# Sirui-Xu/InterDiff

Hardware: AMD Instinct MI355X
Metric: denoising frame-steps/sec (denoising-steps/sec x B x T frames) (higher is better)
Workload: dtype f32 (every contraction of the denoiser -- feed-forward block, QKV projection, self-attention, row-block contractions and the two token GEMMs: every fp32 operand as two f16 planes, 3 f16 MFMAs per product, fp32 accumulate; SMPL and everything else fp32 MFMA / VALU)

## Files before the change

include/interdiff_hip.h:

```cpp
#ifndef INTERDIFF_HIP_H
#define INTERDIFF_HIP_H

#include <stddef.h>
#include <stdint.h>

#ifdef __cplusplus
extern "C" {
#endif

#define IDF_OK            0
#define IDF_E_INVAL      -22
#define IDF_E_NOMEM      -12
#define IDF_E_LAUNCH     -5

int         interdiff_abi_version(void);
const char *interdiff_build_info(void);

int interdiff_rotation_6d_to_matrix   (const float *d6, float *m,  int64_t n, void *stream);
int interdiff_matrix_to_rotation_6d   (const float *m,  float *d6, int64_t n, void *stream);
int interdiff_matrix_to_axis_angle    (const float *m,  float *aa, int64_t n, void *stream);
int interdiff_axis_angle_to_matrix    (const float *aa, float *m,  int64_t n, void *stream);
int interdiff_axis_angle_to_quaternion(const float *aa, float *q,  int64_t n, void *stream);
int interdiff_rotation_6d_to_axis_angle(const float *d6, float *aa, int64_t n, void *stream);

typedef struct {
    int32_t V, J, n_betas, KB, S;
    const float   *blend;
    const float   *jt;
    const float   *js;
    const int32_t *parents;
    const int32_t *skin_idx;
    const float   *skin_w;
} idf_smpl_model;

size_t interdiff_smpl_workspace_bytes(const idf_smpl_model *m, int64_t N);
int interdiff_smpl_forward(const idf_smpl_model *m, const float *pose, const float *betas,
                           const float *trans, int64_t N, float *verts, float *jtr,
                           float *v_posed, void *ws, size_t ws_bytes, void *stream);

int interdiff_vertex_normals(const float *verts, int64_t N, int32_t V, const int32_t *faces,
                             const int32_t *adj_ptr, const int32_t *adj_face,
                             const int32_t *adj_corner, float *normals, void *stream);
int interdiff_nn_argmin(const float *q, int32_t Pq, const float *r, int32_t Pr, int64_t N,
                        int32_t *idx, void *stream);
int interdiff_point2point_signed(const float *x, int32_t P1, const float *y, int32_t P2, int64_t N,
                                 const float *x_normals, const float *y_normals,
                                 float *y2x_signed, float *x2y_signed, int32_t *yidx, int32_t *xidx,
                                 float *y2x, float *x2y, void *stream);

#define IDF_MDM_LAYERS 8
#define IDF_MDM_D      256
#define IDF_MDM_FF     1024
#define IDF_MDM_HEADS  4
#define IDF_MDM_NQ     10
#define IDF_MDM_MEM    10
#define IDF_MDM_MEM_MAX 16
#define IDF_FFN_SLICES 5

typedef struct {
    int64_t is_qan;
    int64_t sa_in_w, sa_in_b, sa_out_w, sa_out_b;
    int64_t qc, wk;
    int64_t ca_q_w, ca_q_b;
    int64_t ca_kv_w, ca_kv_b;
    int64_t ca_out_w, ca_out_b;
    int64_t ff1_w, ff1_b, ff2_w, ff2_b;
    int64_t ffn_pack;
    int64_t ffn_b1p;
    int64_t sa_in_pack;
    int64_t sa_out_frag;
    int64_t ln_w[3], ln_b[3];
    int64_t ffn_pack_h2;
    int64_t sa_in_pack_h2;
    int64_t qc_h2;
    int64_t rb_h2_ok;
    int64_t sa_out_frag_h2;
    int64_t qkv_bounds_ok;
} idf_mdm_layer;

typedef struct {
    int32_t C;
    int32_t n_steps;
    const float *arena;
    int64_t in_w, in_b;
    int64_t out_w, out_b;
    int64_t temb_table;
    int64_t pe;
    int32_t max_T, has_encoder;
    idf_mdm_layer layer[IDF_MDM_LAYERS];
    idf_mdm_layer enc_layer[IDF_MDM_LAYERS];
    int32_t tune[8];
    int64_t out_w_h2, in_w_h2;
    int64_t tail_h2_ok;
    int32_t mem_len;
    int32_t rb_tokens;
} idf_mdm_weights;

int interdiff_gemm_f32(const float *A, int32_t lda, const float *W, const float *bias, const float *resid, float *C,
                       int32_t ldc, int32_t M, int32_t N, int32_t K, int32_t epi, int32_t cfg, void *stream);

int interdiff_mdm_ffn(const idf_mdm_weights *w, int32_t layer, int32_t encoder, const float *x2, int32_t M, float *parts, void *stream);
size_t interdiff_mdm_memctx_floats_for(int32_t B, int32_t mem_len);

size_t interdiff_mdm_memctx_floats(int32_t B);
size_t interdiff_mdm_workspace_bytes(int32_t B, int32_t T);
int interdiff_mdm_prepare_memory(const idf_mdm_weights *w, const float *cond, int32_t B,
                                 float *memctx, void *ws, size_t ws_bytes, void *stream);
int interdiff_mdm_forward(const idf_mdm_weights *w, const float *memctx, const float *x,
                          const int64_t *ts, int32_t B, int32_t T, float *x0,
                          void *ws, size_t ws_bytes, void *stream);

typedef struct {
    int64_t w[3], b[3];
    int32_t c[4];
} idf_pn_mlp;

typedef struct {
    const float *arena;
    idf_pn_mlp sa1[2];
    idf_pn_mlp sa2[2];
    int64_t lin_w, lin_b;
} idf_pointnet2;

int interdiff_pointnet2_encode(const idf_pointnet2 *pn, const float *obj_points, int32_t B, int32_t P, float *out,
                               void *stream);
size_t interdiff_mdm_encode_workspace_bytes(int32_t B, int32_t Tp);
int interdiff_mdm_encode(const idf_mdm_weights *w, const float *pc, const float *x_past, int32_t B, int32_t Tp,
                         float *cond, void *ws, size_t ws_bytes, void *stream);

int interdiff_inpaint(float *x0, const float *gt, const uint8_t *mask, int64_t n, void *stream);
int interdiff_posterior_step(float *x, const float *x0, const float *noise, int64_t n,
                             float c1, float c2, float sigma, uint64_t seed, uint64_t step_index,
                             void *stream);
int interdiff_randn(float *out, int64_t n, uint64_t seed, uint64_t step_index, void *stream);
int interdiff_posterior_step_at(float *x, const float *x0, const float *noise, int64_t n,
                                float c1, float c2, float sigma, uint64_t seed, uint64_t step_index,
                                uint64_t elem0, void *stream);
int interdiff_randn_at(float *out, int64_t n, uint64_t seed, uint64_t step_index, uint64_t elem0, void *stream);
int interdiff_posterior_step_dev(float *x, const float *x0, const float *gt, const uint8_t *mask, int64_t n,
                                 const float *table, int64_t *state, int64_t *ts, int32_t B, void *stream);
int interdiff_sampler_advance(int64_t *state, int64_t *ts, int32_t B, void *stream);
int interdiff_posterior_step_dev_map(float *x, const float *x0, const float *gt, const uint8_t *mask, int64_t n,
                                     const float *table, const int64_t *tmap, int64_t *state, int64_t *ts, int32_t B, void *stream);
int interdiff_sampler_advance_map(int64_t *state, int64_t *ts, const int64_t *tmap, int32_t B, void *stream);
int interdiff_mdm_forward_step(const idf_mdm_weights *w, const float *memctx, float *x, int64_t *ts, int32_t B, int32_t T,
                               const float *gt, const uint8_t *mask, const float *table, int64_t *state,
                               void *ws, size_t ws_bytes, void *stream);
#define IDF_STEP_EMBED_READY 1
#define IDF_STEP_EMBED_NEXT 2
int interdiff_mdm_forward_step_ex(const idf_mdm_weights *w, const float *memctx, float *x, int64_t *ts, int32_t B, int32_t T,
                                  const float *gt, const uint8_t *mask, const float *table, int64_t *state, void *ws,
                                  size_t ws_bytes, int32_t flags, void *stream);
int interdiff_mdm_forward_step_map(const idf_mdm_weights *w, const float *memctx, float *x, int64_t *ts, int32_t B, int32_t T,
                                   const float *gt, const uint8_t *mask, const float *table, const int64_t *tmap, int64_t *state,
                                   void *ws, size_t ws_bytes, int32_t flags, void *stream);
int interdiff_mdm_step_chaining(const idf_mdm_weights *w);
int interdiff_exclusive_cu_report(char *buf, int32_t cap);
int interdiff_debug_deny_exclusive(const char *patterns);

typedef struct {
    int32_t T, past_len, P, n_pre;
    const float *arena;
    int64_t dct_pad;
    int64_t dct;
    int64_t idct;
    int64_t hand_bonus;
    int64_t layer[12];
    int32_t cin[12], cout[12];
} idf_objproj;

int interdiff_objprojector_sample(const idf_objproj *op, const float *obj_angles,
                                  const float *obj_trans, const float *markers,
                                  const int32_t *contact, int32_t B, float *out, void *stream);
size_t interdiff_objprojector_forward_workspace_bytes(int32_t B);
int interdiff_objprojector_forward(const idf_objproj *op, const float *obj_angles, const float *obj_trans, const float *markers,
                                   const int32_t *contact, int32_t B, int32_t initialize, float *out, void *ws, size_t ws_bytes, void *stream);

typedef struct {
    const idf_smpl_model *smpl;
    const idf_objproj    *objproj;
    const int32_t *faces;
    const int32_t *adj_ptr, *adj_face, *adj_corner;
    const int32_t *markers_idx;
    int32_t n_markers, n_points, past_len;
    int32_t tune;
    const int32_t *vorder, *faces_scan, *markers_scan, *adj_pair_scan;
    const int32_t *adj_pair;
    const int32_t *vrank;
} idf_correction_ctx;

size_t interdiff_correction_workspace_bytes(const idf_correction_ctx *c, int32_t B, int32_t T);
int interdiff_correction(const idf_correction_ctx *c, float *x0, const float *gt,
                         const float *hand_pose, const float *beta, const float *obj_points,
                         int32_t B, int32_t T, float blend_t ,
                         uint8_t *condition, int32_t *contact, float *distance, float *loss,
                         void *ws, size_t ws_bytes, void *stream);
int interdiff_correction_dev(const idf_correction_ctx *c, float *x0, const float *gt, const float *hand_pose,
                             const float *beta, const float *obj_points, int32_t B, int32_t T, const float *table,
                             const int64_t *state, void *ws, size_t ws_bytes, void *stream);

#define IDF_CONTACT_STATS 12
size_t interdiff_contact_nn_workspace_bytes(const idf_correction_ctx *c, int32_t B, int32_t T);
int interdiff_contact_nn(const idf_correction_ctx *c, const float *verts, const float *obj_points, const float *objR,
                         const float *objT, int32_t B, int32_t T, float *o2h, int32_t *idx, uint64_t *stats,
                         void *ws, size_t ws_bytes, void *stream);

size_t interdiff_metrics_workspace_bytes(const idf_correction_ctx *c, int32_t B, int32_t T);
int interdiff_metrics(const idf_correction_ctx *c, const float *obj_pred, const float *jtr,
                      const float *body_trans, const float *obj_gt, const float *jtr_gt,
                      const float *body_trans_gt, const float *verts, const float *obj_points,
                      int32_t B, int32_t T, int32_t J, float *out6 ,
                      void *ws, size_t ws_bytes, void *stream);

typedef struct {
    int32_t T, past_len, J, n_pre;
    const float *arena;
    int64_t dct_pad;
    int64_t dct;
    int64_t idct;
    int64_t layer[12];
    int32_t cin[12], cout[12];
} idf_skel_objproj;

int interdiff_skeleton_objprojector_sample(const idf_skel_objproj *op, const float *obj_angles,
                                           const float *obj_trans, const float *human_points, int32_t B,
                                           float *quat_out, float *trans_out, void *stream);
int interdiff_skeleton_correction(const idf_skel_objproj *op, const float *x, const float *gt,
                                  const float *zero_pose_obj, int32_t B, int32_t T, float blend_t,
                                  float *out, void *stream);
int interdiff_skeleton_metrics(const float *body_pred, const float *body_gt, const float *obj_pred,
                               const float *obj_gt, const float *pose_pred, const float *pose_gt,
                               int32_t T, int32_t B, int32_t from_frame, float *out4, void *stream);

int interdiff_skeleton_finetune_param_table(const idf_skel_objproj *op, int32_t *table, int32_t *n_param, int32_t *n_bn);
size_t interdiff_skeleton_finetune_workspace_bytes(const idf_skel_objproj *op, int32_t B);
int interdiff_skeleton_finetune_grads(const idf_skel_objproj *op, const float *params, const float *bn, const float *obj_angles,
                                      const float *obj_trans, const float *human_points, const float *pose_gt, int32_t B, int32_t T,
                                      const float *weights8, float *out9, float *grads, void *ws, size_t ws_bytes, void *stream);
int interdiff_skeleton_finetune_step(const idf_skel_objproj *op, float *arena, float *params, const float *bn, const float *grads,
                                     float *exp_avg, float *exp_avg_sq, int32_t step, double lr, double beta1, double beta2, double eps,
                                     double weight_decay, void *stream);

typedef struct idf_skel_head {
    int32_t n_body, n_points;
    int32_t n_tiles, reserved;
    int64_t out_w, out_b;
    int64_t shape_w, shape_b;
} idf_skel_head;
int interdiff_skeleton_mdm_forward(const idf_mdm_weights *w, const idf_skel_head *head, const float *memctx, const float *x,
                                   const int64_t *ts, const float *zero_pose_obj, int32_t B, int32_t T, float *x0,
                                   void *ws, size_t ws_bytes, void *stream);
int interdiff_skeleton_mdm_forward_step(const idf_mdm_weights *w, const idf_skel_head *head, const float *memctx, float *x,
                                        int64_t *ts, const float *zero_pose_obj, int32_t B, int32_t T, const float *gt,
                                        const uint8_t *mask, const float *table, int64_t *state, void *ws, size_t ws_bytes,
                                        void *stream);
int interdiff_skeleton_mdm_forward_step_map(const idf_mdm_weights *w, const idf_skel_head *head, const float *memctx, float *x,
                                            int64_t *ts, const float *zero_pose_obj, int32_t B, int32_t T, const float *gt,
                                            const uint8_t *mask, const float *table, const int64_t *tmap, int64_t *state, void *ws,
                                            size_t ws_bytes, void *stream);
size_t interdiff_skeleton_mdm_encode_workspace_bytes(int32_t B, int32_t Tp);
int interdiff_skeleton_mdm_encode(const idf_mdm_weights *w, const idf_skel_head *head, const float *zero_pose_obj,
                                  const float *x_past, int32_t B, int32_t Tp, float *cond, void *ws, size_t ws_bytes,
                                  void *stream);

#define IDF_OPT_NP 483
#define IDF_OPT_NLOSS 6
typedef struct {
    const idf_correction_ctx *geo;
    const float   *blendT;
    const int32_t *jv_ptr;
    const int32_t *jv_vtx;
    const float   *jv_w;
    int32_t K3P, _pad;
} idf_opt_ctx;

typedef struct {
    int32_t B, T, P, max_iters;
    const float *betas;
    const float *obj_points;
    float *param, *init, *grad, *m, *v, *best;
    float *pose, *tr;
    float *verts, *vposed, *verts_gt, *gv;
    float *jtr;
    float *pts, *y2x;
    float *y2x_signed;
    int32_t *yidx;
    int32_t *near;
    float *dvposed;
    float *dA;
    float *dfeat;
    float *gtr;
    float *lossf;
    float *loss;
    float *loss_hist;
    float *best_loss;
    int32_t *flag;
    uint8_t *foot_static;
    int32_t *foot_cnt;
    int32_t *ctl;
    void *smpl_ws; size_t smpl_ws_bytes;
    int32_t *porder; float *psort, *pbox;
} idf_opt_state;

int interdiff_optimize_init(const idf_opt_ctx *c, const idf_opt_state *st, const float *pose, const float *trans,
                            const float *obj_angles, const float *obj_trans, int32_t first_iter, void *stream);
int interdiff_optimize_loss_grad(const idf_opt_ctx *c, const idf_opt_state *st, void *stream);
int interdiff_optimize_step(const idf_opt_ctx *c, const idf_opt_state *st, void *stream);
int interdiff_optimize_finish(const idf_opt_ctx *c, const idf_opt_state *st, float *pose, float *trans, float *obj_angles,
                              float *obj_trans, void *stream);
int interdiff_debug_joint_map_vjp(const float *R, const float *g_out, float *g_in, int32_t n);
int interdiff_debug_lds_sentinel(uint32_t *out, int32_t n_wg, int32_t spin, void *stream);
int interdiff_debug_f16_aggressor(const float *src, size_t n_floats, float *sink, int32_t iters, int32_t grid, int32_t with_loads, void *stream);

enum { IDF_LOSS_VAL = 0, IDF_LOSS_TEST = 1 };
int interdiff_q_sample(float *x_t, const float *x0, const float *noise, const int64_t *ts, const float *sqrt_ac, const float *sqrt_1mac,
                       int32_t n_steps, const float *gt, const uint8_t *mask, int32_t B, int64_t per_clip, uint64_t seed, uint64_t elem0,
                       void *stream);
int interdiff_denoising_losses(const float *pred, const float *target, int32_t B, int32_t T, int32_t past_len, float *out, void *stream);
size_t interdiff_sample_losses_workspace_bytes(int32_t K, int32_t B);
int interdiff_sample_losses(const float *samples, const float *gt, const float *hand_pose, int32_t K, int32_t B, int32_t T, int32_t past_len,
                            int32_t variant, float *out_terms, float *out_per_clip, void *ws, size_t ws_bytes, void *stream);

size_t interdiff_skeleton_sample_losses_workspace_bytes(int32_t K, int32_t B);
int interdiff_skeleton_sample_losses(const float *pred, const float *gt, int32_t K, int32_t B, int32_t C, int32_t T, int32_t past_len,
                                     int32_t n_body, int32_t n_points, float *out_terms, float *out_per_clip, void *ws, size_t ws_bytes,
                                     void *stream);
int interdiff_skeleton_denoising_losses(const float *pred, const float *target, int32_t B, int32_t T, int32_t past_len, int32_t n_body,
                                        int32_t n_points, float *out, void *stream);

size_t interdiff_correction_losses_workspace_bytes(int32_t T, int32_t B, int32_t V, int32_t P);
int interdiff_correction_losses(const float *obj_pred, const float *obj_gt, const float *obj_points, int32_t point_stride, const float *human_verts,
                                int32_t T, int32_t B, int32_t V, int32_t P, int32_t rot_width, int32_t past_len, float *out_terms, float *out_frames,
                                void *ws, size_t ws_bytes, void *stream);

size_t interdiff_contact_labels_workspace_bytes(int64_t N, int32_t V, int32_t F, int32_t P);
int interdiff_contact_labels(const float *verts, int64_t N, int32_t V, const int32_t *faces, int32_t F, const float *points, int32_t P,
                             int64_t point_frame_stride, const float *objR, const float *objT, float thres, uint8_t *obj_label ,
                             uint8_t *human_label , float *signed_dist , void *ws, size_t ws_bytes, void *stream);
int interdiff_debug_point_triangle(const float *tri, const float *p, float *out, int32_t n);

#define IDF_RENDER_SUBPIX 16
#define IDF_RENDER_GUARD 32768
#define IDF_RENDER_MAX_DIM 2048
#define IDF_RENDER_ZONE (1 << 28)
#define IDF_RENDER_REC_INTS 20
#define IDF_RENDER_TILE 16
#define IDF_RENDER_MAX_MESHES 8
enum { IDF_RMESH_SCENE_SPACE = 1, IDF_RMESH_VERTEX_RGB = 2 };
typedef struct {
    float off[3], cam_t[3];
    float cam_cos, cam_sin, znear, focal;
    float light[9];
    float light_gain, ambient;
    float bg[3];
    float reserved;
} idf_render_scene;
typedef struct {
    const float *verts, *normals;
    const int32_t *faces;
    const float *rgb, *R, *t;
    int32_t V, F, frames, flags;
} idf_render_mesh;
size_t interdiff_render_frames_workspace_bytes(int64_t n_images, int64_t n_triangles, int32_t H, int32_t W);
int interdiff_render_frames(const idf_render_scene *scene, const idf_render_mesh *meshes, int32_t n_meshes, int64_t N, int32_t views, int32_t H,
                            int32_t W, uint8_t *out_rgb, int32_t *out_id, int32_t *out_depth, int32_t *out_setup, int64_t *dropped, float *stage_ms,
                            void *ws, size_t ws_bytes, void *stream);
int interdiff_debug_render_setup_vertex(const idf_render_scene *scene, int32_t view, int32_t scene_space, int32_t H, int32_t W, const float *pos,
                                        const float *nrm, const float *rgb, float *out_f, int32_t *out_i, int32_t n);
int interdiff_debug_render_pixel(const int32_t *rec, const int32_t *ij, int32_t *out, int32_t n);

enum {
    IDF_K_EMBED = 0, IDF_K_GEMM_QKV, IDF_K_SELF_ATTN, IDF_K_GEMM_OUTPROJ, IDF_K_ROWBLOCK_QAN,
    IDF_K_ROWBLOCK_STD, IDF_K_FFN_FUSED, IDF_K_RESERVED7, IDF_K_GEMM_HEADS, IDF_K_MEM_PREP,
    IDF_K_INPAINT, IDF_K_POSTERIOR, IDF_K_CORR_PREPARE, IDF_K_SMPL_POSE, IDF_K_SMPL_BLEND_SKIN,
    IDF_K_CORR_CONTACT, IDF_K_CORR_REDUCE, IDF_K_OBJPROJ, IDF_K_CORR_BLEND, IDF_K_OTHER,
    IDF_K_COUNT
};
int interdiff_profile_begin(int32_t capacity);
int interdiff_profile_end(double *ms_per_kind, int64_t *count_per_kind);

enum {
    IDF_TUNE_FFN = 3, IDF_TUNE_FFN_MATH = 4, IDF_TUNE_COUNT = 8
};

#ifdef __cplusplus
}
#endif
#endif
```

interdiff_amd/_lib.py:

```python
import ctypes as C
import os
import torch

_HERE = os.path.dirname(os.path.abspath(__file__))
LIB_PATH = os.environ.get('INTERDIFF_HIP_LIB') or os.path.join(_HERE, 'csrc', 'libinterdiff_hip.so')
ABI_VERSION = 17

vp, i32, i64, f32, u64, sz = C.c_void_p, C.c_int32, C.c_int64, C.c_float, C.c_uint64, C.c_size_t

MDM_LAYERS = 8
FFN_SLICES = 5
STEP_EMBED_READY, STEP_EMBED_NEXT = 1, 2
LOSS_VAL, LOSS_TEST = 0, 1
TUNE = dict(ffn=3, ffn_math=4)


class SmplModel(C.Structure):
    _fields_ = [('V', i32), ('J', i32), ('n_betas', i32), ('KB', i32), ('S', i32),
                ('blend', vp), ('jt', vp), ('js', vp), ('parents', vp), ('skin_idx', vp), ('skin_w', vp)]


class MdmLayer(C.Structure):
    _fields_ = [('is_qan', i64),
                ('sa_in_w', i64), ('sa_in_b', i64), ('sa_out_w', i64), ('sa_out_b', i64),
                ('qc', i64), ('wk', i64),
                ('ca_q_w', i64), ('ca_q_b', i64), ('ca_kv_w', i64), ('ca_kv_b', i64),
                ('ca_out_w', i64), ('ca_out_b', i64),
                ('ff1_w', i64), ('ff1_b', i64), ('ff2_w', i64), ('ff2_b', i64), ('ffn_pack', i64), ('ffn_b1p', i64), ('sa_in_pack', i64), ('sa_out_frag', i64),
                ('ln_w', i64 * 3), ('ln_b', i64 * 3), ('ffn_pack_h2', i64), ('sa_in_pack_h2', i64), ('qc_h2', i64), ('rb_h2_ok', i64), ('sa_out_frag_h2', i64), ('qkv_bounds_ok', i64)]


class MdmWeights(C.Structure):
    _fields_ = [('C', i32), ('n_steps', i32), ('arena', vp),
                ('in_w', i64), ('in_b', i64), ('out_w', i64), ('out_b', i64),
                ('temb_table', i64), ('pe', i64), ('max_T', i32), ('has_encoder', i32),
                ('layer', MdmLayer * MDM_LAYERS), ('enc_layer', MdmLayer * MDM_LAYERS), ('tune', i32 * 8), ('out_w_h2', i64), ('in_w_h2', i64), ('tail_h2_ok', i64), ('mem_len', i32), ('rb_tokens', i32)]


class PnMlp(C.Structure):
    _fields_ = [('w', i64 * 3), ('b', i64 * 3), ('c', i32 * 4)]


class PointNet2(C.Structure):
    _fields_ = [('arena', vp), ('sa1', PnMlp * 2), ('sa2', PnMlp * 2), ('lin_w', i64), ('lin_b', i64)]


class ObjProj(C.Structure):
    _fields_ = [('T', i32), ('past_len', i32), ('P', i32), ('n_pre', i32), ('arena', vp),
                ('dct_pad', i64), ('dct', i64), ('idct', i64), ('hand_bonus', i64),
                ('layer', i64 * 12), ('cin', i32 * 12), ('cout', i32 * 12)]


class SkelObjProj(C.Structure):
    _fields_ = [('T', i32), ('past_len', i32), ('J', i32), ('n_pre', i32), ('arena', vp),
                ('dct_pad', i64), ('dct', i64), ('idct', i64),
                ('layer', i64 * 12), ('cin', i32 * 12), ('cout', i32 * 12)]


class SkelHead(C.Structure):
    _fields_ = [('n_body', i32), ('n_points', i32), ('n_tiles', i32), ('reserved', i32),
                ('out_w', i64), ('out_b', i64), ('shape_w', i64), ('shape_b', i64)]


class CorrectionCtx(C.Structure):
    _fields_ = [('smpl', C.POINTER(SmplModel)), ('objproj', C.POINTER(ObjProj)),
                ('faces', vp), ('adj_ptr', vp), ('adj_face', vp), ('adj_corner', vp), ('markers_idx', vp),
                ('n_markers', i32), ('n_points', i32), ('past_len', i32), ('tune', i32),
                ('vorder', vp), ('faces_scan', vp), ('markers_scan', vp), ('adj_pair_scan', vp), ('adj_pair', vp), ('vrank', vp)]


class OptCtx(C.Structure):
    _fields_ = [('geo', C.POINTER(CorrectionCtx)), ('blendT', vp), ('jv_ptr', vp), ('jv_vtx', vp), ('jv_w', vp), ('K3P', i32), ('_pad', i32)]


OPT_NP, OPT_NLOSS = 483, 6
_OPT_PTRS = ('betas', 'obj_points', 'param', 'init', 'grad', 'm', 'v', 'best', 'pose', 'tr', 'verts', 'vposed', 'verts_gt', 'gv',
             'jtr', 'pts', 'y2x', 'y2x_signed', 'yidx', 'near', 'dvposed', 'dA', 'dfeat', 'gtr', 'lossf', 'loss', 'loss_hist',
             'best_loss', 'flag', 'foot_static', 'foot_cnt', 'ctl', 'smpl_ws')


class OptState(C.Structure):
    _fields_ = [('B', i32), ('T', i32), ('P', i32), ('max_iters', i32)] + [(k, vp) for k in _OPT_PTRS] + [('smpl_ws_bytes', sz), ('porder', vp), ('psort', vp), ('pbox', vp)]


class RenderScene(C.Structure):
    _fields_ = [('off', f32 * 3), ('cam_t', f32 * 3), ('cam_cos', f32), ('cam_sin', f32), ('znear', f32), ('focal', f32),
                ('light', f32 * 9), ('light_gain', f32), ('ambient', f32), ('bg', f32 * 3), ('reserved', f32)]


class RenderMesh(C.Structure):
    _fields_ = [('verts', vp), ('normals', vp), ('faces', vp), ('rgb', vp), ('R', vp), ('t', vp),
                ('V', i32), ('F', i32), ('frames', i32), ('flags', i32)]


RMESH_SCENE_SPACE, RMESH_VERTEX_RGB = 1, 2
RENDER_SUBPIX, RENDER_GUARD, RENDER_MAX_DIM, RENDER_ZONE, RENDER_REC_INTS, RENDER_TILE = 16, 32768, 2048, 1 << 28, 20, 16

_SIGS = {
    'interdiff_abi_version': (C.c_int, []),
    'interdiff_build_info': (C.c_char_p, []),
    'interdiff_rotation_6d_to_matrix': (C.c_int, [vp, vp, i64, vp]),
    'interdiff_matrix_to_rotation_6d': (C.c_int, [vp, vp, i64, vp]),
    'interdiff_matrix_to_axis_angle': (C.c_int, [vp, vp, i64, vp]),
    'interdiff_axis_angle_to_matrix': (C.c_int, [vp, vp, i64, vp]),
    'interdiff_axis_angle_to_quaternion': (C.c_int, [vp, vp, i64, vp]),
    'interdiff_rotation_6d_to_axis_angle': (C.c_int, [vp, vp, i64, vp]),
    'interdiff_smpl_workspace_bytes': (sz, [C.POINTER(SmplModel), i64]),
    'interdiff_smpl_forward': (C.c_int, [C.POINTER(SmplModel), vp, vp, vp, i64, vp, vp, vp, vp, sz, vp]),
    'interdiff_vertex_normals': (C.c_int, [vp, i64, i32, vp, vp, vp, vp, vp, vp]),
    'interdiff_nn_argmin': (C.c_int, [vp, i32, vp, i32, i64, vp, vp]),
    'interdiff_point2point_signed': (C.c_int, [vp, i32, vp, i32, i64, vp, vp, vp, vp, vp, vp, vp, vp, vp]),
    'interdiff_gemm_f32': (C.c_int, [vp, i32, vp, vp, vp, vp, i32, i32, i32, i32, i32, i32, vp]),
    'interdiff_pointnet2_encode': (C.c_int, [C.POINTER(PointNet2), vp, i32, i32, vp, vp]),
    'interdiff_mdm_encode_workspace_bytes': (sz, [i32, i32]),
    'interdiff_mdm_encode': (C.c_int, [C.POINTER(MdmWeights), vp, vp, i32, i32, vp, vp, sz, vp]),
    'interdiff_mdm_ffn': (C.c_int, [C.POINTER(MdmWeights), i32, i32, vp, i32, vp, vp]),
    'interdiff_mdm_memctx_floats': (sz, [i32]),
    'interdiff_mdm_memctx_floats_for': (sz, [i32, i32]),
    'interdiff_mdm_workspace_bytes': (sz, [i32, i32]),
    'interdiff_mdm_prepare_memory': (C.c_int, [C.POINTER(MdmWeights), vp, i32, vp, vp, sz, vp]),
    'interdiff_mdm_forward': (C.c_int, [C.POINTER(MdmWeights), vp, vp, vp, i32, i32, vp, vp, sz, vp]),
    'interdiff_mdm_forward_step': (C.c_int, [C.POINTER(MdmWeights), vp, vp, vp, i32, i32, vp, vp, vp, vp, vp, sz, vp]),
    'interdiff_mdm_forward_step_ex': (C.c_int, [C.POINTER(MdmWeights), vp, vp, vp, i32, i32, vp, vp, vp, vp, vp, sz, i32, vp]),
    'interdiff_mdm_forward_step_map': (C.c_int, [C.POINTER(MdmWeights), vp, vp, vp, i32, i32, vp, vp, vp, vp, vp, vp, sz, i32, vp]),
    'interdiff_mdm_step_chaining': (C.c_int, [C.POINTER(MdmWeights)]),
    'interdiff_inpaint': (C.c_int, [vp, vp, vp, i64, vp]),
    'interdiff_posterior_step': (C.c_int, [vp, vp, vp, i64, f32, f32, f32, u64, u64, vp]),
    'interdiff_randn': (C.c_int, [vp, i64, u64, u64, vp]),
    'interdiff_posterior_step_at': (C.c_int, [vp, vp, vp, i64, f32, f32, f32, u64, u64, u64, vp]),
    'interdiff_randn_at': (C.c_int, [vp, i64, u64, u64, u64, vp]),
    'interdiff_posterior_step_dev': (C.c_int, [vp, vp, vp, vp, i64, vp, vp, vp, i32, vp]),
    'interdiff_sampler_advance': (C.c_int, [vp, vp, i32, vp]),
    'interdiff_posterior_step_dev_map': (C.c_int, [vp, vp, vp, vp, i64, vp, vp, vp, vp, i32, vp]),
    'interdiff_sampler_advance_map': (C.c_int, [vp, vp, vp, i32, vp]),
    'interdiff_objprojector_sample': (C.c_int, [C.POINTER(ObjProj), vp, vp, vp, vp, i32, vp, vp]),
    'interdiff_objprojector_forward_workspace_bytes': (sz, [i32]),
    'interdiff_objprojector_forward': (C.c_int, [C.POINTER(ObjProj), vp, vp, vp, vp, i32, i32, vp, vp, sz, vp]),
    'interdiff_correction_workspace_bytes': (sz, [C.POINTER(CorrectionCtx), i32, i32]),
    'interdiff_correction': (C.c_int, [C.POINTER(CorrectionCtx), vp, vp, vp, vp, vp, i32, i32, f32,
                                       vp, vp, vp, vp, vp, sz, vp]),
    'interdiff_correction_dev': (C.c_int, [C.POINTER(CorrectionCtx), vp, vp, vp, vp, vp, i32, i32, vp, vp, vp, sz, vp]),
    'interdiff_metrics_workspace_bytes': (sz, [C.POINTER(CorrectionCtx), i32, i32]),
    'interdiff_metrics': (C.c_int, [C.POINTER(CorrectionCtx), vp, vp, vp, vp, vp, vp, vp, vp, i32, i32, i32,
                                    vp, vp, sz, vp]),
    'interdiff_contact_nn_workspace_bytes': (sz, [C.POINTER(CorrectionCtx), i32, i32]),
    'interdiff_contact_nn': (C.c_int, [C.POINTER(CorrectionCtx), vp, vp, vp, vp, i32, i32, vp, vp, vp, vp, sz, vp]),
    'interdiff_skeleton_objprojector_sample': (C.c_int, [C.POINTER(SkelObjProj), vp, vp, vp, i32, vp, vp, vp]),
    'interdiff_skeleton_correction': (C.c_int, [C.POINTER(SkelObjProj), vp, vp, vp, i32, i32, f32, vp, vp]),
    'interdiff_skeleton_metrics': (C.c_int, [vp, vp, vp, vp, vp, vp, i32, i32, i32, vp, vp]),
    'interdiff_skeleton_finetune_param_table': (C.c_int, [C.POINTER(SkelObjProj), vp, C.POINTER(i32), C.POINTER(i32)]),
    'interdiff_skeleton_finetune_workspace_bytes': (sz, [C.POINTER(SkelObjProj), i32]),
    'interdiff_skeleton_finetune_grads': (C.c_int, [C.POINTER(SkelObjProj), vp, vp, vp, vp, vp, vp, i32, i32, C.POINTER(f32), vp, vp, vp, sz, vp]),
    'interdiff_skeleton_finetune_step': (C.c_int, [C.POINTER(SkelObjProj), vp, vp, vp, vp, vp, vp, i32, C.c_double, C.c_double, C.c_double, C.c_double,
                                                   C.c_double, vp]),
    'interdiff_skeleton_mdm_forward': (C.c_int, [C.POINTER(MdmWeights), C.POINTER(SkelHead), vp, vp, vp, vp, i32, i32, vp, vp, sz, vp]),
    'interdiff_skeleton_mdm_forward_step': (C.c_int, [C.POINTER(MdmWeights), C.POINTER(SkelHead), vp, vp, vp, vp, i32, i32, vp, vp, vp, vp, vp, sz, vp]),
    'interdiff_skeleton_mdm_forward_step_map': (C.c_int, [C.POINTER(MdmWeights), C.POINTER(SkelHead), vp, vp, vp, vp, i32, i32, vp, vp, vp, vp, vp, vp, sz, vp]),
    'interdiff_skeleton_mdm_encode_workspace_bytes': (sz, [i32, i32]),
    'interdiff_skeleton_mdm_encode': (C.c_int, [C.POINTER(MdmWeights), C.POINTER(SkelHead), vp, vp, i32, i32, vp, vp, sz, vp]),
    'interdiff_q_sample': (C.c_int, [vp, vp, vp, vp, vp, vp, i32, vp, vp, i32, i64, u64, u64, vp]),
    'interdiff_denoising_losses': (C.c_int, [vp, vp, i32, i32, i32, vp, vp]),
    'interdiff_sample_losses_workspace_bytes': (sz, [i32, i32]),
    'interdiff_sample_losses': (C.c_int, [vp, vp, vp, i32, i32, i32, i32, i32, vp, vp, vp, sz, vp]),
    'interdiff_skeleton_sample_losses_workspace_bytes': (sz, [i32, i32]),
    'interdiff_skeleton_sample_losses': (C.c_int, [vp, vp, i32, i32, i32, i32, i32, i32, i32, vp, vp, vp, sz, vp]),
    'interdiff_skeleton_denoising_losses': (C.c_int, [vp, vp, i32, i32, i32, i32, i32, vp, vp]),
    'interdiff_correction_losses_workspace_bytes': (sz, [i32, i32, i32, i32]),
    'interdiff_correction_losses': (C.c_int, [vp, vp, vp, i32, vp, i32, i32, i32, i32, i32, i32, vp, vp, vp, sz, vp]),
    'interdiff_contact_labels_workspace_bytes': (sz, [i64, i32, i32, i32]),
    'interdiff_contact_labels': (C.c_int, [vp, i64, i32, vp, i32, vp, i32, i64, vp, vp, f32, vp, vp, vp, vp, sz, vp]),
    'interdiff_debug_point_triangle': (C.c_int, [vp, vp, vp, i32]),
    'interdiff_render_frames_workspace_bytes': (sz, [i64, i64, i32, i32]),
    'interdiff_render_frames': (C.c_int, [C.POINTER(RenderScene), C.POINTER(RenderMesh), i32, i64, i32, i32, i32, vp, vp, vp, vp, C.POINTER(i64), C.POINTER(f32),
                                          vp, sz, vp]),
    'interdiff_debug_render_setup_vertex': (C.c_int, [C.POINTER(RenderScene), i32, i32, i32, i32, vp, vp, vp, vp, vp, i32]),
    'interdiff_debug_render_pixel': (C.c_int, [vp, vp, vp, i32]),
    'interdiff_optimize_init': (C.c_int, [C.POINTER(OptCtx), C.POINTER(OptState), vp, vp, vp, vp, i32, vp]),
    'interdiff_optimize_loss_grad': (C.c_int, [C.POINTER(OptCtx), C.POINTER(OptState), vp]),
    'interdiff_optimize_step': (C.c_int, [C.POINTER(OptCtx), C.POINTER(OptState), vp]),
    'interdiff_optimize_finish': (C.c_int, [C.POINTER(OptCtx), C.POINTER(OptState), vp, vp, vp, vp, vp]),
    'interdiff_debug_joint_map_vjp': (C.c_int, [vp, vp, vp, i32]),
    'interdiff_debug_lds_sentinel': (C.c_int, [vp, i32, i32, vp]),
    'interdiff_exclusive_cu_report': (C.c_int, [C.c_char_p, i32]),
    'interdiff_debug_deny_exclusive': (C.c_int, [C.c_char_p]),
    'interdiff_debug_f16_aggressor': (C.c_int, [vp, sz, vp, i32, i32, i32, vp]),
    'interdiff_profile_begin': (C.c_int, [i32]),
    'interdiff_profile_end': (C.c_int, [C.POINTER(C.c_double), C.POINTER(C.c_int64)]),
}

KERNEL_KINDS = ('embed', 'gemm_qkv', 'self_attn', 'gemm_outproj', 'rowblock_qan', 'rowblock_std', 'ffn_fused', 'reserved7',
                'gemm_heads', 'mem_prep', 'inpaint', 'posterior', 'corr_prepare', 'smpl_pose', 'smpl_blend_skin',
                'corr_contact', 'corr_reduce', 'objproj', 'corr_blend', 'other')

_lib = None


class HipLibraryMissing(RuntimeError):
    pass


def load():
    global _lib
    if _lib is not None:
        return _lib
    if not os.path.exists(LIB_PATH):
        raise HipLibraryMissing('%s not found: build it with `python -m interdiff_amd.csrc.build` '
                                '(there is no CPU/torch fallback for the hot path)' % LIB_PATH)
    lib = C.CDLL(LIB_PATH)
    for name, (res, args) in _SIGS.items():
        fn = getattr(lib, name)
        fn.restype, fn.argtypes = res, args
    if lib.interdiff_abi_version() != ABI_VERSION:
        raise HipLibraryMissing('stale %s: abi %d != %d, rebuild' % (LIB_PATH, lib.interdiff_abi_version(), ABI_VERSION))
    _lib = lib
    return lib


def exclusive_cu_report():
    buf = C.create_string_buffer(8192)
    bad = load().interdiff_exclusive_cu_report(buf, len(buf))
    if bad < 0:
        check(bad, 'exclusive_cu_report')
    return buf.value.decode(), bad


def debug_deny_exclusive(patterns=''):
    check(load().interdiff_debug_deny_exclusive(patterns.encode() if patterns else None), 'debug_deny_exclusive')


def exported_symbols():
    return sorted(_SIGS)


_ERR = {-22: 'IDF_E_INVAL (bad shape / pointer / unsupported size)', -12: 'IDF_E_NOMEM (workspace too small)',
        -5: 'IDF_E_LAUNCH (kernel launch failed)'}


def check(rc, what=''):
    if rc != 0:
        raise RuntimeError('interdiff_hip %s failed: %s' % (what, _ERR.get(rc, rc)))


def dptr(t, dtype=None, allow_none=False):
    if t is None:
        if allow_none:
            return vp(None)
        raise ValueError('null tensor')
    if not t.is_cuda:
        raise ValueError('interdiff_amd ops need device tensors (got %s); the HIP path has no CPU fallback' % t.device)
    if not t.is_contiguous():
        raise ValueError('tensor must be contiguous')
    if dtype is not None and t.dtype != dtype:
        raise ValueError('expected %s, got %s' % (dtype, t.dtype))
    return vp(t.data_ptr())


def stream():
    return vp(torch.cuda.current_stream().cuda_stream)
```

interdiff_amd/correction.py:

```python
import ctypes as C
import os
import itertools
import numpy as np
import torch
from . import _lib
from .geometry import MeshTopology

MARKERS67 = [3470, 3171, 3327, 857, 1812, 628, 182, 3116, 3040, 239,
             1666, 1725, 0, 2174, 1568, 1368, 3387, 2112, 1053, 1058,
             3336, 3346, 1323, 2108, 3122, 3314, 1252, 1082, 1861, 1454,
             850, 2224, 3233, 1769, 6728, 4343, 5273, 4116, 3694, 6399,
             6540, 6488, 3749, 5135, 5194, 3512, 5635, 5210, 4360, 4841,
             6786, 5573, 4538, 4544, 6736, 6747, 4804, 5568, 6544, 6682,
             5322, 4927, 5686, 4598, 6633, 3506, 3508]


_UID = itertools.count(1)


def correction_gate(t0):
    return not (t0 > 500 or t0 % 50 != 0)


class HipCorrection:
    def __init__(self, smpl_layer, objprojector, n_points=2048, past_len=10, markers=MARKERS67, device='cuda', scan_order=True):
        self.lib = _lib.load()
        self.device = torch.device(device)
        self.smpl, self.objproj, self.past_len = smpl_layer, objprojector, past_len
        self.topo = MeshTopology(smpl_layer.th_faces, smpl_layer.cmodel.V, self.device, rest_vertices=getattr(smpl_layer, 'v_template', None) if scan_order else None)
        self.markers_idx = torch.tensor(list(markers), dtype=torch.int32, device=self.device)
        ctx = _lib.CorrectionCtx()
        ctx.smpl = C.pointer(smpl_layer.cmodel)
        ctx.objproj = C.pointer(objprojector.cop)
        ctx.faces, ctx.adj_ptr = self.topo.faces.data_ptr(), self.topo.adj_ptr.data_ptr()
        ctx.adj_face, ctx.adj_corner = self.topo.adj_face.data_ptr(), self.topo.adj_corner.data_ptr()
        ctx.markers_idx = self.markers_idx.data_ptr()
        ctx.n_markers, ctx.n_points, ctx.past_len = len(markers), n_points, past_len
        if self.topo.vorder is not None:
            self.markers_scan = self.topo.scan_positions(markers, self.device)
            ctx.vorder, ctx.faces_scan, ctx.markers_scan = self.topo.vorder.data_ptr(), self.topo.faces_scan.data_ptr(), self.markers_scan.data_ptr()
            ctx.adj_pair_scan = self.topo.adj_pair_scan.data_ptr()
            ctx.vrank = self.topo.vrank.data_ptr()
        ctx.tune = 0
        self.ctx = ctx
        self._ws = {}
        self.debug = None
        self._uid = next(_UID)

    graph_capturable = True

    def workspace_for(self, B, T):
        return torch.empty(self.lib.interdiff_correction_workspace_bytes(C.byref(self.ctx), B, T), dtype=torch.uint8, device=self.device)

    def apply_dev(self, x, table, state, y, ws):
        B, _, Cc, T = x.shape
        if y['obj_points'].shape[1] != self.ctx.n_points:
            raise ValueError('obj_points must have %d points' % self.ctx.n_points)
        _lib.check(self.lib.interdiff_correction_dev(C.byref(self.ctx), _lib.dptr(x, torch.float32), _lib.dptr(y['inpainted_motion'], torch.float32),
                                                     _lib.dptr(y['hand_pose'], torch.float32), _lib.dptr(y['beta'], torch.float32),
                                                     _lib.dptr(y['obj_points'], torch.float32), B, T, _lib.dptr(table), _lib.dptr(state),
                                                     _lib.dptr(ws), ws.numel(), _lib.stream()), 'correction_dev')
        return x

    def _workspace(self, B, T):
        need = self.lib.interdiff_correction_workspace_bytes(C.byref(self.ctx), B, T)
        key = torch.cuda.current_stream(self.device).cuda_stream
        ws = self._ws.pop(key, None)
        if ws is None or ws.numel() < need:
            ws = torch.empty(need, dtype=torch.uint8, device=self.device)
        self._ws[key] = ws
        if len(self._ws) > self.MAX_STREAM_WORKSPACES:
            torch.cuda.synchronize(self.device)
            self._ws.pop(next(iter(self._ws)))
        return ws

    MAX_STREAM_WORKSPACES = 4

    def apply(self, x, t0, y):
        B, _, Cc, T = x.shape
        if not x.is_contiguous():
            raise ValueError('x must be contiguous (it is updated in place)')
        if y['obj_points'].shape[1] != self.ctx.n_points:
            raise ValueError('obj_points must have %d points' % self.ctx.n_points)
        gt = y['inpainted_motion'].contiguous()
        hp, beta, pts = y['hand_pose'].contiguous().float(), y['beta'].contiguous().float(), y['obj_points'].contiguous().float()
        ws = self._workspace(B, T)
        dbg = [None] * 4
        if self.debug is not None:
            dbg = [torch.empty(B, dtype=torch.uint8, device=self.device), torch.empty(B, len(MARKERS67), dtype=torch.int32, device=self.device),
                   torch.empty(B, device=self.device), torch.empty(B, device=self.device)]
        blend_t = float(np.float32(t0) / np.float32(1000))
        _lib.check(self.lib.interdiff_correction(C.byref(self.ctx), _lib.dptr(x, torch.float32), _lib.dptr(gt, torch.float32),
                                                 _lib.dptr(hp), _lib.dptr(beta), _lib.dptr(pts), B, T, blend_t,
                                                 *[_lib.dptr(d, allow_none=True) for d in dbg], _lib.dptr(ws), ws.numel(),
                                                 _lib.stream()), 'correction')
        if self.debug is not None:
            self.debug.update(condition=dbg[0], contact=dbg[1], distance=dbg[2], loss=dbg[3])
        return x

    def contact_nn(self, verts, obj_points, objR, objT, want_stats=False):
        T, B = verts.shape[:2]
        P = self.ctx.n_points
        o2h = torch.empty(T, B, P, device=self.device)
        idx = torch.empty(T, B, P, dtype=torch.int32, device=self.device)
        stats = torch.zeros(12, dtype=torch.int64, device=self.device) if want_stats else None
        need = self.lib.interdiff_contact_nn_workspace_bytes(C.byref(self.ctx), B, T)
        ws = getattr(self, '_nn_ws', None)
        if ws is None or ws.numel() < need:
            ws = self._nn_ws = torch.empty(need, dtype=torch.uint8, device=self.device)
        v, pts, R_, t_ = (a.contiguous().float() for a in (verts, obj_points, objR, objT))
        _lib.check(self.lib.interdiff_contact_nn(C.byref(self.ctx), _lib.dptr(v), _lib.dptr(pts), _lib.dptr(R_), _lib.dptr(t_), B, T, _lib.dptr(o2h),
                                                 _lib.dptr(idx), _lib.dptr(stats, allow_none=True), _lib.dptr(ws), ws.numel(), _lib.stream()), 'contact_nn')
        return (o2h, idx, tuple(int(x) for x in stats.cpu())) if want_stats else (o2h, idx)

    def is_active(self, t0):
        return correction_gate(int(t0))

    def __call__(self, x, t, model_kwargs):
        t0 = getattr(t, 'host_value', None)
        if t0 is None:
            t0 = int(t[0])
        if not correction_gate(t0):
            return x
        return self.apply(x, t0, model_kwargs['y'])
```

interdiff_amd/csrc/correction.hip:

```cpp
#include "common.h"
#include "objproj.h"
#include "rot_math.h"
#include <float.h>

namespace {

constexpr int NBODY = 22;
constexpr int CTOK = 144;

__global__ __launch_bounds__(256) void corr_prepare_kernel(const float *__restrict__ x0, const float *__restrict__ gt,
                                                           const float *__restrict__ hand_pose, int B, int T,
                                                           float *__restrict__ pose, float *__restrict__ trans,
                                                           float *__restrict__ objR, float *__restrict__ objT,
                                                           float *__restrict__ gt_angles, float *__restrict__ gt_trans) {
    const int64_t i = (int64_t)blockIdx.x * 256 + threadIdx.x;
    const int64_t N = (int64_t)B * T;
    if (i >= N * 24) return;
    const int64_t n = i / 24;
    const int slot = (int)(i - n * 24), t = (int)(n / B), b = (int)(n - (int64_t)t * B);
    const float *xb = x0 + (size_t)b * CTOK * T + t;
    if (slot < NBODY) {
        float d[6], m[9], a[3];
#pragma unroll
        for (int k = 0; k < 6; ++k) d[k] = xb[(size_t)(slot * 6 + k) * T];
        rot::rot6d_to_matrix(d, m);
        rot::matrix_to_axis_angle(m, a);
        float *p = pose + n * 156 + slot * 3;
        p[0] = a[0]; p[1] = a[1]; p[2] = a[2];
    } else if (slot == 22) {
        for (int k = 0; k < 90; ++k) pose[n * 156 + 66 + k] = hand_pose[n * 90 + k];
#pragma unroll
        for (int k = 0; k < 3; ++k) trans[n * 3 + k] = xb[(size_t)(132 + k) * T];
    } else {
        float d[6], m[9];
#pragma unroll
        for (int k = 0; k < 6; ++k) d[k] = xb[(size_t)(135 + k) * T];
        rot::rot6d_to_matrix(d, m);
#pragma unroll
        for (int k = 0; k < 9; ++k) objR[n * 9 + k] = m[k];
        const float *gb = gt + (size_t)b * CTOK * T + t;
#pragma unroll
        for (int k = 0; k < 3; ++k) {
            objT[n * 3 + k] = xb[(size_t)(141 + k) * T];
            gt_trans[n * 3 + k] = gb[(size_t)(141 + k) * T];
        }
#pragma unroll
        for (int k = 0; k < 6; ++k) gt_angles[n * 6 + k] = gb[(size_t)(135 + k) * T];
    }
}

__device__ __forceinline__ float dist2_exact(float qx, float qy, float qz, float rx, float ry, float rz) {
#pragma clang fp contract(off)
    const float dx = qx - rx, dy = qy - ry, dz = qz - rz;
    const float xx = dx * dx, yy = dy * dy, zz = dz * dz;
    return (xx + yy) + zz;
}

__device__ __forceinline__ float3 f3(const float4 v) { return make_float3(v.x, v.y, v.z); }
__device__ __forceinline__ float3 sub3(float3 a, float3 b) { return make_float3(a.x - b.x, a.y - b.y, a.z - b.z); }
__device__ __forceinline__ float3 cross3(float3 a, float3 b) {
    return make_float3(a.y * b.z - a.z * b.y, a.z * b.x - a.x * b.z, a.x * b.y - a.y * b.x);
}

constexpr int MAXP = 2048;
__global__ __launch_bounds__(1024) void corr_point_order_kernel(const float *__restrict__ obj_points, int P, int32_t *__restrict__ porder) {
    __shared__ unsigned long long keys[MAXP];
    __shared__ float red[6][1024];
    const int b = blockIdx.x, tid = threadIdx.x;
    const float *op = obj_points + (size_t)b * P * 3;
    float p[2][3];
    float lo[3] = {FLT_MAX, FLT_MAX, FLT_MAX}, hi[3] = {-FLT_MAX, -FLT_MAX, -FLT_MAX};
#pragma unroll
    for (int k = 0; k < 2; ++k) {
        const int i = tid + 1024 * k;
#pragma unroll
        for (int a = 0; a < 3; ++a) {
            p[k][a] = i < P ? op[3 * i + a] : 0.f;
            if (i < P) { lo[a] = fminf(lo[a], p[k][a]); hi[a] = fmaxf(hi[a], p[k][a]); }
        }
    }
#pragma unroll
    for (int a = 0; a < 3; ++a) { red[a][tid] = lo[a]; red[3 + a][tid] = hi[a]; }
    __syncthreads();
    for (int s = 512; s > 0; s >>= 1) {
        if (tid < s) {
#pragma unroll
            for (int a = 0; a < 3; ++a) {
                red[a][tid] = fminf(red[a][tid], red[a][tid + s]);
                red[3 + a][tid] = fmaxf(red[3 + a][tid], red[3 + a][tid + s]);
            }
        }
        __syncthreads();
    }
#pragma unroll
    for (int k = 0; k < 2; ++k) {
        const int i = tid + 1024 * k;
        unsigned long long key = ~0ull;
        if (i < P) {
            unsigned code = 0;
            unsigned q[3];
#pragma unroll
            for (int a = 0; a < 3; ++a) {
                const float ext = red[3 + a][0] - red[a][0];
                const float u = ext > 0.f ? (p[k][a] - red[a][0]) / ext : 0.f;
                q[a] = (unsigned)fminf(fmaxf(u * 1023.0f, 0.f), 1023.0f);
            }
#pragma unroll
            for (int bit = 0; bit < 10; ++bit)
#pragma unroll
                for (int a = 0; a < 3; ++a) code |= ((q[a] >> bit) & 1u) << (3 * bit + a);
            key = ((unsigned long long)code << 11) | (unsigned)i;
        }
        keys[i] = key;
    }
    __syncthreads();
    for (int k = 2; k <= MAXP; k <<= 1) {
        for (int j = k >> 1; j > 0; j >>= 1) {
            const int l = 2 * j * (tid / j) + (tid % j), r = l + j;
            const unsigned long long x = keys[l], y = keys[r];
            const bool up = (l & k) == 0;
            if ((x > y) == up) { keys[l] = y; keys[r] = x; }
            __syncthreads();
        }
    }
#pragma unroll
    for (int k = 0; k < 2; ++k) {
        const int i = tid + 1024 * k;
        if (i < P) porder[(size_t)b * P + i] = (int32_t)(keys[i] & 2047u);
    }
}

constexpr int MAXM = 128;
constexpr float MARK_D2 = 0.00039999996079131961f;
constexpr int CB = 16;
constexpr int SB = 8;
constexpr int SEED_STRIDE = 4;
constexpr int CT = 1024;
constexpr int TASK = 64;
typedef float v2f __attribute__((ext_vector_type(2)));

struct ContactLds {
    int V4, nCB, nSB, nSeed;
    int rec, mark, box, sbox, seed, flags, red, pl, total;
    __host__ __device__ explicit ContactLds(int V) {
        V4 = (V + CB - 1) / CB * CB; nCB = V4 / CB; nSB = (nCB + SB - 1) / SB; nSeed = (nCB + SEED_STRIDE - 1) / SEED_STRIDE;
        rec = 0;
        mark = rec + V4;
        box = mark + MAXM;
        sbox = box + 3 * (nSB * SB / 2);
        seed = sbox + 3 * ((nSB + 2) / 2);
        flags = seed + 2 * ((nSeed + 1) / 2);
        red = flags + MAXM / 4;
        pl = red + CT / 4;
        total = pl + MAXP / 4;
    }
};

__device__ __forceinline__ float3 lds_rec(const float4 *vs, int pos) {
    const float *f = reinterpret_cast<const float *>(vs + 2 * (pos >> 1));
    const int h = pos & 1;
    return make_float3(f[h], f[2 + h], f[4 + h]);
}
__device__ __forceinline__ void lds_rec_store(float4 *vs, int pos, float x, float y, float z) {
    float *f = reinterpret_cast<float *>(vs + 2 * (pos >> 1));
    const int h = pos & 1;
    f[h] = x; f[2 + h] = y; f[4 + h] = z;
}
__device__ __forceinline__ void lds_box_store(float4 *bx, int k, float3 lo, float3 hi) {
    float *f = reinterpret_cast<float *>(bx + 3 * (k >> 1));
    const int h = k & 1;
    f[h] = lo.x; f[2 + h] = lo.y; f[4 + h] = lo.z; f[6 + h] = hi.x; f[8 + h] = hi.y; f[10 + h] = hi.z;
}
__device__ __forceinline__ void lds_box_load(const float4 *bx, int k, float3 &lo, float3 &hi) {
    const float *f = reinterpret_cast<const float *>(bx + 3 * (k >> 1));
    const int h = k & 1;
    lo = make_float3(f[h], f[2 + h], f[4 + h]);
    hi = make_float3(f[6 + h], f[8 + h], f[10 + h]);
}

struct PredArgs {
    idf_objproj op;
    const float *obj_angles, *obj_trans;
    const int32_t *markers_idx;
    float *markers, *keep;
    int nclips;
};
template <bool OPT, bool WITH_PRED = false>
__global__ __launch_bounds__(CT) void corr_contact_kernel(const float *__restrict__ verts, int V,
                                                          const float *__restrict__ obj_points, int P,
                                                          const int32_t *__restrict__ porder ,
                                                          const float *__restrict__ objR, const float *__restrict__ objT,
                                                          const int32_t *__restrict__ faces ,
                                                          const int32_t *__restrict__ adj_ptr,
                                                          const int32_t *__restrict__ adj_face,
                                                          const int32_t *__restrict__ adj_corner,
                                                          const int32_t *__restrict__ adj_pair ,
                                                          const int32_t *__restrict__ vorder ,
                                                          const int32_t *__restrict__ vrank ,
                                                          const int32_t *__restrict__ markers_pos , int M, int B,
                                                          float *__restrict__ markers_out, float *__restrict__ loss_sum,
                                                          float *__restrict__ min_dist, int32_t *__restrict__ label,
                                                          float *__restrict__ o2h_out ,
                                                          int32_t *__restrict__ idx_out ,
                                                          unsigned long long *__restrict__ stats ,
                                                          int64_t nn_from ,
                                                          const float *__restrict__ pts_frame , int frames_per_clip ,
                                                          const PredArgs pred) {
    extern __shared__ __attribute__((aligned(16))) float4 vs[];
    if constexpr (WITH_PRED) {
        if ((int)blockIdx.x < pred.nclips) {
            const int b = blockIdx.x, Tn = pred.op.T;
            for (int i = threadIdx.x; i < Tn * M; i += CT) {
                const int t = i / M, m = i - t * M;
                const size_t nfr = (size_t)t * B + b;
                const float *v = verts + (nfr * V + pred.markers_idx[m]) * 3;
                float *o = pred.markers + (nfr * M + m) * 3;
                o[0] = v[0]; o[1] = v[1]; o[2] = v[2];
            }
            __threadfence();
            __syncthreads();
            idf_objproj_dev::objproj_body<1>(reinterpret_cast<float *>(vs), pred.op, pred.obj_angles, pred.obj_trans, pred.markers, nullptr, B, b, pred.keep, nullptr);
            return;
        }
    }
    const ContactLds L(V);
    const int nCB = L.nCB, nSB = L.nSB;
    float4 *ms = vs + L.mark, *bb = vs + L.box, *sbb = vs + L.sbox, *sd = vs + L.seed;
    int *flags = reinterpret_cast<int *>(vs + L.flags);
    float *red = reinterpret_cast<float *>(vs + L.red);
    float *pl = reinterpret_cast<float *>(vs + L.pl);
    __shared__ int next_task;
    const int64_t n = WITH_PRED ? (int64_t)blockIdx.x - pred.nclips : (int64_t)blockIdx.x;
    const int b = OPT ? (int)(n / frames_per_clip) : (int)(n % B), tid = threadIdx.x;
    const float *vf = verts + (size_t)n * V * 3;
    const bool do_nn = n >= nn_from;
    long long t_prev = 0;
    int n_phase = 0;
    auto phase_done = [&]() {
        if (stats && tid == 0 && do_nn) {
            const long long now = (long long)__builtin_readcyclecounter();
            if (n_phase > 0) atomicAdd(stats + 3 + n_phase, (unsigned long long)(now - t_prev));
            t_prev = now;
        }
        ++n_phase;
    };
    phase_done();
    float R[9] = {1.f, 0.f, 0.f, 0.f, 1.f, 0.f, 0.f, 0.f, 1.f}, tr[3] = {0.f, 0.f, 0.f};
    if constexpr (!OPT) {
#pragma unroll
        for (int k = 0; k < 9; ++k) R[k] = objR[n * 9 + k];
#pragma unroll
        for (int k = 0; k < 3; ++k) tr[k] = objT[n * 3 + k];
    }
    const int my_marker_pos = (!OPT && tid < M) ? markers_pos[tid] : 0;
    if (vorder && vrank) {
        for (int i0 = tid; i0 < V; i0 += 4 * CT) {
            typedef float f3v __attribute__((ext_vector_type(3), aligned(4)));
            int pos[4];
            f3v pv[4];
#pragma unroll
            for (int k = 0; k < 4; ++k) {
                const int i = min(i0 + k * CT, V - 1);
                pos[k] = vrank[i];
                pv[k] = *reinterpret_cast<const f3v *>(vf + 3 * i);
            }
#pragma unroll
            for (int k = 0; k < 4; ++k) {
                if (i0 + k * CT < V) {
                    lds_rec_store(vs, pos[k], pv[k].x, pv[k].y, pv[k].z);
                    reinterpret_cast<int *>(vs + 2 * (pos[k] >> 1) + 1)[2 + (pos[k] & 1)] = i0 + k * CT;
                }
            }
        }
        for (int v = V + tid; v < L.V4; v += CT) {
            lds_rec_store(vs, v, 3e18f, 3e18f, 3e18f);
            reinterpret_cast<int *>(vs + 2 * (v >> 1) + 1)[2 + (v & 1)] = 0x7fffffff;
        }
    } else
    for (int v0 = tid; v0 < L.V4; v0 += 4 * CT) {
        int o[4];
        float x[4], y[4], z[4];
#pragma unroll
        for (int k = 0; k < 4; ++k) {
            const int v = v0 + k * CT;
            o[k] = v < V ? (vorder ? vorder[v] : v) : -1;
        }
#pragma unroll
        for (int k = 0; k < 4; ++k) {
            x[k] = y[k] = z[k] = 3e18f;
            if (o[k] >= 0) {
                typedef float f3v __attribute__((ext_vector_type(3), aligned(4)));
                const f3v pv = *reinterpret_cast<const f3v *>(vf + 3 * o[k]);
                x[k] = pv.x; y[k] = pv.y; z[k] = pv.z;
            }
        }
#pragma unroll
        for (int k = 0; k < 4; ++k) {
            const int v = v0 + k * CT;
            if (v < L.V4) {
                lds_rec_store(vs, v, x[k], y[k], z[k]);
                reinterpret_cast<int *>(vs + 2 * (v >> 1) + 1)[2 + (v & 1)] = o[k] >= 0 ? o[k] : 0x7fffffff;
            }
        }
    }
    if (tid < MAXM) flags[tid] = 0;
    const int ntask_all = (P + TASK - 1) / TASK;
    const int task0 = (int)((long long)blockIdx.y * ntask_all / gridDim.y), task1 = (int)((long long)(blockIdx.y + 1) * ntask_all / gridDim.y);
    if (tid == 0) next_task = task0;
    for (int i = tid; i < MAXP; i += CT) pl[i] = 0.f;
    __syncthreads();
    phase_done();
    if (!OPT && tid < ((M + 1) & ~1)) {
        float3 mk = make_float3(3e18f, 3e18f, 3e18f);
        if (tid < M) {
            mk = lds_rec(vs, my_marker_pos);
            if (markers_out) {
                float *mo = markers_out + ((size_t)n * M + tid) * 3;
                mo[0] = mk.x; mo[1] = mk.y; mo[2] = mk.z;
            }
        }
        lds_rec_store(ms, tid, mk.x, mk.y, mk.z);
    }
    if (do_nn) {
#define IDF_DPP8(v, op, ctrl) v = op(v, __builtin_bit_cast(float, __builtin_amdgcn_update_dpp(__builtin_bit_cast(int, v), __builtin_bit_cast(int, v), ctrl, 0xf, 0xf, false)))
        const int lane_ = tid & 63, wave_ = tid >> 6, nsw = 2 * ((nSB + 2) / 2);
        for (int sb = wave_; sb < nsw; sb += CT / 64) {
            const int pr = sb * 64 + lane_;
            float lx = FLT_MAX, ly = FLT_MAX, lz = FLT_MAX, hx = -FLT_MAX, hy = -FLT_MAX, hz = -FLT_MAX;
            if (2 * pr < V) {
                const float4 xy = vs[2 * pr], zz = vs[2 * pr + 1];
                const bool two = 2 * pr + 1 < V;
                lx = two ? fminf(xy.x, xy.y) : xy.x; hx = two ? fmaxf(xy.x, xy.y) : xy.x;
                ly = two ? fminf(xy.z, xy.w) : xy.z; hy = two ? fmaxf(xy.z, xy.w) : xy.z;
                lz = two ? fminf(zz.x, zz.y) : zz.x; hz = two ? fmaxf(zz.x, zz.y) : zz.x;
            }
            IDF_DPP8(lx, fminf, 0xB1); IDF_DPP8(lx, fminf, 0x4E); IDF_DPP8(lx, fminf, 0x141);
            IDF_DPP8(ly, fminf, 0xB1); IDF_DPP8(ly, fminf, 0x4E); IDF_DPP8(ly, fminf, 0x141);
            IDF_DPP8(lz, fminf, 0xB1); IDF_DPP8(lz, fminf, 0x4E); IDF_DPP8(lz, fminf, 0x141);
            IDF_DPP8(hx, fmaxf, 0xB1); IDF_DPP8(hx, fmaxf, 0x4E); IDF_DPP8(hx, fmaxf, 0x141);
            IDF_DPP8(hy, fmaxf, 0xB1); IDF_DPP8(hy, fmaxf, 0x4E); IDF_DPP8(hy, fmaxf, 0x141);
            IDF_DPP8(hz, fmaxf, 0xB1); IDF_DPP8(hz, fmaxf, 0x4E); IDF_DPP8(hz, fmaxf, 0x141);
            const int cb = sb * SB + (lane_ >> 3);
            if ((lane_ & 7) == 0 && cb < nSB * SB) lds_box_store(bb, cb, make_float3(lx, ly, lz), make_float3(hx, hy, hz));
            const float slx = -wave_max(-lx), sly = -wave_max(-ly), slz = -wave_max(-lz), shx = wave_max(hx), shy = wave_max(hy), shz = wave_max(hz);
            if (lane_ == 0) lds_box_store(sbb, sb, make_float3(slx, sly, slz), make_float3(shx, shy, shz));
        }
#undef IDF_DPP8
        for (int k = tid; k < 2 * ((L.nSeed + 1) / 2); k += CT) {
            const float3 p = lds_rec(vs, min(k * SEED_STRIDE, nCB - 1) * CB);
            lds_rec_store(sd, k, p.x, p.y, p.z);
        }
    }
    const float *op = OPT ? pts_frame + (size_t)n * P * 3 : obj_points + (size_t)b * P * 3;
    const int ln = tid & 63, ntask = task1;
    __syncthreads();
    phase_done();
    float mind2 = FLT_MAX;
    unsigned n_exec = 0, n_test = 0, n_tasks = 0;
    for (;;) {
        int task = 0;
        if (ln == 0) task = atomicAdd(&next_task, 1);
        task = __builtin_amdgcn_readfirstlane(task);
        if (task >= ntask) break;
        ++n_tasks;
        const int sp = task * TASK + ln;
        const int i = sp < P ? (porder ? porder[(size_t)b * P + sp] : sp) : -1;
        const bool valid = i >= 0;
        float px = 0.f, py = 0.f, pz = 0.f;
        if (valid) { px = op[3 * i]; py = op[3 * i + 1]; pz = op[3 * i + 2]; }
        const float qx = OPT ? px : (px * R[0] + py * R[1] + pz * R[2]) + tr[0];
        const float qy = OPT ? py : (px * R[3] + py * R[4] + pz * R[5]) + tr[1];
        const float qz = OPT ? pz : (px * R[6] + py * R[7] + pz * R[8]) + tr[2];
        if (do_nn) {
#pragma clang fp contract(off)
            const v2f QX = v2f{qx, qx}, QY = v2f{qy, qy}, QZ = v2f{qz, qz};
            auto pair_d2 = [&](const float4 xy, const float4 zz) {
#pragma clang fp contract(off)
                const v2f dx = QX - v2f{xy.x, xy.y}, dy = QY - v2f{xy.z, xy.w}, dz = QZ - v2f{zz.x, zz.y};
                return (dx * dx + dy * dy) + dz * dz;
            };
            auto pair_a2 = [&](const float4 xy, const float2 zz) {
                const v2f dx = QX - v2f{xy.x, xy.y}, dy = QY - v2f{xy.z, xy.w}, dz = QZ - v2f{zz.x, zz.y};
                return __builtin_elementwise_fma(dz, dz, __builtin_elementwise_fma(dy, dy, dx * dx));
            };
            constexpr float SCAN_M = 1.000003814697265625f, SCAN_ABS = 1e-37f;
            float seed = FLT_MAX;
            for (int k = 0; k < (L.nSeed + 1) / 2; k += 4) {
                float4 xy[4]; float2 zz[4];
#pragma unroll
                for (int u = 0; u < 4; ++u) { xy[u] = sd[2 * min(k + u, (L.nSeed + 1) / 2 - 1)]; zz[u] = *reinterpret_cast<const float2 *>(&sd[2 * min(k + u, (L.nSeed + 1) / 2 - 1) + 1]); }
#pragma unroll
                for (int u = 0; u < 4; ++u) {
                    const v2f a2 = pair_a2(xy[u], zz[u]);
                    seed = fminf(fminf(seed, a2.x), a2.y);
                }
            }
            float thr = __builtin_fmaf(seed, SCAN_M, SCAN_ABS);
            float best = FLT_MAX, bthr = FLT_MAX;
            int tie = 0;
            int bblk = 0, bblk2 = 0;
            auto pair_lb = [&](const float4 a, const float4 bq, const float4 c) {
#pragma clang fp contract(off)
                const v2f ax = v2f{a.x, a.y} - QX, bx = QX - v2f{bq.z, bq.w};
                const v2f ay = v2f{a.z, a.w} - QY, by = QY - v2f{c.x, c.y};
                const v2f az = v2f{bq.x, bq.y} - QZ, bz = QZ - v2f{c.z, c.w};
                const v2f ex = v2f{fmaxf(fmaxf(ax.x, bx.x), 0.f), fmaxf(fmaxf(ax.y, bx.y), 0.f)};
                const v2f ey = v2f{fmaxf(fmaxf(ay.x, by.x), 0.f), fmaxf(fmaxf(ay.y, by.y), 0.f)};
                const v2f ez = v2f{fmaxf(fmaxf(az.x, bz.x), 0.f), fmaxf(fmaxf(az.y, bz.y), 0.f)};
                return __builtin_elementwise_fma(ez, ez, __builtin_elementwise_fma(ey, ey, ex * ex));
            };
            auto score_block = [&](int cb) {
                ++n_exec;
                const int v0 = cb * CB;
                float4 xy[CB / 2]; float2 zz[CB / 2];
#pragma unroll
                for (int u = 0; u < CB / 2; ++u) { xy[u] = vs[v0 + 2 * u]; zz[u] = *reinterpret_cast<const float2 *>(&vs[v0 + 2 * u + 1]); }
                float bm = FLT_MAX;
#pragma unroll
                for (int u = 0; u < CB / 2; ++u) {
                    const v2f a2 = pair_a2(xy[u], zz[u]);
                    bm = fminf(fminf(bm, a2.x), a2.y);
                }
                if (bm < best) {
                    const float w = __builtin_fmaf(bm, SCAN_M, SCAN_ABS);
                    if (best <= w) { tie = tie ? 2 : 1; bblk2 = bblk; } else tie = 0;
                    best = bm; bblk = v0; bthr = w; thr = fminf(thr, w);
                } else if (bm <= bthr) { tie = tie ? 2 : 1; bblk2 = v0; }
            };
            auto scan_super = [&](int sb) {
                const int cb0 = sb * SB;
#pragma unroll
                for (int j = 0; j < SB / 2; ++j) {
                    const int cb = cb0 + 2 * j;
                    const float4 *bx = bb + 3 * (cb >> 1);
                    const v2f lb = pair_lb(bx[0], bx[1], bx[2]);
                    n_test += 2;
                    if (__builtin_amdgcn_ballot_w64(valid && lb.x <= thr) != 0ull) score_block(cb);
                    if (__builtin_amdgcn_ballot_w64(valid && lb.y <= thr) != 0ull) score_block(cb + 1);
                }
            };
            if (!vorder) {
                for (int cb = 0; cb < nCB; ++cb) score_block(cb);
            } else
            for (int sb = 0; sb < nSB; sb += 2) {
                const float4 *bx = sbb + 3 * (sb >> 1);
                const v2f lb = pair_lb(bx[0], bx[1], bx[2]);
                n_test += 2;
                if (__builtin_amdgcn_ballot_w64(valid && lb.x <= thr) != 0ull) scan_super(sb);
                if (__builtin_amdgcn_ballot_w64(valid && lb.y <= thr) != 0ull) scan_super(sb + 1);
            }
            int pos = bblk, org = 0x7fffffff;
            float ebest = FLT_MAX;
            auto resolve_pair = [&](int pr) {
                const float4 xy = vs[2 * pr], zz = vs[2 * pr + 1];
                const v2f d2 = pair_d2(xy, zz);
                const int o0 = __builtin_bit_cast(int, zz.z), o1 = __builtin_bit_cast(int, zz.w);
                if (d2.x < ebest || (d2.x == ebest && o0 < org)) { ebest = d2.x; org = o0; pos = 2 * pr; }
                if (d2.y < ebest || (d2.y == ebest && o1 < org)) { ebest = d2.y; org = o1; pos = 2 * pr + 1; }
            };
            if (tie < 2) {
#pragma unroll
                for (int u = 0; u < CB / 2; ++u) resolve_pair((bblk >> 1) + u);
                if (tie) {
#pragma unroll
                    for (int u = 0; u < CB / 2; ++u) resolve_pair((bblk2 >> 1) + u);
                }
            } else {
                for (int pr = 0; pr < (V + 1) / 2; ++pr) resolve_pair(pr);
            }
            pos = min(pos, V - 1);
            if (org == 0x7fffffff) org = vorder ? vorder[pos] : pos;
            if constexpr (OPT) {
                if (valid) idx_out[(size_t)n * P + i] = org;
            } else if (valid) {
                const float3 v3 = lds_rec(vs, pos);
                float3 acc = make_float3(0.f, 0.f, 0.f);
                const int e0 = adj_ptr[org], e1 = adj_ptr[org + 1];
                if (adj_pair) {
                    for (int e = e0; e < e1; e += 4) {
                        int2 ab[4];
#pragma unroll
                        for (int u = 0; u < 4; ++u) ab[u] = *reinterpret_cast<const int2 *>(adj_pair + 2 * (size_t)min(e + u, e1 - 1));
#pragma unroll
                        for (int u = 0; u < 4; ++u) {
                            if (e + u < e1) {
                                const float3 nn = cross3(sub3(lds_rec(vs, ab[u].x), v3), sub3(lds_rec(vs, ab[u].y), v3));
                                acc.x += nn.x; acc.y += nn.y; acc.z += nn.z;
                            }
                        }
                    }
                } else {
                    for (int e = e0; e < e1; ++e) {
                        const int f = adj_face[e], c = adj_corner[e];
                        const float3 p0 = lds_rec(vs, faces[3 * f]), p1 = lds_rec(vs, faces[3 * f + 1]), p2 = lds_rec(vs, faces[3 * f + 2]);
                        float3 nn;
                        if (c == 1) nn = cross3(sub3(p2, p1), sub3(p0, p1));
                        else if (c == 2) nn = cross3(sub3(p0, p2), sub3(p1, p2));
                        else nn = cross3(sub3(p1, p0), sub3(p2, p0));
                        acc.x += nn.x; acc.y += nn.y; acc.z += nn.z;
                    }
                }
                const float nl = fmaxf(sqrtf(acc.x * acc.x + acc.y * acc.y + acc.z * acc.z), 1e-6f);
                const float vx = qx - v3.x, vy = qy - v3.y, vz = qz - v3.z;
                const float dt = (acc.x / nl) * vx + (acc.y / nl) * vy + (acc.z / nl) * vz;
                const float d = sqrtf(vx * vx + vy * vy + vz * vz);
                const float o2h = d * (dt > 0.f ? 1.f : (dt < 0.f ? -1.f : 0.f));
                if (o2h_out) o2h_out[(size_t)n * P + i] = o2h;
                if (idx_out) idx_out[(size_t)n * P + i] = org;
                pl[sp] = o2h < 0.f ? fabsf(o2h) * 20.0f : 0.f;
            }
        }
        if (!OPT && valid) {
#pragma clang fp contract(off)
            const v2f QX = v2f{qx, qx}, QY = v2f{qy, qy}, QZ = v2f{qz, qz};
            for (int p2 = 0; p2 < (M + 1) / 2; ++p2) {
                const float4 xy = ms[2 * p2], zz = ms[2 * p2 + 1];
                const v2f dx = v2f{xy.x, xy.y} - QX, dy = v2f{xy.z, xy.w} - QY, dz = v2f{zz.x, zz.y} - QZ;
                const v2f d2 = __builtin_elementwise_fma(dy, dy, dx * dx) + dz * dz;
                mind2 = fminf(fminf(mind2, d2.x), d2.y);
                if (__builtin_amdgcn_ballot_w64(fminf(d2.x, d2.y) < MARK_D2) != 0ull) {
                    if (d2.x < MARK_D2) flags[2 * p2] = 1;
                    if (d2.y < MARK_D2) flags[2 * p2 + 1] = 1;
                }
            }
        }
    }
    if (stats && ln == 0 && do_nn) {
        atomicAdd(stats, (unsigned long long)n_exec);
        atomicAdd(stats + 1, (unsigned long long)nCB * n_tasks);
        atomicAdd(stats + 2, (unsigned long long)n_test);
    }
    phase_done();
    if constexpr (OPT) return;
    __syncthreads();
    phase_done();
    float loss = 0.f;
#pragma unroll
    for (int k = 0; k < MAXP / CT; ++k) loss += pl[tid + CT * k];
    red[tid] = loss;
    __syncthreads();
    for (int s = CT / 2; s > 0; s >>= 1) {
        if (tid < s) red[tid] += red[tid + s];
        __syncthreads();
    }
    const float loss_total = red[0];
    __syncthreads();
    red[tid] = mind2;
    __syncthreads();
    for (int s = CT / 2; s > 0; s >>= 1) {
        if (tid < s) red[tid] = fminf(red[tid], red[tid + s]);
        __syncthreads();
    }
    if (tid == 0) { loss_sum[n] = loss_total; min_dist[n] = red[0] == FLT_MAX ? FLT_MAX : sqrtf(red[0]); }
    if (tid < M) label[(size_t)n * M + tid] = flags[tid];
    phase_done();
    if (stats && tid == 0 && do_nn) atomicAdd(stats + 3, 1ull);
}

size_t contact_lds_bytes(int V) { return (size_t)ContactLds(V).total * sizeof(float4); }

int launch_contact(hipStream_t s, int64_t N, const float *verts, int V, const float *obj_points, int P, int32_t *porder,
                   const float *objR, const float *objT, const idf_correction_ctx *c, int B, float *markers, float *loss_sum,
                   float *min_dist, int32_t *label, float *o2h, int32_t *idx, unsigned long long *stats, int64_t nn_from, const PredArgs *pred = nullptr) {
    const int M = c->n_markers;
    const size_t lds = contact_lds_bytes(V);
    if (lds > 160 * 1024 - 16384 || P > MAXP) return IDF_E_INVAL;
    const bool ordered = c->vorder != nullptr;
    if (ordered != (c->faces_scan != nullptr) || ordered != (c->markers_scan != nullptr) || ordered != (c->adj_pair_scan != nullptr)) return IDF_E_INVAL;
    const int32_t *faces = ordered ? c->faces_scan : c->faces, *mpos = ordered ? c->markers_scan : c->markers_idx;
    if (porder) hipLaunchKernelGGL(corr_point_order_kernel, dim3((unsigned)B), dim3(1024), 0, s, obj_points, P, porder);
    if (pred) {
        const size_t lds2 = (pred->nclips > 0 && lds < idf_objproj_dev::OBJPROJ_LDS) ? idf_objproj_dev::OBJPROJ_LDS : lds;
        static std::atomic<uint64_t> lds_ok2{0};
        if (lds2 > 160 * 1024 - 2048) return IDF_E_INVAL;
        if (idf_opt_in_lds(reinterpret_cast<const void *>(corr_contact_kernel<false, true>), 160 * 1024 - 2048, lds_ok2) != IDF_OK) return IDF_E_LAUNCH;
        hipLaunchKernelGGL((corr_contact_kernel<false, true>), dim3((unsigned)(N + pred->nclips)), dim3(CT), lds2, s, verts, V, obj_points, P, porder, objR, objT, faces,
                           c->adj_ptr, c->adj_face, c->adj_corner, c->adj_pair_scan, c->vorder, c->vrank, mpos, M, B, markers, loss_sum, min_dist, label, o2h, idx,
                           stats, nn_from, nullptr, 0, *pred);
        return IDF_OK;
    }
    static std::atomic<uint64_t> lds_ok{0};
    if (idf_opt_in_lds(reinterpret_cast<const void *>(corr_contact_kernel<false>), 160 * 1024 - 16384, lds_ok) != IDF_OK) return IDF_E_LAUNCH;
    hipLaunchKernelGGL(corr_contact_kernel<false>, dim3((unsigned)N), dim3(CT), lds, s, verts, V, obj_points, P, porder, objR, objT, faces,
                       c->adj_ptr, c->adj_face, c->adj_corner, c->adj_pair_scan, c->vorder, c->vrank, mpos, M, B, markers, loss_sum, min_dist, label, o2h, idx,
                       stats, nn_from, nullptr, 0, PredArgs{});
    return IDF_OK;
}

__global__ __launch_bounds__(128) void corr_reduce_kernel(const float *__restrict__ loss_sum, const float *__restrict__ min_dist,
                                                          const int32_t *__restrict__ label, int B, int T, int past, int P, int M,
                                                          uint8_t *__restrict__ condition, int32_t *__restrict__ contact,
                                                          float *__restrict__ distance_out, float *__restrict__ loss_out) {
    extern __shared__ float fr[];
    const int b = blockIdx.x, tid = threadIdx.x;
    for (int t = tid; t < T; t += 128) {
        fr[t] = loss_sum[(size_t)t * B + b];
        fr[T + t] = min_dist[(size_t)t * B + b];
    }
    if (tid < M) {
        int c = 0;
#pragma unroll 16
        for (int t = past; t < T; ++t) c += label[((size_t)t * B + b) * M + tid];
        contact[(size_t)b * M + tid] = c;
    }
    __syncthreads();
    if (tid == 0) {
        float ls = 0.f, ds = 0.f;
        for (int t = past; t < T; ++t) ls += fr[t] / (float)P;
        for (int t = 0; t < T; ++t) ds += fr[T + t];
        const float loss = ls / (float)(T - past), dist = ds / (float)T;
        condition[b] = !((loss < 0.002f) && (dist < 0.02f));
        if (distance_out) distance_out[b] = dist;
        if (loss_out) loss_out[b] = loss;
    }
}

__global__ __launch_bounds__(256) void corr_blend_kernel(float *__restrict__ x0, const float *__restrict__ proj,
                                                         const uint8_t *__restrict__ condition, int B, int T, float a,
                                                         const float *__restrict__ a_table, const int64_t *__restrict__ a_state) {
    if (a_table) a = a_table[a_state[0] * 4 + 3];
    const int64_t i = (int64_t)blockIdx.x * 256 + threadIdx.x;
    if (i >= (int64_t)B * CTOK * T) return;
    const int b = (int)(i / (CTOK * T)), r = (int)(i - (int64_t)b * CTOK * T), c = r / T, t = r - c * T;
    if (!condition[b]) return;
    const float x = x0[i];
    const float other = c < 135 ? x : proj[((size_t)t * B + b) * 9 + (c - 135)];
    x0[i] = a * x + (1.0f - a) * other;
}

struct CorrWs {
    float *pose, *trans, *objR, *objT, *gt_angles, *gt_trans, *verts, *jtr, *markers, *loss_sum, *min_dist, *proj, *proj_keep;
    int32_t *label, *contact, *porder;
    uint8_t *condition;
    void *smpl_ws;
    size_t smpl_ws_bytes, total;
};

CorrWs carve(const idf_correction_ctx *c, int B, int T, void *ws) {
    const int64_t N = (int64_t)B * T;
    const int V = c->smpl->V, J = c->smpl->J, M = c->n_markers;
    char *p = reinterpret_cast<char *>(ws);
    size_t off = 0;
    auto take = [&](size_t bytes) { char *r = p ? p + off : nullptr; off += idf_align(bytes); return r; };
    CorrWs w;
    w.pose = (float *)take(N * 156 * 4);
    w.trans = (float *)take(N * 3 * 4);
    w.objR = (float *)take(N * 9 * 4);
    w.objT = (float *)take(N * 3 * 4);
    w.gt_angles = (float *)take(N * 6 * 4);
    w.gt_trans = (float *)take(N * 3 * 4);
    w.verts = (float *)take((size_t)N * V * 3 * 4);
    w.jtr = (float *)take((size_t)N * J * 3 * 4);
    w.markers = (float *)take((size_t)N * M * 3 * 4);
    w.loss_sum = (float *)take(N * 4);
    w.min_dist = (float *)take(N * 4);
    w.proj = (float *)take(N * 9 * 4);
    w.label = (int32_t *)take((size_t)N * M * 4);
    w.contact = (int32_t *)take((size_t)B * M * 4);
    w.condition = (uint8_t *)take(B);
    w.porder = (int32_t *)take((size_t)B * c->n_points * 4);
    w.proj_keep = (float *)take((size_t)B * idf_objproj_keep_floats() * 4);
    w.smpl_ws_bytes = interdiff_smpl_workspace_bytes(c->smpl, N);
    w.smpl_ws = take(w.smpl_ws_bytes);
    w.total = off;
    return w;
}


constexpr int NPATCH = MAXP / 64;
__global__ __launch_bounds__(256) void opt_patch_kernel(const float *__restrict__ pts, int P, const int32_t *__restrict__ porder, int frames_per_clip,
                                                        float4 *__restrict__ psort , float4 *__restrict__ pbox ) {
    const int64_t n = blockIdx.x;
    const int b = (int)(n / frames_per_clip), tid = threadIdx.x, lane = tid & 63, wave = tid >> 6;
    const float *pn = pts + (size_t)n * P * 3;
    for (int k = wave; k < NPATCH; k += 4) {
        const int sp = 64 * k + lane;
        float x = 3e18f, y = 3e18f, z = 3e18f;
        float lx = FLT_MAX, ly = FLT_MAX, lz = FLT_MAX, hx = -FLT_MAX, hy = -FLT_MAX, hz = -FLT_MAX;
        if (sp < P) {
            const int i = porder[(size_t)b * P + sp];
            x = pn[3 * i]; y = pn[3 * i + 1]; z = pn[3 * i + 2];
            lx = hx = x; ly = hy = y; lz = hz = z;
        }
        psort[(size_t)n * MAXP + sp] = make_float4(x, y, z, 0.f);
        lx = -wave_max(-lx); ly = -wave_max(-ly); lz = -wave_max(-lz);
        hx = wave_max(hx); hy = wave_max(hy); hz = wave_max(hz);
        if (lane == 0) {
            pbox[((size_t)n * NPATCH + k) * 2] = make_float4(lx, ly, lz, 0.f);
            pbox[((size_t)n * NPATCH + k) * 2 + 1] = make_float4(hx, hy, hz, 0.f);
        }
    }
}

__global__ __launch_bounds__(256) void opt_near_kernel(const float *__restrict__ verts, int V, int P, const float4 *__restrict__ psort,
                                                       const float4 *__restrict__ pbox, const int32_t *__restrict__ vorder,
                                                       int32_t *__restrict__ near) {
    __shared__ float4 ps[MAXP];
    __shared__ float4 bx[NPATCH * 2];
    const int64_t n = blockIdx.y;
    const int tid = threadIdx.x, pos = blockIdx.x * 256 + tid, vid = vorder[min(pos, V - 1)];
    for (int i = tid; i < MAXP; i += 256) ps[i] = psort[(size_t)n * MAXP + i];
    if (tid < NPATCH * 2) bx[tid] = pbox[(size_t)n * NPATCH * 2 + tid];
    const bool valid = pos < V;
    const float *vp = verts + ((size_t)n * V + vid) * 3;
    const float vx = vp[0], vy = vp[1], vz = vp[2];
    __syncthreads();
    const int npatch = (P + 63) / 64;
    bool hit = false;
    {
#pragma clang fp contract(off)
        const v2f VX = v2f{vx, vx}, VY = v2f{vy, vy}, VZ = v2f{vz, vz};
        for (int k = 0; k < npatch; ++k) {
            if (__builtin_amdgcn_ballot_w64(valid && !hit) == 0ull) break;
            const float4 lo = bx[2 * k], hi = bx[2 * k + 1];
            const float ex = fmaxf(fmaxf(lo.x - vx, vx - hi.x), 0.f), ey = fmaxf(fmaxf(lo.y - vy, vy - hi.y), 0.f), ez = fmaxf(fmaxf(lo.z - vz, vz - hi.z), 0.f);
            const float xx = ex * ex, yy = ey * ey, zz = ez * ez;
            if (__builtin_amdgcn_ballot_w64(valid && !hit && (xx + yy) + zz < 0.25f) == 0ull) continue;
            const float4 *pp = ps + 64 * k;
            for (int j0 = 0; j0 < 64; j0 += 16) {
#pragma unroll
                for (int j = j0; j < j0 + 16; j += 2) {
                    const float4 p = pp[j], q = pp[j + 1];
                    const v2f dx = v2f{p.x, q.x} - VX, dy = v2f{p.y, q.y} - VY, dz = v2f{p.z, q.z} - VZ;
                    const v2f d2 = (dx * dx + dy * dy) + dz * dz;
                    hit = hit || d2.x < 0.25f || d2.y < 0.25f;
                }
                if (__builtin_amdgcn_ballot_w64(valid && !hit) == 0ull) break;
            }
        }
    }
    if (valid) near[(size_t)n * V + vid] = hit ? 1 : 0;
}

}

int idf_point_order(hipStream_t s, const float *obj_points, int B, int P, int32_t *porder) {
    if (P > MAXP) return IDF_E_INVAL;
    hipLaunchKernelGGL(corr_point_order_kernel, dim3((unsigned)B), dim3(1024), 0, s, obj_points, P, porder);
    return IDF_OK;
}

int idf_nn_scan_opt(hipStream_t s, int64_t N, int frames_per_clip, const float *verts, int V, const float *pts_frame, const float *obj_points, int P,
                    const int32_t *porder, const idf_correction_ctx *c, int32_t *yidx) {
    const size_t lds = contact_lds_bytes(V);
    if (lds > 160 * 1024 - 16384 || P > MAXP || !c->vorder) return IDF_E_INVAL;
    const int B = (int)(N / frames_per_clip);
    static std::atomic<uint64_t> lds_ok{0};
    if (idf_opt_in_lds(reinterpret_cast<const void *>(corr_contact_kernel<true>), 160 * 1024 - 16384, lds_ok) != IDF_OK) return IDF_E_LAUNCH;
    hipLaunchKernelGGL(corr_contact_kernel<true>, dim3((unsigned)N, 2), dim3(CT), lds, s, verts, V, obj_points, P, porder, nullptr, nullptr, nullptr,
                       nullptr, nullptr, nullptr, nullptr, c->vorder, c->vrank, nullptr, 0, B, nullptr, nullptr, nullptr, nullptr, nullptr, yidx, nullptr, (int64_t)0,
                       pts_frame, frames_per_clip, PredArgs{});
    return IDF_OK;
}

int idf_near_mask_opt(hipStream_t s, int64_t N, int frames_per_clip, const float *verts, int V, const float *pts_frame, int P, const int32_t *porder,
                      const int32_t *vorder, float *psort, float *pbox, int32_t *near) {
    if (P > MAXP || !vorder) return IDF_E_INVAL;
    hipLaunchKernelGGL(opt_patch_kernel, dim3((unsigned)N), dim3(256), 0, s, pts_frame, P, porder, frames_per_clip, reinterpret_cast<float4 *>(psort),
                       reinterpret_cast<float4 *>(pbox));
    hipLaunchKernelGGL(opt_near_kernel, dim3((unsigned)idf_cdiv(V, 256), (unsigned)N), dim3(256), 0, s, verts, V, P, reinterpret_cast<const float4 *>(psort),
                       reinterpret_cast<const float4 *>(pbox), vorder, near);
    return IDF_OK;
}

namespace {

}

extern "C" size_t interdiff_correction_workspace_bytes(const idf_correction_ctx *c, int32_t B, int32_t T) {
    if (!c || !c->smpl || B <= 0 || T <= 0) return 0;
    return carve(c, B, T, nullptr).total;
}

static int correction_impl(const idf_correction_ctx *c, float *x0, const float *gt, const float *hand_pose,
                           const float *beta, const float *obj_points, int32_t B, int32_t T, float blend_t, const float *blend_table,
                           const int64_t *blend_state, uint8_t *condition, int32_t *contact, float *distance, float *loss, void *ws,
                           size_t ws_bytes, void *stream) {
    if (!c || !c->smpl || !c->objproj || !x0 || !gt || !hand_pose || !beta || !obj_points || !ws || B <= 0 || T <= 0) return IDF_E_INVAL;
    const int V = c->smpl->V, M = c->n_markers, P = c->n_points;
    if (c->smpl->J != 52 || c->smpl->n_betas != 10 || M > MAXM || M != c->objproj->P || P > MAXP || T != c->objproj->T ||
        c->past_len != c->objproj->past_len || c->past_len >= T)
        return IDF_E_INVAL;
    CorrWs w = carve(c, B, T, ws);
    if (ws_bytes < w.total) return IDF_E_NOMEM;
    hipStream_t s = idf_stream(stream);
    const int64_t N = (int64_t)B * T;
    const bool fused = (c->tune & 2) == 0 && idf_objproj_check(c->objproj) == IDF_OK;
    idf_prof_mark(IDF_K_CORR_PREPARE, s);
    hipLaunchKernelGGL(corr_prepare_kernel, dim3((unsigned)idf_cdiv(N * 24, 256)), dim3(256), 0, s, x0, gt, hand_pose, B, T, w.pose,
                       w.trans, w.objR, w.objT, w.gt_angles, w.gt_trans);
    int rc = interdiff_smpl_forward(c->smpl, w.pose, beta, w.trans, N, w.verts, w.jtr, nullptr, w.smpl_ws, w.smpl_ws_bytes, stream);
    if (rc) return rc;
    idf_prof_mark(IDF_K_CORR_CONTACT, s);
    PredArgs pred{};
    if (fused) {
        pred.op = *c->objproj;
        pred.obj_angles = w.gt_angles; pred.obj_trans = w.gt_trans;
        pred.markers_idx = c->markers_idx; pred.markers = w.markers; pred.keep = w.proj_keep;
        pred.nclips = B;
    }
    rc = launch_contact(s, N, w.verts, V, obj_points, P, w.porder, w.objR, w.objT, c, B, fused ? nullptr : w.markers, w.loss_sum, w.min_dist, w.label, nullptr,
                        nullptr, nullptr, (int64_t)c->past_len * B, &pred);
    if (rc) return rc;
    uint8_t *cond = condition ? condition : w.condition;
    int32_t *cont = contact ? contact : w.contact;
    idf_prof_mark(IDF_K_CORR_REDUCE, s);
    hipLaunchKernelGGL(corr_reduce_kernel, dim3(B), dim3(128), 2 * (size_t)T * sizeof(float), s, w.loss_sum, w.min_dist, w.label, B, T, c->past_len, P, M, cond,
                       cont, distance, loss);
    if (fused) {
        idf_prof_mark(IDF_K_OBJPROJ, s);
        rc = idf_objproj_pick(c->objproj, w.proj_keep, cont, B, w.proj, s);
    } else {
        rc = interdiff_objprojector_sample(c->objproj, w.gt_angles, w.gt_trans, w.markers, cont, B, w.proj, stream);
    }
    if (rc) return rc;
    idf_prof_mark(IDF_K_CORR_BLEND, s);
    hipLaunchKernelGGL(corr_blend_kernel, dim3((unsigned)idf_cdiv((int64_t)B * CTOK * T, 256)), dim3(256), 0, s, x0, w.proj, cond, B, T,
                       blend_t, blend_table, blend_state);
    idf_prof_mark(-1, s);
    IDF_CHECK_LAUNCH();
    return IDF_OK;
}

extern "C" int interdiff_correction(const idf_correction_ctx *c, float *x0, const float *gt, const float *hand_pose,
                                    const float *beta, const float *obj_points, int32_t B, int32_t T, float blend_t,
                                    uint8_t *condition, int32_t *contact, float *distance, float *loss, void *ws,
                                    size_t ws_bytes, void *stream) {
    return correction_impl(c, x0, gt, hand_pose, beta, obj_points, B, T, blend_t, nullptr, nullptr, condition, contact, distance, loss, ws, ws_bytes, stream);
}

extern "C" int interdiff_correction_dev(const idf_correction_ctx *c, float *x0, const float *gt, const float *hand_pose,
                                        const float *beta, const float *obj_points, int32_t B, int32_t T, const float *table,
                                        const int64_t *state, void *ws, size_t ws_bytes, void *stream) {
    if (!table || !state) return IDF_E_INVAL;
    return correction_impl(c, x0, gt, hand_pose, beta, obj_points, B, T, 0.f, table, state, nullptr, nullptr, nullptr, nullptr, ws, ws_bytes, stream);
}

namespace {

__global__ __launch_bounds__(256) void metrics_prepare_kernel(const float *__restrict__ obj_pred, int64_t N,
                                                              float *__restrict__ objR, float *__restrict__ objT) {
    const int64_t n = (int64_t)blockIdx.x * 256 + threadIdx.x;
    if (n >= N) return;
    float q[4], m[9];
    rot::axis_angle_to_quaternion(obj_pred + n * 6, q);
    rot::quaternion_to_matrix(q, m);
#pragma unroll
    for (int k = 0; k < 9; ++k) objR[n * 9 + k] = m[k];
#pragma unroll
    for (int k = 0; k < 3; ++k) objT[n * 3 + k] = obj_pred[n * 6 + 3 + k];
}

__device__ __forceinline__ float block_sum(float v, float *red) {
    red[threadIdx.x] = v;
    __syncthreads();
    for (int s = 128; s > 0; s >>= 1) {
        if (threadIdx.x < s) red[threadIdx.x] += red[threadIdx.x + s];
        __syncthreads();
    }
    const float r = red[0];
    __syncthreads();
    return r;
}

__global__ __launch_bounds__(256) void metrics_reduce_kernel(const float *__restrict__ obj_pred, const float *__restrict__ jtr,
                                                             const float *__restrict__ body_trans, const float *__restrict__ obj_gt,
                                                             const float *__restrict__ jtr_gt, const float *__restrict__ body_trans_gt,
                                                             const float *__restrict__ o2h, int B, int T, int J, int P,
                                                             float *__restrict__ out6) {
    __shared__ float red[256];
    const int b = blockIdx.x, tid = threadIdx.x;
    float g = 0.f, l = 0.f;
    for (int i = tid; i < T * J; i += 256) {
        const int t = i / J, j = i - t * J;
        const float *a = jtr + (((size_t)t * B + b) * J + j) * 3, *c = jtr_gt + (((size_t)t * B + b) * J + j) * 3;
        const float *a0 = jtr + ((size_t)t * B + b) * J * 3, *c0 = jtr_gt + ((size_t)t * B + b) * J * 3;
        const float dx = a[0] - c[0], dy = a[1] - c[1], dz = a[2] - c[2];
        g += sqrtf(dx * dx + dy * dy + dz * dz);
        const float ex = (a[0] - a0[0]) - (c[0] - c0[0]), ey = (a[1] - a0[1]) - (c[1] - c0[1]), ez = (a[2] - a0[2]) - (c[2] - c0[2]);
        l += sqrtf(ex * ex + ey * ey + ez * ez);
    }
    float bt = 0.f, ot = 0.f, rq = 0.f;
    for (int t = tid; t < T; t += 256) {
        const size_t n = (size_t)t * B + b;
        const float *x = body_trans + n * 3, *y = body_trans_gt + n * 3;
        bt += sqrtf((x[0] - y[0]) * (x[0] - y[0]) + (x[1] - y[1]) * (x[1] - y[1]) + (x[2] - y[2]) * (x[2] - y[2]));
        const float *p = obj_pred + n * 6, *q = obj_gt + n * 6;
        ot += sqrtf((p[3] - q[3]) * (p[3] - q[3]) + (p[4] - q[4]) * (p[4] - q[4]) + (p[5] - q[5]) * (p[5] - q[5]));
        float qa[4], qb[4];
        rot::axis_angle_to_quaternion(p, qa);
        rot::axis_angle_to_quaternion(q, qb);
        float e1 = 0.f, e2 = 0.f;
#pragma unroll
        for (int k = 0; k < 4; ++k) { e1 += fabsf(qa[k] - qb[k]); e2 += fabsf(qa[k] + qb[k]); }
        rq += fminf(e1, e2);
    }
    const float gs = block_sum(g, red), ls = block_sum(l, red), bs = block_sum(bt, red), os = block_sum(ot, red), rs = block_sum(rq, red);
    float pen = 0.f;
    for (int t = 0; t < T; ++t) {
        const float *row = o2h + ((size_t)t * B + b) * P;
        float c = 0.f;
        for (int i = tid; i < P; i += 256) c += row[i] < 0.f ? 1.f : 0.f;
        const float cs = block_sum(c, red);
        pen += cs / (float)P;
    }
    if (tid == 0) {
        out6[0 * B + b] = gs / (float)J / (float)T;
        out6[1 * B + b] = ls / (float)J / (float)T;
        out6[2 * B + b] = bs / (float)T;
        out6[3 * B + b] = os / (float)T;
        out6[4 * B + b] = rs / (float)T;
        out6[5 * B + b] = pen / (float)T;
    }
}

struct MetWs {
    float *objR, *objT, *o2h, *markers, *loss_sum, *min_dist;
    int32_t *label, *porder;
    size_t total;
};
MetWs carve_metrics(const idf_correction_ctx *c, int B, int T, void *ws) {
    const int64_t N = (int64_t)B * T;
    char *p = reinterpret_cast<char *>(ws);
    size_t off = 0;
    auto take = [&](size_t bytes) { char *r = p ? p + off : nullptr; off += idf_align(bytes); return r; };
    MetWs w;
    w.objR = (float *)take(N * 9 * 4);
    w.objT = (float *)take(N * 3 * 4);
    w.o2h = (float *)take((size_t)N * c->n_points * 4);
    w.markers = (float *)take((size_t)N * c->n_markers * 3 * 4);
    w.loss_sum = (float *)take(N * 4);
    w.min_dist = (float *)take(N * 4);
    w.label = (int32_t *)take((size_t)N * c->n_markers * 4);
    w.porder = (int32_t *)take((size_t)B * c->n_points * 4);
    w.total = off;
    return w;
}

}

extern "C" size_t interdiff_contact_nn_workspace_bytes(const idf_correction_ctx *c, int32_t B, int32_t T) {
    if (!c || B <= 0 || T <= 0) return 0;
    return carve_metrics(c, B, T, nullptr).total;
}

extern "C" int interdiff_contact_nn(const idf_correction_ctx *c, const float *verts, const float *obj_points, const float *objR,
                                    const float *objT, int32_t B, int32_t T, float *o2h, int32_t *idx, uint64_t *stats, void *ws,
                                    size_t ws_bytes, void *stream) {
    if (!c || !c->smpl || !verts || !obj_points || !objR || !objT || !ws || B <= 0 || T <= 0 || (!o2h && !idx)) return IDF_E_INVAL;
    if (c->n_markers > MAXM || c->n_points > MAXP) return IDF_E_INVAL;
    MetWs w = carve_metrics(c, B, T, ws);
    if (ws_bytes < w.total) return IDF_E_NOMEM;
    hipStream_t s = idf_stream(stream);
    if (stats && hipMemsetAsync(stats, 0, IDF_CONTACT_STATS * sizeof(uint64_t), s) != hipSuccess) return IDF_E_LAUNCH;
    const int rc = launch_contact(s, (int64_t)B * T, verts, c->smpl->V, obj_points, c->n_points, w.porder, objR, objT, c, B, w.markers, w.loss_sum,
                                  w.min_dist, w.label, o2h ? o2h : w.o2h, idx, reinterpret_cast<unsigned long long *>(stats), 0);
    if (rc) return rc;
    IDF_CHECK_LAUNCH();
    return IDF_OK;
}

extern "C" size_t interdiff_metrics_workspace_bytes(const idf_correction_ctx *c, int32_t B, int32_t T) {
    if (!c || B <= 0 || T <= 0) return 0;
    return carve_metrics(c, B, T, nullptr).total;
}

extern "C" int interdiff_metrics(const idf_correction_ctx *c, const float *obj_pred, const float *jtr, const float *body_trans,
                                 const float *obj_gt, const float *jtr_gt, const float *body_trans_gt, const float *verts,
                                 const float *obj_points, int32_t B, int32_t T, int32_t J, float *out6, void *ws, size_t ws_bytes,
                                 void *stream) {
    if (!c || !c->smpl || !obj_pred || !jtr || !body_trans || !obj_gt || !jtr_gt || !body_trans_gt || !verts || !obj_points || !out6 ||
        !ws || B <= 0 || T <= 0 || J <= 0)
        return IDF_E_INVAL;
    const int V = c->smpl->V, M = c->n_markers, P = c->n_points;
    if (M > MAXM || P > MAXP) return IDF_E_INVAL;
    MetWs w = carve_metrics(c, B, T, ws);
    if (ws_bytes < w.total) return IDF_E_NOMEM;
    hipStream_t s = idf_stream(stream);
    const int64_t N = (int64_t)B * T;
    idf_prof_mark(IDF_K_OTHER, s);
    hipLaunchKernelGGL(metrics_prepare_kernel, dim3((unsigned)idf_cdiv(N, 256)), dim3(256), 0, s, obj_pred, N, w.objR, w.objT);
    const int rc = launch_contact(s, N, verts, V, obj_points, P, w.porder, w.objR, w.objT, c, B, w.markers, w.loss_sum, w.min_dist, w.label, w.o2h,
                                  nullptr, nullptr, 0);
    if (rc) return rc;
    hipLaunchKernelGGL(metrics_reduce_kernel, dim3(B), dim3(256), 0, s, obj_pred, jtr, body_trans, obj_gt, jtr_gt, body_trans_gt, w.o2h, B,
                       T, J, P, out6);
    idf_prof_mark(-1, s);
    IDF_CHECK_LAUNCH();
    return IDF_OK;
}
```

interdiff_amd/csrc/smpl.hip:

```cpp
#include "common.h"
#include "rot_math.h"
#include <algorithm>

#ifndef IDF_SMPL_STAMP
#define IDF_SMPL_STAMP(i) do { } while (0)
#endif

namespace {

constexpr int MAXJ = 64;

__global__ __launch_bounds__(64) void smpl_pose_kernel(const idf_smpl_model m, const float *__restrict__ pose,
                                                       const float *__restrict__ betas, const float *__restrict__ trans,
                                                       float *__restrict__ feat, float *__restrict__ A,
                                                       float *__restrict__ jtr) {
    __shared__ float Rs[MAXJ * 9], Js[MAXJ * 3], Gs[MAXJ * 12];
    const int64_t n = blockIdx.x;
    const int j = threadIdx.x, J = m.J, nb = m.n_betas, KB = m.KB;
    const float *beta = betas + n * nb;
    if (j < J) {
        rot::rodrigues_smpl(pose + n * 3 * J + 3 * j, Rs + j * 9);
#pragma unroll
        for (int c = 0; c < 3; ++c) {
            float s = m.jt[j * 3 + c];
            const float *jsr = m.js + (size_t)(j * 3 + c) * nb;
            for (int k = 0; k < nb; ++k) s += jsr[k] * beta[k];
            Js[j * 3 + c] = s;
        }
    }
    float *f = feat + n * KB;
    if (j >= 1 && j < J) {
#pragma unroll
        for (int e = 0; e < 9; ++e) f[(j - 1) * 9 + e] = Rs[j * 9 + e] - ((e == 0 || e == 4 || e == 8) ? 1.0f : 0.0f);
    }
    const int base = 9 * (J - 1);
    for (int k = j; k < KB - base; k += 64) f[base + k] = k < nb ? beta[k] : (k == nb ? 1.0f : 0.0f);
    __syncthreads();
    if (j < 12) {
        const int r = j >> 2, c = j & 3;
        Gs[j] = c < 3 ? Rs[r * 3 + c] : Js[r];
    }
    __syncthreads();
    for (int i = 1; i < J; ++i) {
        const int p = m.parents[i];
        if (j < 12) {
            const int r = j >> 2, c = j & 3;
            const float *gp = Gs + p * 12 + r * 4;
            float v;
            if (c < 3)
                v = gp[0] * Rs[i * 9 + c] + gp[1] * Rs[i * 9 + 3 + c] + gp[2] * Rs[i * 9 + 6 + c];
            else
                v = gp[0] * (Js[i * 3] - Js[p * 3]) + gp[1] * (Js[i * 3 + 1] - Js[p * 3 + 1]) +
                    gp[2] * (Js[i * 3 + 2] - Js[p * 3 + 2]) + gp[3];
            Gs[i * 12 + j] = v;
        }
        __syncthreads();
    }
    if (j < J) {
        const float *g = Gs + j * 12;
        const float jx = Js[j * 3], jy = Js[j * 3 + 1], jz = Js[j * 3 + 2];
        float *a = A + ((size_t)n * J + j) * 12;
#pragma unroll
        for (int r = 0; r < 3; ++r) {
            a[r * 4 + 0] = g[r * 4 + 0];
            a[r * 4 + 1] = g[r * 4 + 1];
            a[r * 4 + 2] = g[r * 4 + 2];
            a[r * 4 + 3] = g[r * 4 + 3] - (g[r * 4] * jx + g[r * 4 + 1] * jy + g[r * 4 + 2] * jz);
            jtr[((size_t)n * J + j) * 3 + r] = g[r * 4 + 3] + trans[n * 3 + r];
        }
    }
}

constexpr int FT = 32, VT = 64, NTC = 3 * VT;
constexpr int BT = 256;
constexpr int FM = FT / 16;
constexpr int STS = NTC + 1;
constexpr int SF = 16;
constexpr int TBF = 10, TBV = 4;

template <int NG>
__global__ __launch_bounds__(BT) void smpl_blend_skin_kernel(const idf_smpl_model m, const float *__restrict__ feat,
                                                              const float *__restrict__ A, const float *__restrict__ trans,
                                                              int64_t N, float *__restrict__ verts,
                                                              float *__restrict__ v_posed) {
    extern __shared__ __attribute__((aligned(16))) float sm[];
    idf_args_now(m.V, m.J, m.S, m.blend, m.skin_idx, m.skin_w, feat, A, trans, N, verts, v_posed, gridDim.x);
    constexpr int KB = 16 * NG, nq = KB / 4;
    const int V = m.V, J = m.J, S = m.S;
    float *As = sm, *stage = sm;
    const int tid = threadIdx.x, lane = tid & 63, wave = (tid >> 6) & 3, fh = tid >> 8, li = lane & 15, kq = lane >> 4;
    const int nft = (int)((N + FT - 1) / FT), nvt = (V + VT - 1) / VT;
    const int nwg = gridDim.x, id = blockIdx.x;
    const int xq = nwg >> 3, xr = nwg & 7, xcd = id & 7;
    const int lid = (xcd < xr ? xcd * (xq + 1) : xr * (xq + 1) + (xcd - xr) * xq) + (id >> 3);
    const int blk = lid / (TBF * TBV), wi = lid - blk * (TBF * TBV);
    const int nvb = (nvt + TBV - 1) / TBV;
    const int ftile = blk / nvb * TBF + wi % TBF, vtile = blk % nvb * TBV + wi / TBF;
    if (ftile >= nft || vtile >= nvt) return;
    const int64_t f0 = (int64_t)ftile * FT;
    const int v0 = vtile * VT;
    IDF_SMPL_STAMP(0);

    {
        const uint32_t as_lds = idf_lds_addr(As);
        const int ncell = FT * nq;
        for (int i = wave; i * 64 < ncell; i += BT / 64) {
            const int p = min(i * 64 + lane, ncell - 1), row = p / nq, pos = p - row * nq;
            idf_dma16_v(feat + (size_t)min(f0 + row, N - 1) * KB + ((pos ^ ((row >> 1) & 7)) << 2), as_lds + (uint32_t)(i * 1024));
        }
    }
    const int vl = tid & 63, vme = v0 + vl;
    float sw[4];
    int so[4];
#pragma unroll
    for (int k = 0; k < 4; ++k) {
        const size_t e = (size_t)min(vme, V - 1) * S + min(k, S - 1);
        sw[k] = m.skin_w[e];
        so[k] = m.skin_idx[e] * 12;
    }
#pragma unroll
    for (int k = 0; k < 4; ++k) {
        const bool ok = k < S && vme < V;
        sw[k] = ok ? sw[k] : 0.f;
        so[k] = ok ? so[k] : 0;
    }
    asm volatile("s_waitcnt vmcnt(0)" ::: "memory");
    __syncthreads();
    IDF_SMPL_STAMP(1);

    const float *brow[3];
#pragma unroll
    for (int t = 0; t < 3; ++t) brow[t] = m.blend + ((size_t)((vtile * 4 + wave) * 3 + t) * NG * 64 + lane) * 4;
    f32x4 acc[FM][3];
#pragma unroll
    for (int i = 0; i < FM; ++i)
#pragma unroll
        for (int t = 0; t < 3; ++t) acc[i][t] = f32x4{0.f, 0.f, 0.f, 0.f};
    constexpr int PD = 3;
    float4 bq[PD + 1][3];
    auto ldg = [&](float4 (&dst)[3], int gi) {
#pragma unroll
        for (int t = 0; t < 3; ++t) dst[t] = *reinterpret_cast<const float4 *>(brow[t] + gi * 256);
    };
    auto mac = [&](const float4 (&bc)[3], int gi) {
#pragma unroll
        for (int i = 0; i < FM; ++i) {
            const int row = (fh * FM + i) * 16 + li;
            const float4 a = *reinterpret_cast<const float4 *>(As + row * KB + (((gi * 4 + kq) ^ ((row >> 1) & 7)) << 2));
#pragma unroll
            for (int t = 0; t < 3; ++t) acc[i][t] = __builtin_amdgcn_mfma_f32_16x16x4f32(a.x, bc[t].x, acc[i][t], 0, 0, 0);
#pragma unroll
            for (int t = 0; t < 3; ++t) acc[i][t] = __builtin_amdgcn_mfma_f32_16x16x4f32(a.y, bc[t].y, acc[i][t], 0, 0, 0);
#pragma unroll
            for (int t = 0; t < 3; ++t) acc[i][t] = __builtin_amdgcn_mfma_f32_16x16x4f32(a.z, bc[t].z, acc[i][t], 0, 0, 0);
#pragma unroll
            for (int t = 0; t < 3; ++t) acc[i][t] = __builtin_amdgcn_mfma_f32_16x16x4f32(a.w, bc[t].w, acc[i][t], 0, 0, 0);
        }
    };
#pragma unroll
    for (int g = 0; g < PD && g < NG; ++g) ldg(bq[g], g);
#pragma unroll
    for (int g = 0; g < NG; ++g) {
        if (g + PD < NG) ldg(bq[(g + PD) % (PD + 1)], g + PD);
        __builtin_amdgcn_sched_barrier(0);
        mac(bq[g % (PD + 1)], g);
        __builtin_amdgcn_sched_barrier(0);
    }
    __syncthreads();
    IDF_SMPL_STAMP(2);
#pragma unroll
    for (int i = 0; i < FM; ++i)
#pragma unroll
        for (int t = 0; t < 3; ++t)
#pragma unroll
            for (int r = 0; r < 4; ++r) stage[((fh * FM + i) * 16 + kq * 4 + r) * STS + (wave * 3 + t) * 16 + li] = acc[i][t][r];

    float *Asub = sm + ((FT * STS + 255) & ~255);
    float *ost = Asub + ((SF * J * 12 + 255) & ~255);
    float *trs = ost + SF * NTC;
    const int arow = J * 12;
    if (tid < FT * 3) trs[tid] = trans[min(f0 + tid / 3, N - 1) * 3 + tid % 3];
    for (int sub = 0; sub < FT / SF; ++sub) {
        const int64_t fs = f0 + sub * SF;
        if (fs >= N) break;
        __syncthreads();
        {
            const uint32_t asub_lds = idf_lds_addr(Asub);
            const float *src = idf_uniform_ptr(A + (size_t)fs * arow);
            for (int i = wave; i * 256 < SF * arow; i += BT / 64) idf_dma16_s(src + (size_t)i * 256, (uint32_t)(lane << 4), asub_lds + (uint32_t)(i * 1024));
            asm volatile("s_waitcnt vmcnt(0)" ::: "memory");
        }
        __syncthreads();
        IDF_SMPL_STAMP(3 + 3 * sub);
#pragma unroll
        for (int k = 0; k < SF * VT / BT; ++k) {
            const int f = (tid >> 6) + (BT / 64) * k, fr = sub * SF + f;
            const float px = stage[fr * STS + 3 * vl], py = stage[fr * STS + 3 * vl + 1], pz = stage[fr * STS + 3 * vl + 2];
            float4 t0 = make_float4(0.f, 0.f, 0.f, 0.f), t1 = t0, t2 = t0;
            const float *Af = Asub + f * arow;
#pragma unroll
            for (int b = 0; b < 4; ++b) {
                if (b < S) {
                    const float w = sw[b];
                    const float4 *a = reinterpret_cast<const float4 *>(Af + so[b]);
                    const float4 a0 = a[0], a1 = a[1], a2 = a[2];
                    t0.x = fmaf(w, a0.x, t0.x); t0.y = fmaf(w, a0.y, t0.y); t0.z = fmaf(w, a0.z, t0.z); t0.w = fmaf(w, a0.w, t0.w);
                    t1.x = fmaf(w, a1.x, t1.x); t1.y = fmaf(w, a1.y, t1.y); t1.z = fmaf(w, a1.z, t1.z); t1.w = fmaf(w, a1.w, t1.w);
                    t2.x = fmaf(w, a2.x, t2.x); t2.y = fmaf(w, a2.y, t2.y); t2.z = fmaf(w, a2.z, t2.z); t2.w = fmaf(w, a2.w, t2.w);
                }
            }
            float *o = ost + f * NTC + 3 * vl;
            o[0] = fmaf(t0.x, px, fmaf(t0.y, py, fmaf(t0.z, pz, t0.w))) + trs[fr * 3 + 0];
            o[1] = fmaf(t1.x, px, fmaf(t1.y, py, fmaf(t1.z, pz, t1.w))) + trs[fr * 3 + 1];
            o[2] = fmaf(t2.x, px, fmaf(t2.y, py, fmaf(t2.z, pz, t2.w))) + trs[fr * 3 + 2];
        }
        __syncthreads();
        IDF_SMPL_STAMP(4 + 3 * sub);
        const int nvalid = min(VT, V - v0) * 3;
        for (int idx = tid; idx < SF * (NTC / 2); idx += BT) {
            const int f = idx / (NTC / 2), c2 = (idx - f * (NTC / 2)) * 2;
            if (fs + f >= N || c2 >= nvalid) continue;
            const size_t go = ((size_t)(fs + f) * V + v0) * 3 + c2;
            *reinterpret_cast<float2 *>(verts + go) = *reinterpret_cast<const float2 *>(ost + f * NTC + c2);
            if (v_posed) *reinterpret_cast<float2 *>(v_posed + go) = make_float2(stage[(sub * SF + f) * STS + c2], stage[(sub * SF + f) * STS + c2 + 1]);
        }
        IDF_SMPL_STAMP(5 + 3 * sub);
    }
}

}

extern "C" size_t interdiff_smpl_workspace_bytes(const idf_smpl_model *m, int64_t N) {
    if (!m || N < 0) return 0;
    return idf_align((size_t)N * m->KB * sizeof(float)) + idf_align(((size_t)N + SF) * m->J * 12 * sizeof(float));
}

extern "C" int interdiff_smpl_forward(const idf_smpl_model *m, const float *pose, const float *betas, const float *trans,
                                      int64_t N, float *verts, float *jtr, float *v_posed, void *ws, size_t ws_bytes,
                                      void *stream) {
    if (!m || !pose || !betas || !trans || !verts || !jtr || !ws || N < 0) return IDF_E_INVAL;
    if (m->J < 1 || m->J > MAXJ || m->KB % 16 != 0 || m->KB < 9 * (m->J - 1) + m->n_betas + 1 || m->S < 1) return IDF_E_INVAL;
    if (ws_bytes < interdiff_smpl_workspace_bytes(m, N)) return IDF_E_NOMEM;
    if (N == 0) return IDF_OK;
    hipStream_t s = idf_stream(stream);
    float *feat = reinterpret_cast<float *>(ws);
    float *A = reinterpret_cast<float *>(reinterpret_cast<char *>(ws) + idf_align((size_t)N * m->KB * sizeof(float)));
    idf_prof_mark(IDF_K_SMPL_POSE, s);
    hipLaunchKernelGGL(smpl_pose_kernel, dim3((unsigned)N), dim3(64), 0, s, *m, pose, betas, trans, feat, A, jtr);
    const size_t lds = std::max((size_t)FT * m->KB, (size_t)((FT * STS + 255) & ~255) + ((SF * m->J * 12 + 255) & ~255) + (size_t)SF * NTC + FT * 3) * sizeof(float);
    if (lds > 150 * 1024 || m->KB % 32 != 0 || (m->V * 3) % 2 != 0 || m->S > 4) return IDF_E_INVAL;
    if (m->KB != 480) return IDF_E_INVAL;
    static std::atomic<uint64_t> lds_ok{0};
    if (lds > 64 * 1024 && idf_opt_in_lds(reinterpret_cast<const void *>(smpl_blend_skin_kernel<30>), 150 * 1024, lds_ok) != IDF_OK) return IDF_E_LAUNCH;
    idf_prof_mark(IDF_K_SMPL_BLEND_SKIN, s);
    const unsigned nwg_launch = (unsigned)(idf_cdiv(idf_cdiv(N, FT), TBF) * idf_cdiv(idf_cdiv(m->V, VT), TBV) * TBF * TBV);
    hipLaunchKernelGGL(smpl_blend_skin_kernel<30>, dim3(nwg_launch), dim3(BT), lds, s, *m,
                       feat, A, trans, N, verts, v_posed);
    idf_prof_mark(-1, s);
    IDF_CHECK_LAUNCH();
    return IDF_OK;
}
```

interdiff_amd/diffusion.py:

```python
import itertools
import math
import os
import numpy as np
import torch
from . import _lib
from . import graph_sampler


def get_named_beta_schedule(schedule_name, num_diffusion_timesteps, scale_betas=1.):
    n = num_diffusion_timesteps
    if schedule_name == 'linear':
        scale = scale_betas * 1000 / n
        return np.linspace(scale * 0.0001, scale * 0.02, n, dtype=np.float64)
    if schedule_name == 'cosine':
        abar = lambda t: math.cos((t + 0.008) / 1.008 * math.pi / 2) ** 2
        return np.array([min(1 - abar((i + 1) / n) / abar(i / n), 0.999) for i in range(n)], dtype=np.float64)
    raise NotImplementedError('unknown beta schedule: %s' % schedule_name)


GRAPH_BLOCKS = (49, 7, 1)
SPLIT_MAX_BATCH = int(os.environ.get('INTERDIFF_SPLIT_MAX_BATCH', 128))
N_CHAINS = int(os.environ.get('INTERDIFF_CHAINS', 2))
MAX_GRAPH_SHAPES = 8
_UID = itertools.count(1)


def fresh_seed():
    return int(torch.randint(0, 2 ** 62, (1,), dtype=torch.int64).item())


def mask_operands(mask, gt, like):
    if mask is None or gt is None:
        return None, None
    assert like.shape == mask.shape == gt.shape
    return (mask if mask.dtype == torch.uint8 else mask.view(torch.uint8)).contiguous(), gt.contiguous()


def inpaint(x, gt, mask_u8):
    _lib.check(_lib.load().interdiff_inpaint(_lib.dptr(x, torch.float32), _lib.dptr(gt, torch.float32), _lib.dptr(mask_u8), x.numel(), _lib.stream()), 'inpaint')


def seeded_state(t_start, seed, elem0):
    return torch.tensor([t_start, 0, int(seed) & 0x7FFFFFFFFFFFFFFF, 0, 0, 0, elem0, 0], dtype=torch.int64)


def space_timesteps(num_timesteps, section_counts):
    if isinstance(section_counts, str):
        if section_counts.startswith('ddim'):
            want = int(section_counts[len('ddim'):])
            for stride in range(1, num_timesteps):
                if len(range(0, num_timesteps, stride)) == want:
                    return set(range(0, num_timesteps, stride))
            raise ValueError('cannot create exactly %d steps with an integer stride' % num_timesteps)
        section_counts = [int(c) for c in section_counts.split(',')]
    size_per, extra = divmod(num_timesteps, len(section_counts))
    start, kept = 0, []
    for k, count in enumerate(section_counts):
        size = size_per + (1 if k < extra else 0)
        if size < count:
            raise ValueError('cannot divide section of %d steps into %d' % (size, count))
        stride = 1 if count <= 1 else (size - 1) / (count - 1)
        kept += [start + round(cur) for cur in _strided(stride, count)]
        start += size
    return set(kept)


def _strided(stride, count):
    cur = 0.0
    for _ in range(count):
        yield cur
        cur += stride


def ddim_coefficients(alphas_cumprod, alphas_cumprod_prev, eta):
    ab, abp = np.asarray(alphas_cumprod, np.float64), np.asarray(alphas_cumprod_prev, np.float64)
    sigma = float(eta) * np.sqrt((1.0 - abp) / (1.0 - ab)) * np.sqrt(1.0 - ab / abp)
    k = np.sqrt(np.maximum(1.0 - abp - sigma ** 2, 0.0)) / np.sqrt(1.0 / ab - 1.0)
    return np.sqrt(abp) - k, k * np.sqrt(1.0 / ab), sigma


class GaussianDiffusion:

    def __init__(self, betas):
        betas = np.array(betas, dtype=np.float64)
        assert betas.ndim == 1 and (betas > 0).all() and (betas <= 1).all()
        self.betas = betas
        self.num_timesteps = int(betas.shape[0])
        alphas = 1.0 - betas
        self.alphas_cumprod = np.cumprod(alphas, axis=0)
        self.alphas_cumprod_prev = np.append(1.0, self.alphas_cumprod[:-1])
        self.posterior_variance = betas * (1.0 - self.alphas_cumprod_prev) / (1.0 - self.alphas_cumprod)
        self.posterior_log_variance_clipped = np.log(np.append(self.posterior_variance[1], self.posterior_variance[1:]))
        self.posterior_mean_coef1 = betas * np.sqrt(self.alphas_cumprod_prev) / (1.0 - self.alphas_cumprod)
        self.posterior_mean_coef2 = (1.0 - self.alphas_cumprod_prev) * np.sqrt(alphas) / (1.0 - self.alphas_cumprod)
        self._c1 = self.posterior_mean_coef1.astype(np.float32)
        self._c2 = self.posterior_mean_coef2.astype(np.float32)
        self._sigma = np.exp(np.float32(0.5) * self.posterior_log_variance_clipped.astype(np.float32)).astype(np.float32)
        self.sqrt_alphas_cumprod = np.sqrt(self.alphas_cumprod)
        self.sqrt_one_minus_alphas_cumprod = np.sqrt(1.0 - self.alphas_cumprod)
        self.timestep_map = list(range(self.num_timesteps))
        self.original_num_steps = self.num_timesteps
        self.identity_tmap_is_null = True
        self._t_cache = {}
        self._tables = {}
        self._rows_cache = {}
        self._tmaps = {}
        self._q_tables = {}
        self.fuse_plain_step = True
        self.chain_plain_steps = os.environ.get('INTERDIFF_CHAIN_STEPS', '1') != '0'
        self.split_chains = True
        self.split_min_rows = None
        self._uid = next(_UID)

    @property
    def is_respaced(self):
        return self.timestep_map != list(range(self.num_timesteps))

    def _timesteps(self, B, device, loop_side=False):
        key = (B, str(device), bool(loop_side) and self.is_respaced)
        if key not in self._t_cache:
            vals = torch.tensor(self.timestep_map, dtype=torch.int64) if not key[2] and self.is_respaced else torch.arange(self.num_timesteps, dtype=torch.int64)
            self._t_cache[key] = vals.to(device)[:, None].repeat(1, B).contiguous()
        return self._t_cache[key]

    def _tmap(self, device):
        if not self.is_respaced and self.identity_tmap_is_null:
            return None
        key = str(device)
        if key not in self._tmaps:
            self._tmaps[key] = torch.tensor(self.timestep_map, dtype=torch.int64).to(device)
        return self._tmaps[key]

    def _rows(self, sampler=('ddpm',)):
        if sampler not in self._rows_cache:
            if sampler[0] == 'ddpm':
                c1, c2, sig = self._c1, self._c2, self._sigma.copy()
            else:
                c1, c2, sig = (v.astype(np.float32) for v in ddim_coefficients(self.alphas_cumprod, self.alphas_cumprod_prev, sampler[1]))
            sig[0] = 0.0
            blend = (np.arange(self.num_timesteps, dtype=np.float32) / np.float32(1000)).astype(np.float32)
            self._rows_cache[sampler] = np.ascontiguousarray(np.stack([c1, c2, sig, blend], axis=1).astype(np.float32))
        return self._rows_cache[sampler]

    def _table(self, device, sampler=('ddpm',)):
        key = (str(device), sampler)
        if key not in self._tables:
            self._tables[key] = torch.from_numpy(self._rows(sampler)).to(device)
        return self._tables[key]

    def _step(self, model, img, x0_buf, i, it, t, model_kwargs, denoised_fn, noise_i, seed, elem0=0, rows_kw={}, t_hook=None, rows=None):
        lib = _lib.load()
        y = model_kwargs.get('y', {})
        x0 = model(img, t, **model_kwargs, **rows_kw)
        mu8, gc = mask_operands(y.get('inpainting_mask'), y.get('inpainted_motion'), x0)
        if mu8 is not None:
            inpaint(x0, gc, mu8)
        if denoised_fn is not None:
            x0 = denoised_fn(x0, t if t_hook is None else t_hook, model_kwargs)
        c1, c2, sigma = (float(v) for v in (self._rows() if rows is None else rows)[i, :3])
        _lib.check(lib.interdiff_posterior_step_at(_lib.dptr(img, torch.float32), _lib.dptr(x0, torch.float32),
                                                   _lib.dptr(noise_i, torch.float32, allow_none=True), img.numel(),
                                                   c1, c2, sigma, seed, it, elem0, _lib.stream()),
                   'posterior_step')
        return x0

    def p_sample_loop(self, model, shape, noise=None, clip_denoised=True, denoised_fn=None, cond_fn=None, model_kwargs=None,
                      device=None, progress=False, skip_timesteps=0, init_image=None, randomize_class=False,
                      cond_fn_with_grad=False, dump_steps=None, const_noise=False, step_noise=None, seed=None, n_steps=None,
                      use_graph=True, first_t=None, shard=None):
        return self._sample_loop(('ddpm',), model, shape, noise, clip_denoised, denoised_fn, cond_fn, model_kwargs, device, skip_timesteps,
                                 init_image, randomize_class, cond_fn_with_grad, dump_steps, const_noise, step_noise, seed, n_steps, use_graph,
                                 first_t, shard)

    def ddim_sample_loop(self, model, shape, noise=None, clip_denoised=True, denoised_fn=None, cond_fn=None, model_kwargs=None,
                         device=None, progress=False, eta=0.0, skip_timesteps=0, init_image=None, randomize_class=False,
                         cond_fn_with_grad=False, dump_steps=None, const_noise=False, step_noise=None, seed=None, n_steps=None,
                         use_graph=True, first_t=None, shard=None):
        return self._sample_loop(('ddim', float(eta)), model, shape, noise, clip_denoised, denoised_fn, cond_fn, model_kwargs, device,
                                 skip_timesteps, init_image, randomize_class, cond_fn_with_grad, dump_steps, const_noise, step_noise, seed,
                                 n_steps, use_graph, first_t, shard)

    def _sample_loop(self, sampler, model, shape, noise, clip_denoised, denoised_fn, cond_fn, model_kwargs, device, skip_timesteps, init_image,
                     randomize_class, cond_fn_with_grad, dump_steps, const_noise, step_noise, seed, n_steps, use_graph, first_t, shard):
        if clip_denoised:
            raise NotImplementedError('clip_denoised=True is not used on the eval path (eval_smpl_short.py:153)')
        if cond_fn is not None or skip_timesteps or init_image is not None or randomize_class or cond_fn_with_grad or const_noise:
            raise NotImplementedError('only noise=, denoised_fn=, model_kwargs=, dump_steps= are live (SURVEY.md §8(b))')
        if model_kwargs is None:
            model_kwargs = {}
        if seed is None:
            seed = fresh_seed()
        if device is None:
            device = next(model.parameters()).device
        assert isinstance(shape, (tuple, list))
        if shard is not None:
            shard = (int(shard[0]), int(shard[1]))
            if not 0 <= shard[0] <= shard[0] + shape[0] <= shard[1]:
                raise ValueError('shard=(first_clip, total_clips) must contain this batch of %d clips' % shape[0])
        first, total = (0, shape[0]) if shard is None else shard
        per_clip = int(np.prod(shape[1:]))
        elem0 = first * per_clip
        if shard is not None and elem0 % 4:
            raise ValueError('a shard must start at a multiple of 4 elements (C * T = %d per clip)' % per_clip)
        if noise is not None:
            img = noise.clone().contiguous().float()
        else:
            img = torch.empty(*shape, dtype=torch.float32, device=device)
            _lib.check(_lib.load().interdiff_randn_at(_lib.dptr(img), img.numel(), seed, 0xFFFFFFFF, elem0, _lib.stream()), 'randn')
            y = model_kwargs.get('y', {})
            mu8, gc = mask_operands(y.get('inpainting_mask'), y.get('inpainted_motion'), img) if sampler[0] == 'ddpm' else (None, None)
            if mu8 is not None:
                inpaint(img, gc, mu8)
        t_first = self.num_timesteps - 1 if first_t is None else int(first_t)
        if not 0 <= t_first < self.num_timesteps:
            raise ValueError('first_t outside the schedule')
        todo = t_first + 1 if n_steps is None else min(int(n_steps), t_first + 1)
        if (step_noise is None and use_graph and getattr(model, 'graph_safe', False) and img.is_cuda
                and 'cond' in model_kwargs.get('y', {}) and os.environ.get('INTERDIFF_NO_GRAPH') != '1'):
            return graph_sampler.sample(self, model, img, model_kwargs, denoised_fn, seed, todo, dump_steps, t_first, shard, sampler)
        rows_kw = {'batch_rows': total * shape[-1]} if shard is not None and getattr(model, 'accepts_batch_rows', False) else {}
        ts, ts_hook, rows = self._timesteps(shape[0], device), self._timesteps(shape[0], device, loop_side=True), self._rows(sampler)
        dump = []
        cond = model_kwargs.get('y', {}).get('cond') if isinstance(model_kwargs.get('y', None), dict) else None
        if cond is not None and hasattr(model, 'prepare_memory'):
            model.prepare_memory(cond)
        for it, i in enumerate(range(t_first, t_first - todo, -1)):
            t, th = ts[i], ts_hook[i]
            t.host_value = th.host_value = i
            if step_noise is None:
                nz = None
            elif callable(step_noise):
                nz = step_noise(it, img).contiguous()
            else:
                nz = step_noise[it]
            self._step(model, img, None, i, it, t, model_kwargs, denoised_fn, nz, seed, elem0, rows_kw, th, rows)
            if dump_steps is not None and it in dump_steps:
                dump.append(img.clone())
        return dump if dump_steps is not None else img

    def sample_timesteps(self, B, device, generator=None):
        gdev = generator.device if generator is not None else device
        t = torch.randint(0, self.num_timesteps, (B,), dtype=torch.int64, device=gdev, generator=generator).to(device)
        return t, torch.ones(B, dtype=torch.float32, device=device)

    def q_sample(self, x_start, t, noise=None, seed=None, inpainted_motion=None, inpainting_mask=None, elem0=0):
        lib = _lib.load()
        x0 = x_start.contiguous()
        if x0.dtype != torch.float32:
            raise ValueError('x_start must be float32')
        B = x0.shape[0]
        if tuple(t.shape) != (B,):
            raise ValueError('t must be [B]')
        if not t.is_cuda:
            if int(t.min()) < 0 or int(t.max()) >= self.num_timesteps:
                raise ValueError('t outside the schedule')
            t = t.to(x0.device)
        key = str(x0.device)
        if key not in self._q_tables:
            self._q_tables[key] = tuple(torch.from_numpy(v.astype(np.float32)).to(x0.device) for v in (self.sqrt_alphas_cumprod, self.sqrt_one_minus_alphas_cumprod))
        sa, s1 = self._q_tables[key]
        if (inpainted_motion is None) != (inpainting_mask is None):
            raise ValueError('inpainted_motion and inpainting_mask go together')
        mu8, gc = mask_operands(inpainting_mask, inpainted_motion, x0)
        if noise is not None:
            assert noise.shape == x0.shape
            noise = noise.contiguous()
        elif seed is None:
            seed = fresh_seed()
        x_t = torch.empty_like(x0)
        _lib.check(lib.interdiff_q_sample(_lib.dptr(x_t), _lib.dptr(x0), _lib.dptr(noise, torch.float32, allow_none=True),
                                          _lib.dptr(t.contiguous(), torch.int64), _lib.dptr(sa), _lib.dptr(s1), self.num_timesteps,
                                          _lib.dptr(gc, torch.float32, allow_none=True), _lib.dptr(mu8, allow_none=True), B, x0.numel() // B,
                                          int(seed or 0) & 0xFFFFFFFFFFFFFFFF, int(elem0), _lib.stream()), 'q_sample')
        return x_t

    def training_losses(self, model, x_start, t, model_kwargs=None, noise=None, seed=None):
        if model_kwargs is None:
            model_kwargs = {}
        y = model_kwargs.get('y', {})
        both = 'inpainting_mask' in y and 'inpainted_motion' in y
        x_t = self.q_sample(x_start, t, noise=noise, seed=seed, inpainted_motion=y['inpainted_motion'] if both else None,
                            inpainting_mask=y['inpainting_mask'] if both else None)
        t = t.to(x_t.device)
        if self.is_respaced:
            t = torch.tensor(self.timestep_map, dtype=torch.int64, device=x_t.device)[t]
        model_output = model(x_t, t, **model_kwargs)
        assert model_output.shape == x_start.shape
        return model_output, x_start


def sample_loop(diffusion, model, shape, sampler='ddpm', eta=0.0, **kw):
    if sampler == 'ddpm':
        return diffusion.p_sample_loop(model, shape, **kw)
    if sampler == 'ddim':
        return diffusion.ddim_sample_loop(model, shape, eta=eta, **kw)
    raise ValueError("sampler must be 'ddpm' or 'ddim'")


class SpacedDiffusion(GaussianDiffusion):

    def __init__(self, use_timesteps, betas, rescale_timesteps=False):
        if rescale_timesteps:
            raise NotImplementedError('rescale_timesteps=True is not built (the reference configuration is False: model/diffusion_smpl.py:258)')
        base = GaussianDiffusion(betas)
        self.use_timesteps = set(use_timesteps)
        last, new_betas, tmap = 1.0, [], []
        for i, ac in enumerate(base.alphas_cumprod):
            if i in self.use_timesteps:
                new_betas.append(1 - ac / last)
                last = ac
                tmap.append(i)
        super().__init__(np.array(new_betas))
        self.timestep_map, self.original_num_steps, self.rescale_timesteps = tmap, len(base.betas), False


def create_gaussian_diffusion(noise_schedule='cosine', diffusion_steps=1000, timestep_respacing=''):
    betas = get_named_beta_schedule(noise_schedule, diffusion_steps, 1.)
    if not timestep_respacing:
        timestep_respacing = [diffusion_steps]
    return SpacedDiffusion(space_timesteps(diffusion_steps, timestep_respacing), betas)
```

interdiff_amd/graph_sampler.py:

```python
import os
import torch
from . import _lib, diffusion

HOOK_KEYS = ('hand_pose', 'beta', 'obj_points')


def plan_steps(t_start, todo, active, dump_steps, fuse_hook):
    blocks = diffusion.GRAPH_BLOCKS
    dumps = () if dump_steps is None else dump_steps
    ops, i, it, end = [], t_start, 0, t_start - todo
    while i > end:
        if active(i):
            ops.append(('hook', 0) if fuse_hook else ('eager_hook',))
            k = 1
        else:
            run = 1
            while i - run > end and not active(i - run) and (it + run - 1) not in dumps:
                run += 1
            k = next(b for b in blocks if b <= run)
            if fuse_hook and k == run and i - run > end and active(i - run) and (it + k - 1) not in dumps:
                ops.append(('hook', k))
                k += 1
            else:
                ops.append(('plain', k))
        i -= k
        it += k
        if (it - 1) in dumps:
            ops.append(('dump', it - 1))
    return ops


def capture(enqueue, *args):
    g = torch.cuda.CUDAGraph()
    with torch.cuda.graph(g):
        enqueue(*args)
    return g


def posterior_update(x, x0, gt, mask, table, state, ts, tmap=None):
    _lib.check(_lib.load().interdiff_posterior_step_dev_map(_lib.dptr(x), _lib.dptr(x0), _lib.dptr(gt, allow_none=True), _lib.dptr(mask, allow_none=True),
                                                            x.numel(), _lib.dptr(table), _lib.dptr(tmap, torch.int64, allow_none=True), _lib.dptr(state),
                                                            _lib.dptr(ts), ts.numel(), _lib.stream()),
               'posterior_step_dev')


class Chain:

    def __init__(self, model, entry, sl, own_state):
        dev, h, mem_len = entry.x.device, sl.stop - sl.start, entry.cond.shape[0]
        self.sl = sl
        self.x, self.ts = entry.x[sl], entry.ts[sl]
        self.gt = None if entry.gt is None else entry.gt[sl]
        self.mask = None if entry.mask is None else entry.mask[sl]
        self.kwargs = {} if entry.zpo is None else {'zero_pose_obj': entry.zpo[sl]}
        self.state = torch.zeros(8, dtype=torch.int64, device=dev) if own_state else entry.state
        self.cond = torch.empty(mem_len, h, entry.cond.shape[2], device=dev)
        self.memctx = torch.empty(model.memctx_floats(h, mem_len), dtype=torch.float32, device=dev)
        self.ws = torch.empty(model.workspace_bytes(h, entry.x.shape[-1]), dtype=torch.uint8, device=dev)
        self.stream = torch.cuda.Stream(dev)


class HookBuffers:

    def __init__(self, hook, entry, y, shapes):
        B, T = entry.x.shape[0], entry.x.shape[-1]
        self.shapes = shapes
        self.ws = hook.workspace_for(B, T)
        self.y = {k: torch.empty(y[k].shape, dtype=torch.float32, device=entry.x.device) for k in HOOK_KEYS}
        self.y['inpainted_motion'] = entry.gt if entry.gt is not None else torch.empty_like(entry.x)
        self.fresh = True


class Entry:

    def __init__(self, img, cond, has_mask, zpo):
        dev = img.device
        self.x, self.x0 = torch.zeros_like(img), torch.empty_like(img)
        self.ts = torch.zeros(img.shape[0], dtype=torch.int64, device=dev)
        self.state = torch.zeros(8, dtype=torch.int64, device=dev)
        self.cond = torch.empty_like(cond, memory_format=torch.contiguous_format)
        self.gt = torch.empty_like(img) if has_mask else None
        self.mask = torch.empty(img.shape, dtype=torch.uint8, device=dev) if has_mask else None
        self.zpo = None if zpo is None else torch.empty(zpo.shape, dtype=torch.float32, device=dev)
        self.kwargs = {'y': {'cond': self.cond}}
        if zpo is not None:
            self.kwargs['zero_pose_obj'] = self.zpo
        self.graphs = {}
        self.chains = []
        self.hooks = {}
        self.chain_steps = None
        self.pool_keys = ()

    @staticmethod
    def of(model, key, img, cond, has_mask, zpo):
        cache = model.__dict__.setdefault('_graph_cache', {})
        entry = cache.get(key)
        if entry is not None:
            return entry, False
        entry = Entry(img, cond, has_mask, zpo)
        if len(cache) >= diffusion.MAX_GRAPH_SHAPES:
            evicted = list(cache.values())
            cache.clear()
            for old in evicted:
                model.forget_shape_buffers(old.pool_keys)
        cache[key] = entry
        return entry, True

    def load(self, cond, zpo, gt, mask):
        self.cond.copy_(cond)
        if zpo is not None:
            self.zpo.copy_(zpo)
        if mask is not None:
            self.gt.copy_(gt)
            self.mask.copy_(mask)

    def warm_up(self, model, table, rows, tmap=None):
        model(self.x, self.ts, out=self.x0, **self.kwargs, batch_rows=rows)
        if model.supports_forward_step:
            t0 = min(2, table.shape[0] - 1)
            x, ts, state = self.x.clone(), self.ts.clone(), diffusion.seeded_state(t0, 1, 0).to(self.x.device)
            model.forward_step(x, ts, table, state, gt=self.gt, mask=self.mask, tmap=tmap, **self.kwargs, batch_rows=rows)
            if model.step_chaining:
                state.copy_(diffusion.seeded_state(t0, 1, 0))
                ts.copy_(self.ts)
                model.forward_step(x, ts, table, state, gt=self.gt, mask=self.mask, tmap=tmap, embed_next=True, **self.kwargs, batch_rows=rows)
                model.forward_step(x, ts, table, state, gt=self.gt, mask=self.mask, tmap=tmap, embed_ready=True, **self.kwargs, batch_rows=rows)
        torch.cuda.synchronize(self.x.device)

    def split_into_chains(self, model, n):
        B = self.x.shape[0]
        for c in range(n):
            start = c * (B // n) + min(c, B % n)
            self.chains.append(Chain(model, self, slice(start, start + B // n + (1 if c < B % n else 0)), own_state=c > 0))

    def hook_buffers(self, hook, y, table):
        shapes = tuple(tuple(y[k].shape) for k in HOOK_KEYS)
        hk = self.hooks.get(hook._uid)
        if hk is None or hk.shapes != shapes:
            hk = self.hooks[hook._uid] = HookBuffers(hook, self, y, shapes)
            for stale in [gk for gk in self.graphs if isinstance(gk, tuple) and gk[0] == 'hook' and gk[1] == hook._uid]:
                del self.graphs[stale]
        for k in HOOK_KEYS + (() if self.gt is not None else ('inpainted_motion',)):
            hk.y[k].copy_(y[k])
        if hk.fresh:
            hook.apply_dev(hk.y['inpainted_motion'].clone(), table, torch.zeros(8, dtype=torch.int64, device=self.x.device), hk.y, hk.ws)
            torch.cuda.synchronize(self.x.device)
            hk.fresh = False
        return hk


def hook_capturable(hook, y):
    return (hook is not None and getattr(hook, 'graph_capturable', False) and getattr(hook, 'debug', None) is None
            and getattr(hook, 'is_active', None) is not None and all(k in y for k in ('inpainted_motion',) + HOOK_KEYS)
            and os.environ.get('INTERDIFF_EAGER_HOOK') != '1')


def hook_gate(hook):
    if hook is None:
        return lambda t: False
    return getattr(hook, 'is_active', None) or (lambda t: True)


class Run:

    def __init__(self, model, entry, table, rows, fused, split, hook, hk, tmap=None):
        self.model, self.entry, self.table, self.rows, self.tmap = model, entry, table, rows, tmap
        self.fused, self.split, self.hook, self.hk = fused, split, hook, hk

    def enqueue_forward(self):
        st = self.entry
        self.model(st.x, st.ts, out=st.x0, **st.kwargs, batch_rows=self.rows)

    def enqueue_plain(self, k):
        st, model = self.entry, self.model
        links = [dict(embed_ready=i > 0, embed_next=i + 1 < k) if st.chain_steps else {} for i in range(k)]
        if self.split:
            cur = torch.cuda.current_stream()
            for ch in st.chains:
                ch.stream.wait_stream(cur)
                with torch.cuda.stream(ch.stream):
                    for link in links:
                        model.forward_step(ch.x, ch.ts, self.table, ch.state, gt=ch.gt, mask=ch.mask, tmap=self.tmap, memctx=ch.memctx, ws=ch.ws, batch_rows=self.rows, **link, **ch.kwargs)
            for ch in st.chains:
                cur.wait_stream(ch.stream)
        elif self.fused:
            for link in links:
                model.forward_step(st.x, st.ts, self.table, st.state, gt=st.gt, mask=st.mask, tmap=self.tmap, **link, **st.kwargs, batch_rows=self.rows)
        else:
            for _ in links:
                self.enqueue_forward()
                posterior_update(st.x, st.x0, st.gt, st.mask, self.table, st.state, st.ts, self.tmap)

    def finish_hook_step(self, x0):
        st = self.entry
        posterior_update(st.x, x0, None, None, self.table, st.state, st.ts, self.tmap)
        if self.split:
            for ch in st.chains[1:]:
                ch.state[:6].copy_(st.state[:6])

    def enqueue_hook_block(self, k):
        st = self.entry
        if k:
            self.enqueue_plain(k)
        self.enqueue_forward()
        if st.mask is not None:
            diffusion.inpaint(st.x0, st.gt, st.mask)
        self.hook.apply_dev(st.x0, self.table, st.state, self.hk.y, self.hk.ws)
        self.finish_hook_step(st.x0)

    def graph(self, key, enqueue, *args):
        graphs = self.entry.graphs
        if key not in graphs:
            graphs[key] = capture(enqueue, *args)
        return graphs[key]

    def plain_block(self, k):
        return self.graph((k, self.fused, self.split), self.enqueue_plain, k)

    def hook_block(self, k):
        return self.graph(('hook', self.hook._uid, k, self.fused, self.split), self.enqueue_hook_block, k)

    def eager_hook_step(self, t, model_kwargs):
        st = self.entry
        self.graph('fwd', self.enqueue_forward).replay()
        if st.mask is not None:
            diffusion.inpaint(st.x0, st.gt, st.mask)
        self.finish_hook_step(self.hook(st.x0, t, model_kwargs).contiguous())

    def play(self, plan, t_start, ts_all, model_kwargs):
        st, dump, i = self.entry, [], t_start
        for op in plan:
            if op[0] == 'plain':
                self.plain_block(op[1]).replay()
                i -= op[1]
            elif op[0] == 'hook':
                self.hook_block(op[1]).replay()
                i -= op[1] + 1
            elif op[0] == 'eager_hook':
                t = ts_all[i]
                t.host_value = i
                self.eager_hook_step(t, model_kwargs)
                i -= 1
            else:
                dump.append(st.x.clone())
        return dump


def sample(diff, model, img, model_kwargs, hook, seed, todo, dump_steps, t_start, shard=None, sampler=('ddpm',)):
    y = model_kwargs.get('y', {})
    B, T, dev = img.shape[0], img.shape[-1], img.device
    first, total = (0, B) if shard is None else shard
    per_clip = img.numel() // B
    elem0 = first * per_clip
    rows = total * T
    table, tmap = diff._table(dev, sampler), diff._tmap(dev)
    mask, gt = diffusion.mask_operands(y.get('inpainting_mask'), y.get('inpainted_motion'), img)
    cond, zpo = y['cond'], model_kwargs.get('zero_pose_obj')
    key = (diff._uid, tuple(img.shape), mask is not None, tuple(cond.shape), model.ffn_graph_key(rows)) + (() if sampler == ('ddpm',) and tmap is None else (sampler, tmap is not None))
    if zpo is not None:
        key += (tuple(zpo.shape),)
    st, fresh = Entry.of(model, key, img, cond, mask is not None, zpo)
    st.load(cond, zpo, gt, mask)
    pools_before = model.shape_buffer_keys() if fresh else None
    model.prepare_memory(st.cond)
    if fresh:
        st.warm_up(model, table, rows, tmap)
        st.pool_keys = model.shape_buffer_keys() - pools_before

    fused = diff.fuse_plain_step and model.supports_forward_step
    nch = diffusion.N_CHAINS
    split = (fused and diff.split_chains and nch > 1 and 2 * nch <= B <= diffusion.SPLIT_MAX_BATCH
             and B * T > (model.one_chain_max_rows() if diff.split_min_rows is None else diff.split_min_rows))
    if split:
        if not st.chains:
            st.split_into_chains(model, nch)
        for ch in st.chains:
            ch.cond.copy_(st.cond[:, ch.sl])
            model.prepare_memory(ch.cond, into=ch.memctx)
    chain_steps = diff.chain_plain_steps and fused and model.step_chaining
    if st.chain_steps != chain_steps:
        st.graphs.clear()
        st.chain_steps = chain_steps
    fuse_hook = hook_capturable(hook, y)
    run = Run(model, st, table, rows, fused, split, hook, st.hook_buffers(hook, y, table) if fuse_hook else None, tmap)

    st.x.copy_(img)
    st.state.copy_(diffusion.seeded_state(t_start, seed, elem0))
    if split:
        for ch in st.chains[1:]:
            ch.state.copy_(diffusion.seeded_state(t_start, seed, elem0 + ch.sl.start * per_clip))
    st.ts.fill_(diff.timestep_map[t_start])
    dump = run.play(plan_steps(t_start, todo, hook_gate(hook), dump_steps, fuse_hook), t_start, diff._timesteps(B, dev, loop_side=True), model_kwargs)
    return dump if dump_steps is not None else st.x.clone()
```

Measured before the change: 7.157 million.

## Precompute per-sample SMPL blend base and point order; hint contact NN scans

Adds a per-sample preparation step for the correction hook. Before the denoising loop it computes the SMPL shape-blend base and the object point ordering once, and the per-step correction reuses them, with ready flags letting kernels skip recomputation. The contact nearest-neighbour scan also stores the previous step's best vertex per point as a 16-bit hint and uses it to tighten the initial search bound. This removes repeated work across diffusion steps, at the cost of extra workspace, new entry points and state that is only valid within a single sample.

```diff
diff --git a/include/interdiff_hip.h b/include/interdiff_hip.h
--- a/include/interdiff_hip.h
+++ b/include/interdiff_hip.h
@@ -37,6 +37,11 @@
 int interdiff_smpl_forward(const idf_smpl_model *m, const float *pose, const float *betas,
                            const float *trans, int64_t N, float *verts, float *jtr,
                            float *v_posed, void *ws, size_t ws_bytes, void *stream);
+
+size_t interdiff_smpl_blend_base_bytes(const idf_smpl_model *m, int64_t N);
+int interdiff_smpl_blend_base(const idf_smpl_model *m, const float *pose, const float *betas, int64_t N, float *base, void *ws, size_t ws_bytes, void *stream);
+int interdiff_smpl_forward_based(const idf_smpl_model *m, const float *pose, const float *betas, const float *trans, int64_t N, float *verts, float *jtr,
+                                 float *v_posed, float *base, void *ws, size_t ws_bytes, void *stream);
 
 int interdiff_vertex_normals(const float *verts, int64_t N, int32_t V, const int32_t *faces,
                              const int32_t *adj_ptr, const int32_t *adj_face,
@@ -199,11 +204,22 @@
                              const float *beta, const float *obj_points, int32_t B, int32_t T, const float *table,
                              const int64_t *state, void *ws, size_t ws_bytes, void *stream);
 
+int interdiff_correction_begin_sample(const idf_correction_ctx *c, const float *hand_pose, const float *beta, const float *obj_points, int32_t B,
+                                      int32_t T, void *ws, size_t ws_bytes, void *stream);
+int interdiff_correction_prepared(const idf_correction_ctx *c, float *x0, const float *gt, const float *hand_pose, const float *beta,
+                                  const float *obj_points, int32_t B, int32_t T, float blend_t, const float *table, const int64_t *state,
+                                  uint8_t *condition, int32_t *contact, float *distance, float *loss, uint64_t *stats, void *ws, size_t ws_bytes,
+                                  void *stream);
+
 #define IDF_CONTACT_STATS 12
 size_t interdiff_contact_nn_workspace_bytes(const idf_correction_ctx *c, int32_t B, int32_t T);
 int interdiff_contact_nn(const idf_correction_ctx *c, const float *verts, const float *obj_points, const float *objR,
                          const float *objT, int32_t B, int32_t T, float *o2h, int32_t *idx, uint64_t *stats,
                          void *ws, size_t ws_bytes, void *stream);
+
+int interdiff_contact_nn_hinted(const idf_correction_ctx *c, const float *verts, const float *obj_points, const float *objR,
+                                const float *objT, int32_t B, int32_t T, float *o2h, int32_t *idx, uint64_t *stats, uint16_t *hints,
+                                void *ws, size_t ws_bytes, void *stream);
 
 size_t interdiff_metrics_workspace_bytes(const idf_correction_ctx *c, int32_t B, int32_t T);
 int interdiff_metrics(const idf_correction_ctx *c, const float *obj_pred, const float *jtr,
diff --git a/interdiff_amd/_lib.py b/interdiff_amd/_lib.py
--- a/interdiff_amd/_lib.py
+++ b/interdiff_amd/_lib.py
@@ -107,6 +107,9 @@
     'interdiff_rotation_6d_to_axis_angle': (C.c_int, [vp, vp, i64, vp]),
     'interdiff_smpl_workspace_bytes': (sz, [C.POINTER(SmplModel), i64]),
     'interdiff_smpl_forward': (C.c_int, [C.POINTER(SmplModel), vp, vp, vp, i64, vp, vp, vp, vp, sz, vp]),
+    'interdiff_smpl_blend_base_bytes': (sz, [C.POINTER(SmplModel), i64]),
+    'interdiff_smpl_blend_base': (C.c_int, [C.POINTER(SmplModel), vp, vp, i64, vp, vp, sz, vp]),
+    'interdiff_smpl_forward_based': (C.c_int, [C.POINTER(SmplModel), vp, vp, vp, i64, vp, vp, vp, vp, vp, sz, vp]),
     'interdiff_vertex_normals': (C.c_int, [vp, i64, i32, vp, vp, vp, vp, vp, vp]),
     'interdiff_nn_argmin': (C.c_int, [vp, i32, vp, i32, i64, vp, vp]),
     'interdiff_point2point_signed': (C.c_int, [vp, i32, vp, i32, i64, vp, vp, vp, vp, vp, vp, vp, vp, vp]),
@@ -140,6 +143,9 @@
     'interdiff_correction': (C.c_int, [C.POINTER(CorrectionCtx), vp, vp, vp, vp, vp, i32, i32, f32,
                                        vp, vp, vp, vp, vp, sz, vp]),
     'interdiff_correction_dev': (C.c_int, [C.POINTER(CorrectionCtx), vp, vp, vp, vp, vp, i32, i32, vp, vp, vp, sz, vp]),
+    'interdiff_correction_begin_sample': (C.c_int, [C.POINTER(CorrectionCtx), vp, vp, vp, i32, i32, vp, sz, vp]),
+    'interdiff_correction_prepared': (C.c_int, [C.POINTER(CorrectionCtx), vp, vp, vp, vp, vp, i32, i32, f32, vp, vp, vp, vp, vp, vp, vp, vp, sz, vp]),
+    'interdiff_contact_nn_hinted': (C.c_int, [C.POINTER(CorrectionCtx), vp, vp, vp, vp, i32, i32, vp, vp, vp, vp, vp, sz, vp]),
     'interdiff_metrics_workspace_bytes': (sz, [C.POINTER(CorrectionCtx), i32, i32]),
     'interdiff_metrics': (C.c_int, [C.POINTER(CorrectionCtx), vp, vp, vp, vp, vp, vp, vp, vp, i32, i32, i32,
                                     vp, vp, sz, vp]),
diff --git a/interdiff_amd/correction.py b/interdiff_amd/correction.py
--- a/interdiff_amd/correction.py
+++ b/interdiff_amd/correction.py
@@ -44,6 +44,7 @@
         ctx.tune = 0
         self.ctx = ctx
         self._ws = {}
+        self._prepared = None
         self.debug = None
         self._uid = next(_UID)
 
@@ -52,10 +53,31 @@
     def workspace_for(self, B, T):
         return torch.empty(self.lib.interdiff_correction_workspace_bytes(C.byref(self.ctx), B, T), dtype=torch.uint8, device=self.device)
 
-    def apply_dev(self, x, table, state, y, ws):
+    def begin_sample(self, y, B, T, ws=None):
+        if y['obj_points'].shape[1] != self.ctx.n_points:
+            raise ValueError('obj_points must have %d points' % self.ctx.n_points)
+        own = ws is None
+        if own:
+            ws = self._workspace(B, T)
+        hp, beta, pts = (y[k].contiguous().float() for k in ('hand_pose', 'beta', 'obj_points'))
+        _lib.check(self.lib.interdiff_correction_begin_sample(C.byref(self.ctx), _lib.dptr(hp), _lib.dptr(beta), _lib.dptr(pts), B, T,
+                                                              _lib.dptr(ws), ws.numel(), _lib.stream()), 'correction_begin_sample')
+        if own:
+            self._prepared = ws
+
+    def end_sample(self):
+        self._prepared = None
+
+    def apply_dev(self, x, table, state, y, ws, prepared=False):
         B, _, Cc, T = x.shape
         if y['obj_points'].shape[1] != self.ctx.n_points:
             raise ValueError('obj_points must have %d points' % self.ctx.n_points)
+        if prepared:
+            _lib.check(self.lib.interdiff_correction_prepared(C.byref(self.ctx), _lib.dptr(x, torch.float32), _lib.dptr(y['inpainted_motion'], torch.float32),
+                                                              _lib.dptr(y['hand_pose'], torch.float32), _lib.dptr(y['beta'], torch.float32),
+                                                              _lib.dptr(y['obj_points'], torch.float32), B, T, 0.0, _lib.dptr(table), _lib.dptr(state),
+                                                              None, None, None, None, None, _lib.dptr(ws), ws.numel(), _lib.stream()), 'correction_prepared')
+            return x
         _lib.check(self.lib.interdiff_correction_dev(C.byref(self.ctx), _lib.dptr(x, torch.float32), _lib.dptr(y['inpainted_motion'], torch.float32),
                                                      _lib.dptr(y['hand_pose'], torch.float32), _lib.dptr(y['beta'], torch.float32),
                                                      _lib.dptr(y['obj_points'], torch.float32), B, T, _lib.dptr(table), _lib.dptr(state),
@@ -90,6 +112,15 @@
             dbg = [torch.empty(B, dtype=torch.uint8, device=self.device), torch.empty(B, len(MARKERS67), dtype=torch.int32, device=self.device),
                    torch.empty(B, device=self.device), torch.empty(B, device=self.device)]
         blend_t = float(np.float32(t0) / np.float32(1000))
+        if ws is self._prepared:
+            stats = torch.zeros(12, dtype=torch.int64, device=self.device) if self.debug is not None else None
+            _lib.check(self.lib.interdiff_correction_prepared(C.byref(self.ctx), _lib.dptr(x, torch.float32), _lib.dptr(gt, torch.float32),
+                                                              _lib.dptr(hp), _lib.dptr(beta), _lib.dptr(pts), B, T, blend_t, None, None,
+                                                              *[_lib.dptr(d, allow_none=True) for d in dbg], _lib.dptr(stats, allow_none=True),
+                                                              _lib.dptr(ws), ws.numel(), _lib.stream()), 'correction_prepared')
+            if self.debug is not None:
+                self.debug.update(condition=dbg[0], contact=dbg[1], distance=dbg[2], loss=dbg[3], scan_stats=stats)
+            return x
         _lib.check(self.lib.interdiff_correction(C.byref(self.ctx), _lib.dptr(x, torch.float32), _lib.dptr(gt, torch.float32),
                                                  _lib.dptr(hp), _lib.dptr(beta), _lib.dptr(pts), B, T, blend_t,
                                                  *[_lib.dptr(d, allow_none=True) for d in dbg], _lib.dptr(ws), ws.numel(),
@@ -98,7 +129,7 @@
             self.debug.update(condition=dbg[0], contact=dbg[1], distance=dbg[2], loss=dbg[3])
         return x
 
-    def contact_nn(self, verts, obj_points, objR, objT, want_stats=False):
+    def contact_nn(self, verts, obj_points, objR, objT, want_stats=False, hints=None):
         T, B = verts.shape[:2]
         P = self.ctx.n_points
         o2h = torch.empty(T, B, P, device=self.device)
@@ -109,8 +140,15 @@
         if ws is None or ws.numel() < need:
             ws = self._nn_ws = torch.empty(need, dtype=torch.uint8, device=self.device)
         v, pts, R_, t_ = (a.contiguous().float() for a in (verts, obj_points, objR, objT))
-        _lib.check(self.lib.interdiff_contact_nn(C.byref(self.ctx), _lib.dptr(v), _lib.dptr(pts), _lib.dptr(R_), _lib.dptr(t_), B, T, _lib.dptr(o2h),
-                                                 _lib.dptr(idx), _lib.dptr(stats, allow_none=True), _lib.dptr(ws), ws.numel(), _lib.stream()), 'contact_nn')
+        if hints is not None:
+            if hints.element_size() != 2 or tuple(hints.shape) != (T, B, P):
+                raise ValueError('hints must be 16-bit [T, B, P]')
+            _lib.check(self.lib.interdiff_contact_nn_hinted(C.byref(self.ctx), _lib.dptr(v), _lib.dptr(pts), _lib.dptr(R_), _lib.dptr(t_), B, T, _lib.dptr(o2h),
+                                                            _lib.dptr(idx), _lib.dptr(stats, allow_none=True), _lib.dptr(hints), _lib.dptr(ws), ws.numel(),
+                                                            _lib.stream()), 'contact_nn_hinted')
+        else:
+            _lib.check(self.lib.interdiff_contact_nn(C.byref(self.ctx), _lib.dptr(v), _lib.dptr(pts), _lib.dptr(R_), _lib.dptr(t_), B, T, _lib.dptr(o2h),
+                                                     _lib.dptr(idx), _lib.dptr(stats, allow_none=True), _lib.dptr(ws), ws.numel(), _lib.stream()), 'contact_nn')
         return (o2h, idx, tuple(int(x) for x in stats.cpu())) if want_stats else (o2h, idx)
 
     def is_active(self, t0):
diff --git a/interdiff_amd/csrc/correction.hip b/interdiff_amd/csrc/correction.hip
--- a/interdiff_amd/csrc/correction.hip
+++ b/interdiff_amd/csrc/correction.hip
@@ -63,9 +63,11 @@
 }
 
 constexpr int MAXP = 2048;
-__global__ __launch_bounds__(1024) void corr_point_order_kernel(const float *__restrict__ obj_points, int P, int32_t *__restrict__ porder) {
+__global__ __launch_bounds__(1024) void corr_point_order_kernel(const float *__restrict__ obj_points, int P, int32_t *__restrict__ porder,
+                                                                const uint32_t *__restrict__ ready = nullptr, uint32_t ready_want = 0) {
     __shared__ unsigned long long keys[MAXP];
     __shared__ float red[6][1024];
+    if (ready && *ready == ready_want) return;
     const int b = blockIdx.x, tid = threadIdx.x;
     const float *op = obj_points + (size_t)b * P * 3;
     float p[2][3];
@@ -205,7 +207,8 @@
                                                           unsigned long long *__restrict__ stats ,
                                                           int64_t nn_from ,
                                                           const float *__restrict__ pts_frame , int frames_per_clip ,
-                                                          const PredArgs pred) {
+                                                          const PredArgs pred,
+                                                          unsigned short *hints = nullptr ) {
     extern __shared__ __attribute__((aligned(16))) float4 vs[];
     if constexpr (WITH_PRED) {
         if ((int)blockIdx.x < pred.nclips) {
@@ -368,6 +371,8 @@
         const bool valid = i >= 0;
         float px = 0.f, py = 0.f, pz = 0.f;
         if (valid) { px = op[3 * i]; py = op[3 * i + 1]; pz = op[3 * i + 2]; }
+        int hint = 0xFFFF;
+        if constexpr (!OPT) { if (hints && valid && do_nn) hint = hints[(size_t)n * P + sp]; }
         const float qx = OPT ? px : (px * R[0] + py * R[1] + pz * R[2]) + tr[0];
         const float qy = OPT ? py : (px * R[3] + py * R[4] + pz * R[5]) + tr[1];
         const float qz = OPT ? pz : (px * R[6] + py * R[7] + pz * R[8]) + tr[2];
@@ -385,14 +390,48 @@
             };
             constexpr float SCAN_M = 1.000003814697265625f, SCAN_ABS = 1e-37f;
             float seed = FLT_MAX;
-            for (int k = 0; k < (L.nSeed + 1) / 2; k += 4) {
-                float4 xy[4]; float2 zz[4];
-#pragma unroll
-                for (int u = 0; u < 4; ++u) { xy[u] = sd[2 * min(k + u, (L.nSeed + 1) / 2 - 1)]; zz[u] = *reinterpret_cast<const float2 *>(&sd[2 * min(k + u, (L.nSeed + 1) / 2 - 1) + 1]); }
-#pragma unroll
-                for (int u = 0; u < 4; ++u) {
-                    const v2f a2 = pair_a2(xy[u], zz[u]);
-                    seed = fminf(fminf(seed, a2.x), a2.y);
+            if (OPT || !vorder) {
+                for (int k = 0; k < (L.nSeed + 1) / 2; k += 4) {
+                    float4 xy[4]; float2 zz[4];
+#pragma unroll
+                    for (int u = 0; u < 4; ++u) { xy[u] = sd[2 * min(k + u, (L.nSeed + 1) / 2 - 1)]; zz[u] = *reinterpret_cast<const float2 *>(&sd[2 * min(k + u, (L.nSeed + 1) / 2 - 1) + 1]); }
+#pragma unroll
+                    for (int u = 0; u < 4; ++u) {
+                        const v2f a2 = pair_a2(xy[u], zz[u]);
+                        seed = fminf(fminf(seed, a2.x), a2.y);
+                    }
+                }
+            } else {
+                int kb = 0;
+                for (int k = 0; k < (L.nSeed + 1) / 2; k += 4) {
+                    float4 xy[4]; float2 zz[4];
+#pragma unroll
+                    for (int u = 0; u < 4; ++u) { xy[u] = sd[2 * min(k + u, (L.nSeed + 1) / 2 - 1)]; zz[u] = *reinterpret_cast<const float2 *>(&sd[2 * min(k + u, (L.nSeed + 1) / 2 - 1) + 1]); }
+#pragma unroll
+                    for (int u = 0; u < 4; ++u) {
+                        const v2f a2 = pair_a2(xy[u], zz[u]);
+                        const float m2 = fminf(a2.x, a2.y);
+                        if (m2 < seed) { seed = m2; kb = min(k + u, (L.nSeed + 1) / 2 - 1); }
+                    }
+                }
+                {
+                    const v2f a2 = pair_a2(sd[2 * kb], *reinterpret_cast<const float2 *>(&sd[2 * kb + 1]));
+                    const int cbs = min((2 * kb + (a2.y < a2.x ? 1 : 0)) * SEED_STRIDE, nCB - 1);
+                    const float4 *bp = vs + cbs * CB;
+                    float4 xy[CB / 2]; float2 zz[CB / 2];
+#pragma unroll
+                    for (int u = 0; u < CB / 2; ++u) { xy[u] = bp[2 * u]; zz[u] = *reinterpret_cast<const float2 *>(&bp[2 * u + 1]); }
+#pragma unroll
+                    for (int u = 0; u < CB / 2; ++u) {
+                        const v2f b2 = pair_a2(xy[u], zz[u]);
+                        seed = fminf(fminf(seed, b2.x), b2.y);
+                    }
+                }
+                if (hints) {
+                    const int hp = min(hint, V - 1);
+                    const v2f a2 = pair_a2(vs[2 * (hp >> 1)], *reinterpret_cast<const float2 *>(&vs[2 * (hp >> 1) + 1]));
+                    const float ah = (hp & 1) ? a2.y : a2.x;
+                    seed = hint < V ? fminf(seed, ah) : seed;
                 }
             }
             float thr = __builtin_fmaf(seed, SCAN_M, SCAN_ABS);
@@ -469,6 +508,7 @@
                 for (int pr = 0; pr < (V + 1) / 2; ++pr) resolve_pair(pr);
             }
             pos = min(pos, V - 1);
+            if constexpr (!OPT) { if (hints && valid) hints[(size_t)n * P + sp] = (unsigned short)pos; }
             if (org == 0x7fffffff) org = vorder ? vorder[pos] : pos;
             if constexpr (OPT) {
                 if (valid) idx_out[(size_t)n * P + i] = org;
@@ -561,14 +601,16 @@
 
 int launch_contact(hipStream_t s, int64_t N, const float *verts, int V, const float *obj_points, int P, int32_t *porder,
                    const float *objR, const float *objT, const idf_correction_ctx *c, int B, float *markers, float *loss_sum,
-                   float *min_dist, int32_t *label, float *o2h, int32_t *idx, unsigned long long *stats, int64_t nn_from, const PredArgs *pred = nullptr) {
+                   float *min_dist, int32_t *label, float *o2h, int32_t *idx, unsigned long long *stats, int64_t nn_from, const PredArgs *pred = nullptr,
+                   unsigned short *hints = nullptr , const uint32_t *order_ready = nullptr, uint32_t order_ready_want = 0 ) {
     const int M = c->n_markers;
     const size_t lds = contact_lds_bytes(V);
     if (lds > 160 * 1024 - 16384 || P > MAXP) return IDF_E_INVAL;
     const bool ordered = c->vorder != nullptr;
     if (ordered != (c->faces_scan != nullptr) || ordered != (c->markers_scan != nullptr) || ordered != (c->adj_pair_scan != nullptr)) return IDF_E_INVAL;
     const int32_t *faces = ordered ? c->faces_scan : c->faces, *mpos = ordered ? c->markers_scan : c->markers_idx;
-    if (porder) hipLaunchKernelGGL(corr_point_order_kernel, dim3((unsigned)B), dim3(1024), 0, s, obj_points, P, porder);
+    if (porder) hipLaunchKernelGGL(corr_point_order_kernel, dim3((unsigned)B), dim3(1024), 0, s, obj_points, P, porder, order_ready, order_ready_want);
+    if (!ordered || V >= 0xFFFF) hints = nullptr;
     if (pred) {
         const size_t lds2 = (pred->nclips > 0 && lds < idf_objproj_dev::OBJPROJ_LDS) ? idf_objproj_dev::OBJPROJ_LDS : lds;
         static std::atomic<uint64_t> lds_ok2{0};
@@ -576,14 +618,14 @@
         if (idf_opt_in_lds(reinterpret_cast<const void *>(corr_contact_kernel<false, true>), 160 * 1024 - 2048, lds_ok2) != IDF_OK) return IDF_E_LAUNCH;
         hipLaunchKernelGGL((corr_contact_kernel<false, true>), dim3((unsigned)(N + pred->nclips)), dim3(CT), lds2, s, verts, V, obj_points, P, porder, objR, objT, faces,
                            c->adj_ptr, c->adj_face, c->adj_corner, c->adj_pair_scan, c->vorder, c->vrank, mpos, M, B, markers, loss_sum, min_dist, label, o2h, idx,
-                           stats, nn_from, nullptr, 0, *pred);
+                           stats, nn_from, nullptr, 0, *pred, hints);
         return IDF_OK;
     }
     static std::atomic<uint64_t> lds_ok{0};
     if (idf_opt_in_lds(reinterpret_cast<const void *>(corr_contact_kernel<false>), 160 * 1024 - 16384, lds_ok) != IDF_OK) return IDF_E_LAUNCH;
     hipLaunchKernelGGL(corr_contact_kernel<false>, dim3((unsigned)N), dim3(CT), lds, s, verts, V, obj_points, P, porder, objR, objT, faces,
                        c->adj_ptr, c->adj_face, c->adj_corner, c->adj_pair_scan, c->vorder, c->vrank, mpos, M, B, markers, loss_sum, min_dist, label, o2h, idx,
-                       stats, nn_from, nullptr, 0, PredArgs{});
+                       stats, nn_from, nullptr, 0, PredArgs{}, hints);
     return IDF_OK;
 }
 
@@ -634,7 +676,27 @@
     uint8_t *condition;
     void *smpl_ws;
     size_t smpl_ws_bytes, total;
+    unsigned short *hints;
+    uint32_t *ready;
+    float *base;
 };
+
+uint32_t sample_ready_value(const idf_correction_ctx *c, int B, int T) {
+    return 0xc0227e00u ^ ((uint32_t)B * 2654435761u) ^ ((uint32_t)T * 40503u) ^ ((uint32_t)c->n_points << 8);
+}
+
+__global__ __launch_bounds__(256) void corr_begin_kernel(uint4 *__restrict__ hints16, size_t n16, uint32_t *__restrict__ ready, uint32_t value) {
+    for (size_t i = (size_t)blockIdx.x * 256 + threadIdx.x; i < n16; i += (size_t)gridDim.x * 256) hints16[i] = make_uint4(~0u, ~0u, ~0u, ~0u);
+    if (blockIdx.x == 0 && threadIdx.x == 0) *ready = value;
+}
+
+__global__ __launch_bounds__(256) void corr_hand_pose_kernel(const float *__restrict__ hand_pose, int64_t N, float *__restrict__ pose) {
+    const int64_t i = (int64_t)blockIdx.x * 256 + threadIdx.x;
+    if (i >= N * 156) return;
+    const int64_t n = i / 156;
+    const int k = (int)(i - n * 156);
+    pose[i] = k < 66 ? 0.f : hand_pose[n * 90 + (k - 66)];
+}
 
 CorrWs carve(const idf_correction_ctx *c, int B, int T, void *ws) {
     const int64_t N = (int64_t)B * T;
@@ -662,6 +724,9 @@
     w.proj_keep = (float *)take((size_t)B * idf_objproj_keep_floats() * 4);
     w.smpl_ws_bytes = interdiff_smpl_workspace_bytes(c->smpl, N);
     w.smpl_ws = take(w.smpl_ws_bytes);
+    w.hints = (unsigned short *)take((size_t)N * c->n_points * sizeof(unsigned short));
+    w.ready = (uint32_t *)take(sizeof(uint32_t));
+    w.base = (float *)take(interdiff_smpl_blend_base_bytes(c->smpl, N));
     w.total = off;
     return w;
 }
@@ -736,7 +801,7 @@
 
 int idf_point_order(hipStream_t s, const float *obj_points, int B, int P, int32_t *porder) {
     if (P > MAXP) return IDF_E_INVAL;
-    hipLaunchKernelGGL(corr_point_order_kernel, dim3((unsigned)B), dim3(1024), 0, s, obj_points, P, porder);
+    hipLaunchKernelGGL(corr_point_order_kernel, dim3((unsigned)B), dim3(1024), 0, s, obj_points, P, porder, nullptr, 0u);
     return IDF_OK;
 }
 
@@ -749,7 +814,7 @@
     if (idf_opt_in_lds(reinterpret_cast<const void *>(corr_contact_kernel<true>), 160 * 1024 - 16384, lds_ok) != IDF_OK) return IDF_E_LAUNCH;
     hipLaunchKernelGGL(corr_contact_kernel<true>, dim3((unsigned)N, 2), dim3(CT), lds, s, verts, V, obj_points, P, porder, nullptr, nullptr, nullptr,
                        nullptr, nullptr, nullptr, nullptr, c->vorder, c->vrank, nullptr, 0, B, nullptr, nullptr, nullptr, nullptr, nullptr, yidx, nullptr, (int64_t)0,
-                       pts_frame, frames_per_clip, PredArgs{});
+                       pts_frame, frames_per_clip, PredArgs{}, nullptr);
     return IDF_OK;
 }
 
@@ -775,7 +840,7 @@
 static int correction_impl(const idf_correction_ctx *c, float *x0, const float *gt, const float *hand_pose,
                            const float *beta, const float *obj_points, int32_t B, int32_t T, float blend_t, const float *blend_table,
                            const int64_t *blend_state, uint8_t *condition, int32_t *contact, float *distance, float *loss, void *ws,
-                           size_t ws_bytes, void *stream) {
+                           size_t ws_bytes, void *stream, bool prepared = false, uint64_t *stats = nullptr) {
     if (!c || !c->smpl || !c->objproj || !x0 || !gt || !hand_pose || !beta || !obj_points || !ws || B <= 0 || T <= 0) return IDF_E_INVAL;
     const int V = c->smpl->V, M = c->n_markers, P = c->n_points;
     if (c->smpl->J != 52 || c->smpl->n_betas != 10 || M > MAXM || M != c->objproj->P || P > MAXP || T != c->objproj->T ||
@@ -789,8 +854,10 @@
     idf_prof_mark(IDF_K_CORR_PREPARE, s);
     hipLaunchKernelGGL(corr_prepare_kernel, dim3((unsigned)idf_cdiv(N * 24, 256)), dim3(256), 0, s, x0, gt, hand_pose, B, T, w.pose,
                        w.trans, w.objR, w.objT, w.gt_angles, w.gt_trans);
-    int rc = interdiff_smpl_forward(c->smpl, w.pose, beta, w.trans, N, w.verts, w.jtr, nullptr, w.smpl_ws, w.smpl_ws_bytes, stream);
+    int rc = prepared ? interdiff_smpl_forward_based(c->smpl, w.pose, beta, w.trans, N, w.verts, w.jtr, nullptr, w.base, w.smpl_ws, w.smpl_ws_bytes, stream)
+                      : interdiff_smpl_forward(c->smpl, w.pose, beta, w.trans, N, w.verts, w.jtr, nullptr, w.smpl_ws, w.smpl_ws_bytes, stream);
     if (rc) return rc;
+    if (stats && hipMemsetAsync(stats, 0, IDF_CONTACT_STATS * sizeof(uint64_t), s) != hipSuccess) return IDF_E_LAUNCH;
     idf_prof_mark(IDF_K_CORR_CONTACT, s);
     PredArgs pred{};
     if (fused) {
@@ -800,7 +867,8 @@
         pred.nclips = B;
     }
     rc = launch_contact(s, N, w.verts, V, obj_points, P, w.porder, w.objR, w.objT, c, B, fused ? nullptr : w.markers, w.loss_sum, w.min_dist, w.label, nullptr,
-                        nullptr, nullptr, (int64_t)c->past_len * B, &pred);
+                        nullptr, reinterpret_cast<unsigned long long *>(stats), (int64_t)c->past_len * B, &pred, prepared ? w.hints : nullptr, prepared ? w.ready : nullptr,
+                        sample_ready_value(c, B, T));
     if (rc) return rc;
     uint8_t *cond = condition ? condition : w.condition;
     int32_t *cont = contact ? contact : w.contact;
@@ -834,6 +902,35 @@
                                         const int64_t *state, void *ws, size_t ws_bytes, void *stream) {
     if (!table || !state) return IDF_E_INVAL;
     return correction_impl(c, x0, gt, hand_pose, beta, obj_points, B, T, 0.f, table, state, nullptr, nullptr, nullptr, nullptr, ws, ws_bytes, stream);
+}
+
+extern "C" int interdiff_correction_begin_sample(const idf_correction_ctx *c, const float *hand_pose, const float *beta, const float *obj_points, int32_t B,
+                                                 int32_t T, void *ws, size_t ws_bytes, void *stream) {
+    if (!c || !c->smpl || !hand_pose || !beta || !obj_points || !ws || B <= 0 || T <= 0 || c->n_points > MAXP) return IDF_E_INVAL;
+    if (c->smpl->J != 52) return IDF_E_INVAL;
+    CorrWs w = carve(c, B, T, ws);
+    if (ws_bytes < w.total) return IDF_E_NOMEM;
+    hipStream_t s = idf_stream(stream);
+    const int64_t N = (int64_t)B * T;
+    idf_prof_mark(IDF_K_CORR_PREPARE, s);
+    hipLaunchKernelGGL(corr_point_order_kernel, dim3((unsigned)B), dim3(1024), 0, s, obj_points, c->n_points, w.porder, nullptr, 0u);
+    const size_t n16 = idf_align((size_t)N * c->n_points * sizeof(unsigned short)) / 16;
+    hipLaunchKernelGGL(corr_begin_kernel, dim3((unsigned)std::min<size_t>(1024, idf_cdiv((int64_t)n16, 256))), dim3(256), 0, s, reinterpret_cast<uint4 *>(w.hints), n16, w.ready,
+                       sample_ready_value(c, B, T));
+    hipLaunchKernelGGL(corr_hand_pose_kernel, dim3((unsigned)idf_cdiv(N * 156, 256)), dim3(256), 0, s, hand_pose, N, w.pose);
+    const int rc = interdiff_smpl_blend_base(c->smpl, w.pose, beta, N, w.base, w.smpl_ws, w.smpl_ws_bytes, stream);
+    if (rc) return rc;
+    idf_prof_mark(-1, s);
+    IDF_CHECK_LAUNCH();
+    return IDF_OK;
+}
+
+extern "C" int interdiff_correction_prepared(const idf_correction_ctx *c, float *x0, const float *gt, const float *hand_pose, const float *beta,
+                                             const float *obj_points, int32_t B, int32_t T, float blend_t, const float *table, const int64_t *state,
+                                             uint8_t *condition, int32_t *contact, float *distance, float *loss, uint64_t *stats, void *ws, size_t ws_bytes,
+                                             void *stream) {
+    if ((table != nullptr) != (state != nullptr)) return IDF_E_INVAL;
+    return correction_impl(c, x0, gt, hand_pose, beta, obj_points, B, T, blend_t, table, state, condition, contact, distance, loss, ws, ws_bytes, stream, true, stats);
 }
 
 namespace {
@@ -944,9 +1041,9 @@
     return carve_metrics(c, B, T, nullptr).total;
 }
 
-extern "C" int interdiff_contact_nn(const idf_correction_ctx *c, const float *verts, const float *obj_points, const float *objR,
-                                    const float *objT, int32_t B, int32_t T, float *o2h, int32_t *idx, uint64_t *stats, void *ws,
-                                    size_t ws_bytes, void *stream) {
+static int contact_nn_impl(const idf_correction_ctx *c, const float *verts, const float *obj_points, const float *objR,
+                           const float *objT, int32_t B, int32_t T, float *o2h, int32_t *idx, uint64_t *stats, uint16_t *hints, void *ws,
+                           size_t ws_bytes, void *stream) {
     if (!c || !c->smpl || !verts || !obj_points || !objR || !objT || !ws || B <= 0 || T <= 0 || (!o2h && !idx)) return IDF_E_INVAL;
     if (c->n_markers > MAXM || c->n_points > MAXP) return IDF_E_INVAL;
     MetWs w = carve_metrics(c, B, T, ws);
@@ -954,10 +1051,22 @@
     hipStream_t s = idf_stream(stream);
     if (stats && hipMemsetAsync(stats, 0, IDF_CONTACT_STATS * sizeof(uint64_t), s) != hipSuccess) return IDF_E_LAUNCH;
     const int rc = launch_contact(s, (int64_t)B * T, verts, c->smpl->V, obj_points, c->n_points, w.porder, objR, objT, c, B, w.markers, w.loss_sum,
-                                  w.min_dist, w.label, o2h ? o2h : w.o2h, idx, reinterpret_cast<unsigned long long *>(stats), 0);
+                                  w.min_dist, w.label, o2h ? o2h : w.o2h, idx, reinterpret_cast<unsigned long long *>(stats), 0, nullptr, hints);
     if (rc) return rc;
     IDF_CHECK_LAUNCH();
     return IDF_OK;
+}
+
+extern "C" int interdiff_contact_nn(const idf_correction_ctx *c, const float *verts, const float *obj_points, const float *objR,
+                                    const float *objT, int32_t B, int32_t T, float *o2h, int32_t *idx, uint64_t *stats, void *ws,
+                                    size_t ws_bytes, void *stream) {
+    return contact_nn_impl(c, verts, obj_points, objR, objT, B, T, o2h, idx, stats, nullptr, ws, ws_bytes, stream);
+}
+
+extern "C" int interdiff_contact_nn_hinted(const idf_correction_ctx *c, const float *verts, const float *obj_points, const float *objR,
+                                           const float *objT, int32_t B, int32_t T, float *o2h, int32_t *idx, uint64_t *stats, uint16_t *hints,
+                                           void *ws, size_t ws_bytes, void *stream) {
+    return contact_nn_impl(c, verts, obj_points, objR, objT, B, T, o2h, idx, stats, hints, ws, ws_bytes, stream);
 }
 
 extern "C" size_t interdiff_metrics_workspace_bytes(const idf_correction_ctx *c, int32_t B, int32_t T) {
diff --git a/interdiff_amd/csrc/smpl.hip b/interdiff_amd/csrc/smpl.hip
--- a/interdiff_amd/csrc/smpl.hip
+++ b/interdiff_amd/csrc/smpl.hip
@@ -1,6 +1,7 @@
 #include "common.h"
 #include "rot_math.h"
 #include <algorithm>
+#include <type_traits>
 
 #ifndef IDF_SMPL_STAMP
 #define IDF_SMPL_STAMP(i) do { } while (0)
@@ -66,7 +67,7 @@
             a[r * 4 + 1] = g[r * 4 + 1];
             a[r * 4 + 2] = g[r * 4 + 2];
             a[r * 4 + 3] = g[r * 4 + 3] - (g[r * 4] * jx + g[r * 4 + 1] * jy + g[r * 4 + 2] * jz);
-            jtr[((size_t)n * J + j) * 3 + r] = g[r * 4 + 3] + trans[n * 3 + r];
+            if (jtr) jtr[((size_t)n * J + j) * 3 + r] = g[r * 4 + 3] + trans[n * 3 + r];
         }
     }
 }
@@ -78,14 +79,17 @@
 constexpr int SF = 16;
 constexpr int TBF = 10, TBV = 4;
 
-template <int NG>
+constexpr int NGS = 12;
+enum { MODE_FULL = 0, MODE_BASE = 1, MODE_STEP = 2 };
+template <int NG, int MODE>
 __global__ __launch_bounds__(BT) void smpl_blend_skin_kernel(const idf_smpl_model m, const float *__restrict__ feat,
                                                               const float *__restrict__ A, const float *__restrict__ trans,
                                                               int64_t N, float *__restrict__ verts,
-                                                              float *__restrict__ v_posed) {
+                                                              float *__restrict__ v_posed, float *__restrict__ base,
+                                                              const uint32_t *__restrict__ ready, uint32_t ready_want) {
     extern __shared__ __attribute__((aligned(16))) float sm[];
     idf_args_now(m.V, m.J, m.S, m.blend, m.skin_idx, m.skin_w, feat, A, trans, N, verts, v_posed, gridDim.x);
-    constexpr int KB = 16 * NG, nq = KB / 4;
+    constexpr int KB = 16 * NG;
     const int V = m.V, J = m.J, S = m.S;
     float *As = sm, *stage = sm;
     const int tid = threadIdx.x, lane = tid & 63, wave = (tid >> 6) & 3, fh = tid >> 8, li = lane & 15, kq = lane >> 4;
@@ -101,28 +105,48 @@
     const int v0 = vtile * VT;
     IDF_SMPL_STAMP(0);
 
+    bool from_base = false;
+    if constexpr (MODE == MODE_STEP) from_base = __builtin_amdgcn_readfirstlane((int)(*ready == ready_want)) != 0;
+    const int g_lo = MODE == MODE_BASE ? NGS : 0;
+    const int KS = MODE == MODE_BASE ? KB - 16 * NGS : (from_base ? 16 * NGS : KB);
     {
         const uint32_t as_lds = idf_lds_addr(As);
-        const int ncell = FT * nq;
+        const int nqs = KS / 4, ncell = FT * nqs;
         for (int i = wave; i * 64 < ncell; i += BT / 64) {
-            const int p = min(i * 64 + lane, ncell - 1), row = p / nq, pos = p - row * nq;
-            idf_dma16_v(feat + (size_t)min(f0 + row, N - 1) * KB + ((pos ^ ((row >> 1) & 7)) << 2), as_lds + (uint32_t)(i * 1024));
+            const int p = min(i * 64 + lane, ncell - 1), row = p / nqs, pos = p - row * nqs;
+            idf_dma16_v(feat + (size_t)min(f0 + row, N - 1) * KB + ((4 * g_lo + (pos ^ ((row >> 1) & 7))) << 2), as_lds + (uint32_t)(i * 1024));
         }
     }
     const int vl = tid & 63, vme = v0 + vl;
     float sw[4];
     int so[4];
-#pragma unroll
-    for (int k = 0; k < 4; ++k) {
-        const size_t e = (size_t)min(vme, V - 1) * S + min(k, S - 1);
-        sw[k] = m.skin_w[e];
-        so[k] = m.skin_idx[e] * 12;
-    }
-#pragma unroll
-    for (int k = 0; k < 4; ++k) {
-        const bool ok = k < S && vme < V;
-        sw[k] = ok ? sw[k] : 0.f;
-        so[k] = ok ? so[k] : 0;
+    if constexpr (MODE != MODE_BASE) {
+#pragma unroll
+        for (int k = 0; k < 4; ++k) {
+            const size_t e = (size_t)min(vme, V - 1) * S + min(k, S - 1);
+            sw[k] = m.skin_w[e];
+            so[k] = m.skin_idx[e] * 12;
+        }
+#pragma unroll
+        for (int k = 0; k < 4; ++k) {
+            const bool ok = k < S && vme < V;
+            sw[k] = ok ? sw[k] : 0.f;
+            so[k] = ok ? so[k] : 0;
+        }
+    }
+    f32x4 acc[FM][3];
+    f32x4 *bacc = reinterpret_cast<f32x4 *>(base) + ((size_t)(ftile * nvt + vtile) * 4 + wave) * (FM * 3 * 64) + lane;
+#pragma unroll
+    for (int i = 0; i < FM; ++i)
+#pragma unroll
+        for (int t = 0; t < 3; ++t) acc[i][t] = f32x4{0.f, 0.f, 0.f, 0.f};
+    if constexpr (MODE == MODE_STEP) {
+        if (from_base) {
+#pragma unroll
+            for (int i = 0; i < FM; ++i)
+#pragma unroll
+                for (int t = 0; t < 3; ++t) acc[i][t] = bacc[(i * 3 + t) * 64];
+        }
     }
     asm volatile("s_waitcnt vmcnt(0)" ::: "memory");
     __syncthreads();
@@ -131,22 +155,17 @@
     const float *brow[3];
 #pragma unroll
     for (int t = 0; t < 3; ++t) brow[t] = m.blend + ((size_t)((vtile * 4 + wave) * 3 + t) * NG * 64 + lane) * 4;
-    f32x4 acc[FM][3];
-#pragma unroll
-    for (int i = 0; i < FM; ++i)
-#pragma unroll
-        for (int t = 0; t < 3; ++t) acc[i][t] = f32x4{0.f, 0.f, 0.f, 0.f};
     constexpr int PD = 3;
     float4 bq[PD + 1][3];
     auto ldg = [&](float4 (&dst)[3], int gi) {
 #pragma unroll
         for (int t = 0; t < 3; ++t) dst[t] = *reinterpret_cast<const float4 *>(brow[t] + gi * 256);
     };
-    auto mac = [&](const float4 (&bc)[3], int gi) {
+    auto mac = [&](const float4 (&bc)[3], int gi, int ks, int glo) {
 #pragma unroll
         for (int i = 0; i < FM; ++i) {
             const int row = (fh * FM + i) * 16 + li;
-            const float4 a = *reinterpret_cast<const float4 *>(As + row * KB + (((gi * 4 + kq) ^ ((row >> 1) & 7)) << 2));
+            const float4 a = *reinterpret_cast<const float4 *>(As + row * ks + ((((gi - glo) * 4 + kq) ^ ((row >> 1) & 7)) << 2));
 #pragma unroll
             for (int t = 0; t < 3; ++t) acc[i][t] = __builtin_amdgcn_mfma_f32_16x16x4f32(a.x, bc[t].x, acc[i][t], 0, 0, 0);
 #pragma unroll
@@ -157,14 +176,30 @@
             for (int t = 0; t < 3; ++t) acc[i][t] = __builtin_amdgcn_mfma_f32_16x16x4f32(a.w, bc[t].w, acc[i][t], 0, 0, 0);
         }
     };
-#pragma unroll
-    for (int g = 0; g < PD && g < NG; ++g) ldg(bq[g], g);
-#pragma unroll
-    for (int g = 0; g < NG; ++g) {
-        if (g + PD < NG) ldg(bq[(g + PD) % (PD + 1)], g + PD);
-        __builtin_amdgcn_sched_barrier(0);
-        mac(bq[g % (PD + 1)], g);
-        __builtin_amdgcn_sched_barrier(0);
+    auto run = [&](auto first_c, auto n_c, int ks, int glo) {
+        constexpr int first = decltype(first_c)::value, n = decltype(n_c)::value;
+#pragma unroll
+        for (int s = 0; s < PD && s < n; ++s) ldg(bq[s], (first + s) % NG);
+#pragma unroll
+        for (int s = 0; s < n; ++s) {
+            if (s + PD < n) ldg(bq[(s + PD) % (PD + 1)], (first + s + PD) % NG);
+            __builtin_amdgcn_sched_barrier(0);
+            mac(bq[s % (PD + 1)], (first + s) % NG, ks, glo);
+            __builtin_amdgcn_sched_barrier(0);
+        }
+    };
+    if constexpr (MODE == MODE_BASE) {
+        run(std::integral_constant<int, NGS>{}, std::integral_constant<int, NG - NGS>{}, KB - 16 * NGS, NGS);
+#pragma unroll
+        for (int i = 0; i < FM; ++i)
+#pragma unroll
+            for (int t = 0; t < 3; ++t) bacc[(i * 3 + t) * 64] = acc[i][t];
+        return;
+    } else if constexpr (MODE == MODE_STEP) {
+        if (from_base) run(std::integral_constant<int, 0>{}, std::integral_constant<int, NGS>{}, 16 * NGS, 0);
+        else run(std::integral_constant<int, NGS>{}, std::integral_constant<int, NG>{}, KB, 0);
+    } else {
+        run(std::integral_constant<int, NGS>{}, std::integral_constant<int, NG>{}, KB, 0);
     }
     __syncthreads();
     IDF_SMPL_STAMP(2);
@@ -235,11 +270,36 @@
     return idf_align((size_t)N * m->KB * sizeof(float)) + idf_align(((size_t)N + SF) * m->J * 12 * sizeof(float));
 }
 
-extern "C" int interdiff_smpl_forward(const idf_smpl_model *m, const float *pose, const float *betas, const float *trans,
-                                      int64_t N, float *verts, float *jtr, float *v_posed, void *ws, size_t ws_bytes,
-                                      void *stream) {
+extern "C" size_t interdiff_smpl_blend_base_bytes(const idf_smpl_model *m, int64_t N) {
+    if (!m || N < 0) return 0;
+    return idf_align((size_t)idf_cdiv(N, FT) * idf_cdiv(m->V, VT) * FT * NTC * sizeof(float)) + idf_align(sizeof(uint32_t));
+}
+
+namespace {
+
+uint32_t base_ready_value(const idf_smpl_model *m, int64_t N) {
+    return 0x5b1e7d00u ^ ((uint32_t)N * 2654435761u) ^ ((uint32_t)m->V * 40503u) ^ (uint32_t)m->KB;
+}
+
+__global__ void smpl_base_ready_kernel(uint32_t *ready, uint32_t value) { *ready = value; }
+
+int smpl_check(const idf_smpl_model *m, size_t &lds) {
+    if (m->J < 1 || m->J > MAXJ || m->KB % 16 != 0 || m->KB < 9 * (m->J - 1) + m->n_betas + 1 || m->S < 1) return IDF_E_INVAL;
+    lds = std::max((size_t)FT * m->KB, (size_t)((FT * STS + 255) & ~255) + ((SF * m->J * 12 + 255) & ~255) + (size_t)SF * NTC + FT * 3) * sizeof(float);
+    if (lds > 150 * 1024 || m->KB % 32 != 0 || (m->V * 3) % 2 != 0 || m->S > 4) return IDF_E_INVAL;
+    if (m->KB != 480) return IDF_E_INVAL;
+    return IDF_OK;
+}
+
+unsigned blend_grid(const idf_smpl_model *m, int64_t N) {
+    return (unsigned)(idf_cdiv(idf_cdiv(N, FT), TBF) * idf_cdiv(idf_cdiv(m->V, VT), TBV) * TBF * TBV);
+}
+
+int smpl_forward_impl(const idf_smpl_model *m, const float *pose, const float *betas, const float *trans, int64_t N, float *verts, float *jtr,
+                      float *v_posed, float *base, void *ws, size_t ws_bytes, void *stream) {
     if (!m || !pose || !betas || !trans || !verts || !jtr || !ws || N < 0) return IDF_E_INVAL;
-    if (m->J < 1 || m->J > MAXJ || m->KB % 16 != 0 || m->KB < 9 * (m->J - 1) + m->n_betas + 1 || m->S < 1) return IDF_E_INVAL;
+    size_t lds = 0;
+    if (const int rc = smpl_check(m, lds)) return rc;
     if (ws_bytes < interdiff_smpl_workspace_bytes(m, N)) return IDF_E_NOMEM;
     if (N == 0) return IDF_OK;
     hipStream_t s = idf_stream(stream);
@@ -247,16 +307,56 @@
     float *A = reinterpret_cast<float *>(reinterpret_cast<char *>(ws) + idf_align((size_t)N * m->KB * sizeof(float)));
     idf_prof_mark(IDF_K_SMPL_POSE, s);
     hipLaunchKernelGGL(smpl_pose_kernel, dim3((unsigned)N), dim3(64), 0, s, *m, pose, betas, trans, feat, A, jtr);
-    const size_t lds = std::max((size_t)FT * m->KB, (size_t)((FT * STS + 255) & ~255) + ((SF * m->J * 12 + 255) & ~255) + (size_t)SF * NTC + FT * 3) * sizeof(float);
-    if (lds > 150 * 1024 || m->KB % 32 != 0 || (m->V * 3) % 2 != 0 || m->S > 4) return IDF_E_INVAL;
-    if (m->KB != 480) return IDF_E_INVAL;
-    static std::atomic<uint64_t> lds_ok{0};
-    if (lds > 64 * 1024 && idf_opt_in_lds(reinterpret_cast<const void *>(smpl_blend_skin_kernel<30>), 150 * 1024, lds_ok) != IDF_OK) return IDF_E_LAUNCH;
     idf_prof_mark(IDF_K_SMPL_BLEND_SKIN, s);
-    const unsigned nwg_launch = (unsigned)(idf_cdiv(idf_cdiv(N, FT), TBF) * idf_cdiv(idf_cdiv(m->V, VT), TBV) * TBF * TBV);
-    hipLaunchKernelGGL(smpl_blend_skin_kernel<30>, dim3(nwg_launch), dim3(BT), lds, s, *m,
-                       feat, A, trans, N, verts, v_posed);
+    if (base) {
+        static std::atomic<uint64_t> lds_ok{0};
+        if (lds > 64 * 1024 && idf_opt_in_lds(reinterpret_cast<const void *>(smpl_blend_skin_kernel<30, MODE_STEP>), 150 * 1024, lds_ok) != IDF_OK) return IDF_E_LAUNCH;
+        const uint32_t *ready = reinterpret_cast<const uint32_t *>(reinterpret_cast<char *>(base) + interdiff_smpl_blend_base_bytes(m, N) - idf_align(sizeof(uint32_t)));
+        hipLaunchKernelGGL((smpl_blend_skin_kernel<30, MODE_STEP>), dim3(blend_grid(m, N)), dim3(BT), lds, s, *m, feat, A, trans, N, verts, v_posed, base, ready,
+                           base_ready_value(m, N));
+    } else {
+        static std::atomic<uint64_t> lds_ok{0};
+        if (lds > 64 * 1024 && idf_opt_in_lds(reinterpret_cast<const void *>(smpl_blend_skin_kernel<30, MODE_FULL>), 150 * 1024, lds_ok) != IDF_OK) return IDF_E_LAUNCH;
+        hipLaunchKernelGGL((smpl_blend_skin_kernel<30, MODE_FULL>), dim3(blend_grid(m, N)), dim3(BT), lds, s, *m, feat, A, trans, N, verts, v_posed, nullptr, nullptr, 0u);
+    }
     idf_prof_mark(-1, s);
     IDF_CHECK_LAUNCH();
     return IDF_OK;
 }
+
+}
+
+extern "C" int interdiff_smpl_forward(const idf_smpl_model *m, const float *pose, const float *betas, const float *trans,
+                                      int64_t N, float *verts, float *jtr, float *v_posed, void *ws, size_t ws_bytes,
+                                      void *stream) {
+    return smpl_forward_impl(m, pose, betas, trans, N, verts, jtr, v_posed, nullptr, ws, ws_bytes, stream);
+}
+
+extern "C" int interdiff_smpl_blend_base(const idf_smpl_model *m, const float *pose, const float *betas, int64_t N, float *base, void *ws,
+                                         size_t ws_bytes, void *stream) {
+    if (!m || !pose || !betas || !base || !ws || N < 0) return IDF_E_INVAL;
+    size_t lds = 0;
+    if (const int rc = smpl_check(m, lds)) return rc;
+    if (ws_bytes < interdiff_smpl_workspace_bytes(m, N)) return IDF_E_NOMEM;
+    if (N == 0) return IDF_OK;
+    hipStream_t s = idf_stream(stream);
+    float *feat = reinterpret_cast<float *>(ws);
+    float *A = reinterpret_cast<float *>(reinterpret_cast<char *>(ws) + idf_align((size_t)N * m->KB * sizeof(float)));
+    idf_prof_mark(IDF_K_SMPL_POSE, s);
+    hipLaunchKernelGGL(smpl_pose_kernel, dim3((unsigned)N), dim3(64), 0, s, *m, pose, betas, (const float *)nullptr, feat, A, (float *)nullptr);
+    idf_prof_mark(IDF_K_SMPL_BLEND_SKIN, s);
+    const size_t lds_base = (size_t)FT * (m->KB - 16 * NGS) * sizeof(float);
+    hipLaunchKernelGGL((smpl_blend_skin_kernel<30, MODE_BASE>), dim3(blend_grid(m, N)), dim3(BT), lds_base, s, *m, feat, (const float *)nullptr, (const float *)nullptr, N,
+                       (float *)nullptr, (float *)nullptr, base, (const uint32_t *)nullptr, 0u);
+    uint32_t *ready = reinterpret_cast<uint32_t *>(reinterpret_cast<char *>(base) + interdiff_smpl_blend_base_bytes(m, N) - idf_align(sizeof(uint32_t)));
+    hipLaunchKernelGGL(smpl_base_ready_kernel, dim3(1), dim3(1), 0, s, ready, base_ready_value(m, N));
+    idf_prof_mark(-1, s);
+    IDF_CHECK_LAUNCH();
+    return IDF_OK;
+}
+
+extern "C" int interdiff_smpl_forward_based(const idf_smpl_model *m, const float *pose, const float *betas, const float *trans, int64_t N, float *verts,
+                                            float *jtr, float *v_posed, float *base, void *ws, size_t ws_bytes, void *stream) {
+    if (!base) return IDF_E_INVAL;
+    return smpl_forward_impl(m, pose, betas, trans, N, verts, jtr, v_posed, base, ws, ws_bytes, stream);
+}
diff --git a/interdiff_amd/diffusion.py b/interdiff_amd/diffusion.py
--- a/interdiff_amd/diffusion.py
+++ b/interdiff_amd/diffusion.py
@@ -224,18 +224,28 @@
         cond = model_kwargs.get('y', {}).get('cond') if isinstance(model_kwargs.get('y', None), dict) else None
         if cond is not None and hasattr(model, 'prepare_memory'):
             model.prepare_memory(cond)
-        for it, i in enumerate(range(t_first, t_first - todo, -1)):
-            t, th = ts[i], ts_hook[i]
-            t.host_value = th.host_value = i
-            if step_noise is None:
-                nz = None
-            elif callable(step_noise):
-                nz = step_noise(it, img).contiguous()
-            else:
-                nz = step_noise[it]
-            self._step(model, img, None, i, it, t, model_kwargs, denoised_fn, nz, seed, elem0, rows_kw, th, rows)
-            if dump_steps is not None and it in dump_steps:
-                dump.append(img.clone())
+        y = model_kwargs.get('y', None)
+        gate = graph_sampler.hook_gate(denoised_fn)
+        per_sample = (getattr(denoised_fn, 'begin_sample', None) is not None and isinstance(y, dict) and all(k in y for k in graph_sampler.HOOK_KEYS)
+                      and any(gate(i) for i in range(t_first, t_first - todo, -1)))
+        if per_sample:
+            denoised_fn.begin_sample(y, shape[0], shape[-1])
+        try:
+            for it, i in enumerate(range(t_first, t_first - todo, -1)):
+                t, th = ts[i], ts_hook[i]
+                t.host_value = th.host_value = i
+                if step_noise is None:
+                    nz = None
+                elif callable(step_noise):
+                    nz = step_noise(it, img).contiguous()
+                else:
+                    nz = step_noise[it]
+                self._step(model, img, None, i, it, t, model_kwargs, denoised_fn, nz, seed, elem0, rows_kw, th, rows)
+                if dump_steps is not None and it in dump_steps:
+                    dump.append(img.clone())
+        finally:
+            if per_sample:
+                denoised_fn.end_sample()
         return dump if dump_steps is not None else img
 
     def sample_timesteps(self, B, device, generator=None):
diff --git a/interdiff_amd/graph_sampler.py b/interdiff_amd/graph_sampler.py
--- a/interdiff_amd/graph_sampler.py
+++ b/interdiff_amd/graph_sampler.py
@@ -69,6 +69,8 @@
         self.y = {k: torch.empty(y[k].shape, dtype=torch.float32, device=entry.x.device) for k in HOOK_KEYS}
         self.y['inpainted_motion'] = entry.gt if entry.gt is not None else torch.empty_like(entry.x)
         self.fresh = True
+        self.per_sample = getattr(hook, 'begin_sample', None) is not None
+        self.apply_kw = {'prepared': True} if self.per_sample else {}
 
 
 class Entry:
@@ -143,7 +145,9 @@
         for k in HOOK_KEYS + (() if self.gt is not None else ('inpainted_motion',)):
             hk.y[k].copy_(y[k])
         if hk.fresh:
-            hook.apply_dev(hk.y['inpainted_motion'].clone(), table, torch.zeros(8, dtype=torch.int64, device=self.x.device), hk.y, hk.ws)
+            if hk.per_sample:
+                hook.begin_sample(hk.y, self.x.shape[0], self.x.shape[-1], ws=hk.ws)
+            hook.apply_dev(hk.y['inpainted_motion'].clone(), table, torch.zeros(8, dtype=torch.int64, device=self.x.device), hk.y, hk.ws, **hk.apply_kw)
             torch.cuda.synchronize(self.x.device)
             hk.fresh = False
         return hk
@@ -205,7 +209,7 @@
         self.enqueue_forward()
         if st.mask is not None:
             diffusion.inpaint(st.x0, st.gt, st.mask)
-        self.hook.apply_dev(st.x0, self.table, st.state, self.hk.y, self.hk.ws)
+        self.hook.apply_dev(st.x0, self.table, st.state, self.hk.y, self.hk.ws, **self.hk.apply_kw)
         self.finish_hook_step(st.x0)
 
     def graph(self, key, enqueue, *args):
@@ -284,11 +288,22 @@
     fuse_hook = hook_capturable(hook, y)
     run = Run(model, st, table, rows, fused, split, hook, st.hook_buffers(hook, y, table) if fuse_hook else None, tmap)
 
+    gate = hook_gate(hook)
+    if run.hk is not None and run.hk.per_sample and any(gate(i) for i in range(t_start, t_start - todo, -1)):
+        hook.begin_sample(run.hk.y, B, T, ws=run.hk.ws)
     st.x.copy_(img)
     st.state.copy_(diffusion.seeded_state(t_start, seed, elem0))
     if split:
         for ch in st.chains[1:]:
             ch.state.copy_(diffusion.seeded_state(t_start, seed, elem0 + ch.sl.start * per_clip))
     st.ts.fill_(diff.timestep_map[t_start])
-    dump = run.play(plan_steps(t_start, todo, hook_gate(hook), dump_steps, fuse_hook), t_start, diff._timesteps(B, dev, loop_side=True), model_kwargs)
+    eager_sample = (not fuse_hook and getattr(hook, 'begin_sample', None) is not None and all(k in y for k in HOOK_KEYS)
+                    and any(gate(i) for i in range(t_start, t_start - todo, -1)))
+    if eager_sample:
+        hook.begin_sample(y, B, T)
+    try:
+        dump = run.play(plan_steps(t_start, todo, gate, dump_steps, fuse_hook), t_start, diff._timesteps(B, dev, loop_side=True), model_kwargs)
+    finally:
+        if eager_sample:
+            hook.end_sample()
     return dump if dump_steps is not None else st.x.clone()
```

After: 7.051 million. -1.5%, worse.
